# Roywangj/AdaptPoint

Measured on AMD Instinct MI355X. Metric: set-abstraction fwd+bwd point-clouds/sec (B=32,N=1024), higher is better.
Workload: dtype bf16

## Files before the change

adaptpoint_amd/_lib.py:

```python
import ctypes
import os

_HERE = os.path.dirname(os.path.abspath(__file__))
LIB_PATH = os.path.join(_HERE, "libadaptpoint_amd.so")
if os.environ.get("APN_LIB_PATH"):
    if os.environ.get("APN_ALLOW_UNSAFE_LIB") != "1":
        raise RuntimeError("APN_LIB_PATH is for diagnostic builds: set APN_ALLOW_UNSAFE_LIB=1 with it")
    LIB_PATH = os.path.abspath(os.environ["APN_LIB_PATH"])
REQUIRED_BUILD_FLAGS = ("-ffp-contract=off", "-fno-slp-vectorize")

_c_int, _c_float, _c_void_p = ctypes.c_int, ctypes.c_float, ctypes.c_void_p
_c_double = ctypes.c_double
_c_longlong = ctypes.c_longlong

SIGNATURES = {
    "apn_version": [],
    "apn_furthest_point_sampling": [_c_int] * 3 + [_c_void_p] * 4,
    "apn_ball_query": [_c_int] * 3 + [_c_float, _c_int] + [_c_void_p] * 4,
    "apn_group_points": [_c_int] * 5 + [_c_void_p] * 4,
    "apn_group_points_grad": [_c_int] * 5 + [_c_void_p] * 4,
    "apn_gather_points": [_c_int] * 4 + [_c_void_p] * 4,
    "apn_gather_points_grad": [_c_int] * 4 + [_c_void_p] * 4,
    "apn_resample_points": [_c_int] * 6 + [_c_void_p] * 6,
    "apn_three_nn": [_c_int] * 3 + [_c_void_p] * 5,
    "apn_three_interpolate": [_c_int] * 4 + [_c_void_p] * 5,
    "apn_three_interpolate_grad": [_c_int] * 4 + [_c_void_p] * 5,
    "apn_furthest_point_sampling_tuned": [_c_int] * 3 + [_c_void_p] * 3 + [_c_int] * 2 + [_c_void_p],
    "apn_fps_debug_stamps": [_c_int] * 3 + [_c_void_p] * 5,
    "apn_furthest_point_sampling_xyz": [_c_int] * 3 + [_c_void_p] * 5,
    "apn_ball_query_zero": [_c_int] * 3 + [_c_float, _c_int] + [_c_void_p] * 4,
    "apn_sa_grid_blocks": [_c_int] * 2,
    "apn_sa_grid_rows": [_c_int] * 3,
    "apn_sa_bwd_main_rows": [_c_int] * 2,
    "apn_sa_acc_words": [_c_int],
    "apn_sa_debug_stamps": [_c_void_p],
    "apn_zero_fill": [_c_void_p, _c_longlong, _c_void_p],
    "apn_debug_stamp": [_c_void_p, _c_int, _c_void_p],
    "apn_debug_vgpr_hold": [_c_int, _c_int, _c_void_p, _c_void_p],
    "apn_debug_vpk_probe": [_c_int, _c_int, _c_int, _c_void_p, _c_void_p],
    "apn_sa_geo_dd_doubles": [_c_int],
    "apn_sa_point_geo": [_c_int] * 4 + [_c_float] + [_c_void_p] * 6,
    "apn_sa_prep_rows": [_c_int] * 2,
    "apn_sa_prep_stats": [_c_int] * 2 + [_c_void_p] * 4 + [_c_int] * 2 + [_c_void_p] * 3 + [_c_longlong, _c_void_p],
    "apn_sa_reduce_rows": [_c_void_p, _c_int, _c_int, _c_double, _c_void_p, _c_void_p],
    "apn_sa_reduce_acc": [_c_void_p, _c_int, _c_double, _c_void_p, _c_void_p],
    "apn_sa_bn_fold": [_c_void_p, _c_int, _c_void_p, _c_int, _c_double, _c_void_p, _c_void_p,
                       _c_float, _c_float, _c_void_p, _c_void_p, _c_void_p, _c_int, _c_void_p,
                       _c_void_p, _c_int, _c_void_p, _c_void_p],
    "apn_sa_fwd_main": [_c_int] * 4 + [_c_float] + [_c_void_p] * 12 + [_c_float, _c_float, _c_int, _c_double,
                                                                        _c_void_p, _c_int] + [_c_void_p] * 7,
    "apn_sa_fwd_out": [_c_int] * 3 + [_c_void_p] * 8 + [_c_float, _c_float, _c_int, _c_double] + [_c_void_p] * 2
                      + [_c_int] + [_c_void_p] * 3 + [_c_int] + [_c_void_p] * 2 + [_c_longlong, _c_void_p],
    "apn_sa_bwd_prep_rows": [_c_int] * 2,
    "apn_sa_bwd_prep": [_c_int] * 3 + [_c_void_p] + [_c_longlong] * 3 + [_c_void_p] + [_c_int]
                       + [_c_void_p] * 3 + [_c_int] + [_c_void_p] * 8,
    "apn_sa_bwd_main": [_c_int] * 4 + [_c_float] + [_c_void_p] * 11 + [_c_double, _c_int] + [_c_void_p] * 9,
    "apn_sa_bwd_weight_rows": [_c_int] * 2,
    "apn_sa_bwd_point_grads": [_c_int] * 3 + [_c_void_p] * 7 + [_c_double, _c_int] + [_c_void_p] * 2 + [_c_int]
                              + [_c_void_p] * 4 + [_c_float] + [_c_void_p] * 5,
    "apn_sa_bwd_finalize": [_c_void_p, _c_int, _c_float, _c_void_p, _c_void_p, _c_int, _c_void_p, _c_void_p, _c_int]
                           + [_c_void_p] * 11,
    "apn_sa_forward_seq": ([_c_int] * 5 + [_c_float] + [_c_void_p] * 12
                           + [_c_void_p] * 5 + [_c_float, _c_float, _c_int]
                           + [_c_void_p] * 5 + [_c_float, _c_float, _c_int]
                           + [_c_double, _c_int] + [_c_void_p] * 11 + [_c_longlong, _c_void_p]),
    "apn_sa_backward_seq": ([_c_int] * 5 + [_c_float] + [_c_void_p] * 15 + [_c_int] * 3
                            + [_c_double] + [_c_void_p] + [_c_longlong] * 3 + [_c_void_p]
                            + [_c_longlong]
                            + [_c_void_p] * 26),
    "apn_attention_small_max": [],
    "apn_attention_small_fwd": [_c_int] * 3 + [_c_void_p] * 5,
    "apn_attention_small_bwd": [_c_int] * 3 + [_c_void_p] * 8,
    "apn_attention_prep": [_c_int] * 3 + [_c_void_p] * 4 + [_c_int, _c_void_p],
    "apn_attention_fwd": [_c_int] * 3 + [_c_void_p] * 4,
    "apn_attention_bwd": [_c_int] * 3 + [_c_void_p] * 9,
    "apn_token_attention_max_tokens": [],
    "apn_token_attention_fwd": [_c_int] * 3 + [_c_void_p] * 4,
    "apn_token_attention_bwd": [_c_int] * 3 + [_c_void_p] * 7,
    "apn_pointset_group_rows": [_c_int] * 3,
    "apn_pointset_group_max": [_c_int] * 5 + [_c_void_p] * 8,
    "apn_pointset_group_max_grad": [_c_int] * 5 + [_c_void_p] * 9,
    "apn_sa_wide_grid": [_c_int] * 2,
    "apn_sa_wide_colsum_chunks": [_c_int] * 2,
    "apn_sa_wide_colsum": [_c_void_p, _c_int, _c_int, _c_void_p, _c_void_p, _c_void_p],
    "apn_sa_wide_tilemap_ints": [_c_int] * 2,
    "apn_sa_wide_tilemap": [_c_int] * 3 + [_c_void_p] * 3,
    "apn_sa_wide_tilemap_many": [_c_int] * 4 + [_c_void_p] * 3,
    "apn_sa_rowmap_many": [_c_int] * 4 + [_c_void_p] * 6,
    "apn_sa_rowmap_ints": [_c_int] * 2,
    "apn_sa_rowmap_places": [_c_int] * 3,
    "apn_sa_wide_stats1": [_c_int] * 4 + [_c_void_p] * 6,
    "apn_sa_wide_fwd_main": [_c_int] * 5 + [_c_void_p] * 11,
    "apn_sa_wide_bwd_main": [_c_int] * 5 + [_c_void_p] * 15,
    "apn_sa_wide_wgrad_fused": [_c_int],
    "apn_sa_wide_image": [_c_void_p, _c_int, _c_int, _c_void_p, _c_int, _c_int, _c_int, _c_void_p, _c_void_p],
    "apn_sa_wide_bwd_prep_rows": [_c_int] * 2,
    "apn_sa_wide_bwd_prep": [_c_int] * 3 + [_c_void_p] + [_c_longlong] * 3 + [_c_void_p] * 7,
    "apn_sa_wide_consts2": [_c_void_p, _c_int, _c_void_p, _c_int, _c_void_p, _c_double, _c_int] + [_c_void_p] * 4,
    "apn_sa_wide_consts1": [_c_void_p, _c_int, _c_void_p, _c_int, _c_void_p, _c_double, _c_int] + [_c_void_p] * 4,
    "apn_sa_wide_point_terms": [_c_int] * 4 + [_c_void_p] * 5 + [_c_int, _c_float] + [_c_void_p] * 7,
    "apn_sa_wide_wgrad_splits": [_c_int] * 3,
    "apn_sa_wide_csr": [_c_int] * 3 + [_c_void_p] * 9,
    "apn_sa_wide_fwd_prep": [_c_int] * 6 + [_c_float] + [_c_void_p] * 13,
    "apn_sa_wide_fwd_prep_rows": [_c_int] * 3,
    "apn_sa_wide_out": [_c_int] * 3 + [_c_void_p] * 2 + [_c_int] + [_c_void_p] * 3 + [_c_int] + [_c_void_p] * 2,
    "apn_sa_wide_bwd_mid": [_c_void_p, _c_int, _c_void_p, _c_int, _c_int, _c_void_p, _c_double, _c_int] + [_c_void_p] * 7,
    "apn_sa_wide_bwd_fin": [_c_void_p, _c_int, _c_void_p, _c_int, _c_int, _c_void_p, _c_double, _c_int] + [_c_void_p] * 8,
    "apn_sa_wide_point_grads_rows": [_c_int] * 2,
    "apn_sa_wide_point_grads_cols": [_c_int] * 3,
    "apn_sa_wide_point_grads": [_c_int] * 5 + [_c_float] + [_c_void_p] * 13 + [_c_int] + [_c_void_p] * 9,
    "apn_sa_wide_colsum_f32": [_c_void_p, _c_int, _c_int, _c_void_p, _c_void_p],
    "apn_sa_wide_wgrad": [_c_int] * 5 + [_c_void_p] * 7 + [_c_int] + [_c_void_p] * 2,
    "apn_pw_conv_tiles": [_c_int] * 2,
    "apn_pw_conv_forward": [_c_int] * 5 + [_c_void_p] * 5,
    "apn_pw_bn_act": [_c_int] * 3 + [_c_void_p] * 2 + [_c_int] + [_c_void_p] * 2 + [_c_float] * 2 + [_c_int] * 2
                     + [_c_void_p] * 6,
    "apn_pw_bn_act_grad_splits": [_c_int] * 2,
    "apn_pw_bn_act_grad": [_c_int] * 3 + [_c_void_p] * 3 + [_c_int] * 2 + [_c_void_p] * 5,
    "apn_pw_conv_grad_input": [_c_int] * 5 + [_c_void_p] * 4,
    "apn_pw_conv_grad_weight_splits": [_c_int] * 4,
    "apn_pw_conv_grad_weight": [_c_int] * 5 + [_c_void_p] * 5,
    "apn_deform_forward": [_c_int] * 3 + [_c_void_p] * 6 + [_c_float] + [_c_void_p] * 4,
    "apn_deform_backward": [_c_int] * 3 + [_c_void_p] * 4 + [_c_float] + [_c_void_p] * 7,
    "apn_pw_contract_splits": [_c_int] * 4,
    "apn_pw_contract": [_c_int] * 4 + [_c_void_p, _c_longlong, _c_int, _c_int] * 2 + [_c_void_p, _c_longlong, _c_int, _c_int,
                                                                                         _c_void_p, _c_int, _c_void_p],
    "apn_pw_contract2_splits": [_c_int] * 9,
    "apn_pw_contract2": [_c_int] * 3 + [_c_void_p] * 16,
    "apn_fp_blend_stats": [_c_int] * 4 + [_c_void_p] * 6 + [_c_int] + [_c_void_p] * 4 + [_c_float, _c_int] + [_c_void_p] * 3,
    "apn_pw_transpose": [_c_int] * 3 + [_c_void_p] * 3,
    "apn_three_nn_weights": [_c_longlong] + [_c_void_p] * 3,
    "apn_anchor_transforms": [_c_int] + [_c_void_p] * 3 + [_c_float] * 3 + [_c_void_p] * 3,
    "apn_anchor_transforms_grad": [_c_int] + [_c_void_p] * 3 + [_c_float] * 3 + [_c_void_p] * 4,
    "apn_pw_conv_max_tiles": [_c_int],
    "apn_pw_conv_max_forward": [_c_int] * 5 + [_c_void_p] * 3 + [_c_int] + [_c_void_p] * 5,
    "apn_pw_conv_max_backward": [_c_int] * 4 + [_c_void_p] * 5 + [_c_int] + [_c_void_p] * 5,
    "apn_spectral_norm_blocks": [_c_int] * 2,
    "apn_spectral_norm": [_c_int] * 2 + [_c_void_p, _c_int, _c_float] + [_c_void_p] * 8,
    "apn_spectral_norm_grad": [_c_int] * 2 + [_c_void_p] * 8,
    "apn_spectral_norm_many": [_c_int] + [_c_void_p] * 3 + [_c_int, _c_float] + [_c_void_p] * 8,
    "apn_spectral_norm_grad_many": [_c_int] + [_c_void_p] * 10,
    "apn_sa_sample_overlap": [_c_int] * 3 + [_c_float, _c_int] + [_c_void_p] * 7,
    "apn_sa_sample_seq": [_c_int] * 3 + [_c_float, _c_int] + [_c_void_p] * 8,
    "apn_furthest_point_sampling_nested": [_c_int] * 3 + [_c_void_p] * 6,
    "apn_sa_sample_seq_nested": [_c_int] * 3 + [_c_float, _c_int] + [_c_void_p] * 9,
    "apn_pointwolf_params": [_c_int] * 2 + [_c_void_p, _c_int] + [_c_float] * 3 + [_c_void_p] * 4,
    "apn_rsmix_select": [_c_int] * 3 + [_c_void_p] * 2 + [_c_double, _c_int, _c_int] + [_c_void_p] * 3,
    "apn_rsmix_mix": [_c_int] * 4 + [_c_void_p] * 8,
    "apn_cloud_transform": [_c_int] * 4 + [_c_void_p] * 2 + [_c_int] * 2 + [_c_void_p] * 8,
    "apn_cls_confusion": [_c_int] * 2 + [_c_void_p, _c_int] + [_c_void_p] * 5,
    "apn_la_pool_rows": [_c_int] * 2,
    "apn_la_pool_fwd": [_c_int] * 4 + [_c_float] + [_c_void_p] * 3 + [_c_int] + [_c_void_p] * 7,
    "apn_la_stats_fold": [_c_void_p, _c_int, _c_int, _c_double, _c_void_p, _c_void_p],
    "apn_la_pool_bwd": [_c_int] * 4 + [_c_float] + [_c_void_p] * 11 + [_c_int] + [_c_void_p] * 4,
    "apn_knn_query": [_c_int] * 5 + [_c_void_p] * 5,
    "apn_knn_dilated": [_c_int] * 7 + [_c_void_p] * 6,
    "apn_ec_pool_rows": [_c_int] * 2,
    "apn_ec_pool_fwd": [_c_int] * 4 + [_c_void_p, _c_int] + [_c_void_p] * 7,
    "apn_ec_out": [_c_int] * 3 + [_c_void_p] * 2 + [_c_float] + [_c_void_p] * 2,
    "apn_ec_bwd_prep_rows": [_c_int] * 2,
    "apn_ec_bwd_prep": [_c_int] * 3 + [_c_void_p] + [_c_longlong] * 3 + [_c_void_p] * 2 + [_c_float] + [_c_void_p] * 3,
    "apn_ec_out_res": [_c_int] * 3 + [_c_void_p] * 2 + [_c_float, _c_void_p] + [_c_longlong] * 3 + [_c_void_p] * 2,
    "apn_ec_bwd_prep_act": [_c_int] * 3 + [_c_void_p] + [_c_longlong] * 3 + [_c_void_p] * 2 + [_c_float] + [_c_void_p] * 3,
    "apn_ec_csr": [_c_int] * 3 + [_c_void_p] * 5,
    "apn_ec_pool_bwd": [_c_int] * 4 + [_c_void_p] * 5 + [_c_int] + [_c_void_p] * 4,
    "apn_chamfer_max_points": [],
    "apn_chamfer_forward": [_c_int] * 3 + [_c_void_p] * 7,
    "apn_chamfer_backward": [_c_int] * 3 + [_c_void_p] * 9,
    "apn_emd_max_points": [],
    "apn_emd_one_launch_max": [],
    "apn_emd_cost_parts": [_c_int],
    "apn_emd_ratios": [_c_int] * 3 + [_c_void_p] * 6,
    "apn_emd_match": [_c_int] * 3 + [_c_void_p] * 6,
    "apn_emd_cost": [_c_int] * 3 + [_c_void_p] * 8,
    "apn_emd_cost_grad": [_c_int] * 3 + [_c_void_p] * 9,
    "apn_po_knn_query": [_c_int] * 4 + [_c_void_p] * 7,
    "apn_po_ball_query": [_c_int] * 3 + [_c_float, _c_int] + [_c_void_p] * 6,
    "apn_po_furthest_sampling": [_c_int] * 2 + [_c_void_p] * 6,
    "apn_po_csr": [_c_int] * 3 + [_c_void_p] * 5,
    "apn_po_grouping_fwd": [_c_int] * 4 + [_c_void_p] * 4,
    "apn_po_grouping_bwd": [_c_int] * 4 + [_c_void_p] * 5,
    "apn_po_interpolation_fwd": [_c_int] * 4 + [_c_void_p] * 5,
    "apn_po_interpolation_bwd": [_c_int] * 4 + [_c_void_p] * 6,
    "apn_po_subtraction_fwd": [_c_int] * 4 + [_c_void_p] * 5,
    "apn_po_subtraction_bwd": [_c_int] * 4 + [_c_void_p] * 6,
    "apn_po_aggregation_fwd": [_c_int] * 5 + [_c_void_p] * 6,
    "apn_po_aggregation_bwd": [_c_int] * 5 + [_c_void_p] * 11,
    "apn_pt_rows": [_c_int] * 3,
    "apn_pt_mid_rows": [_c_int] * 3,
    "apn_pt_rel_stats": [_c_int] * 3 + [_c_void_p, _c_int] + [_c_void_p] * 5,
    "apn_pt_fold": [_c_void_p, _c_int, _c_int, _c_void_p, _c_void_p],
    "apn_pt_colsum_rows": [_c_int],
    "apn_pt_colsum": [_c_int, _c_int, _c_void_p, _c_int, _c_void_p, _c_void_p],
    "apn_pt_mid": [_c_int] * 3 + [_c_void_p, _c_int] + [_c_void_p] * 7,
    "apn_pt_attend": [_c_int] * 3 + [_c_void_p, _c_int] + [_c_void_p] * 8,
    "apn_pt_attend_bwd": [_c_int] * 3 + [_c_void_p, _c_int] + [_c_void_p] * 10,
    "apn_pt_mid_bwd": [_c_int] * 3 + [_c_void_p, _c_int] + [_c_void_p] * 9,
    "apn_pt_rel_bwd": [_c_int] * 3 + [_c_void_p, _c_int] + [_c_void_p] * 12 + [_c_int, _c_void_p, _c_void_p],
    "apn_pt_scatter_bwd": [_c_int] * 3 + [_c_void_p] * 6 + [_c_int, _c_void_p],
    "apn_vg_scratch_ints": [_c_int],
    "apn_vg_voxelize": [_c_int] * 3 + [_c_void_p] + [_c_double] * 3 + [_c_void_p] * 9,
    "apn_vg_mean_fwd": [_c_int] * 3 + [_c_void_p] * 6,
    "apn_vg_mean_bwd": [_c_int] * 3 + [_c_void_p] * 5,
    "apn_rl_moment_rows": [_c_int] * 3,
    "apn_rl_bwd_rows": [_c_int] * 4,
    "apn_rl_moments": [_c_int] * 3 + [_c_void_p] * 3 + [_c_int] + [_c_void_p] * 3,
    "apn_rl_fold": [_c_int, _c_void_p, _c_double] + [_c_void_p] * 4 + [_c_float, _c_float, _c_int] + [_c_void_p] * 6,
    "apn_rl_forward": [_c_int] * 4 + [_c_void_p] * 3 + [_c_int] + [_c_void_p] * 4,
    "apn_rl_backward": [_c_int] * 4 + [_c_void_p] * 3 + [_c_int] + [_c_void_p] * 6,
    "apn_rl_finalize": [_c_int, _c_int, _c_void_p, _c_void_p, _c_double] + [_c_void_p] * 4 + [_c_int] + [_c_void_p] * 3,
    "apn_ag_moment_rows": [_c_int],
    "apn_ag_point_rows": [_c_int],
    "apn_ag_moments": [_c_int] * 5 + [_c_void_p] * 5,
    "apn_ag_fold": [_c_int] * 2 + [_c_void_p] * 3,
    "apn_ag_combine_fwd": [_c_int] * 5 + [_c_void_p] * 7 + [_c_int] + [_c_void_p] * 4 + [_c_float, _c_int] + [_c_void_p] * 3,
    "apn_ag_combine_bwd": [_c_int] * 5 + [_c_void_p] * 11,
    "apn_ag_sigma_bwd": [_c_int] * 5 + [_c_void_p] * 11,
    "apn_ag_res_relu_max": [_c_int] * 4 + [_c_void_p] * 5,
    "apn_ag_res_relu_max_grad": [_c_int] * 4 + [_c_void_p] * 6,
}

_lib = None


class ExtensionMissing(RuntimeError):
    pass


def load():
    global _lib
    if _lib is not None:
        return _lib
    if not os.path.exists(LIB_PATH):
        raise ExtensionMissing(
            f"{LIB_PATH} not found: build it with `python -m adaptpoint_amd.build` "
            "(hipcc --offload-arch=gfx950). There is no fallback path.")
    lib = ctypes.CDLL(LIB_PATH)
    for name, argtypes in SIGNATURES.items():
        fn = getattr(lib, name)
        fn.argtypes = argtypes
        fn.restype = _c_int
    lib.apn_error_string.argtypes = [_c_int]
    lib.apn_error_string.restype = ctypes.c_char_p
    lib.apn_build_flags.argtypes = []
    lib.apn_build_flags.restype = ctypes.c_char_p
    flags = lib.apn_build_flags().decode("utf-8", "replace").split()
    missing = [f for f in REQUIRED_BUILD_FLAGS if f not in flags]
    if missing and os.environ.get("APN_ALLOW_UNSAFE_LIB") != "1":
        raise ExtensionMissing(f"{LIB_PATH} was built without {missing} (its flags: {' '.join(flags)}): rebuild with "
                               "`python -m adaptpoint_amd.build --force`")
    _lib = lib
    return lib


def check(code, what):
    if code != 0:
        msg = load().apn_error_string(code).decode("utf-8", "replace")
        raise RuntimeError(f"{what} failed: {msg} (code {code})")
```

adaptpoint_amd/csrc/sa_fused.hip:

```cpp
#include "apn_common.h"
#include "apn_mfma.h"
#include <type_traits>
#include "sa_chain.h"

namespace apn {

constexpr int SA_C = 32;
constexpr int SA_C1 = 32;
constexpr int SA_C2 = 64;
constexpr int SA_K = 32;
constexpr int SA_WAVES = 4;

template <int NS>
__device__ __forceinline__ void put_frag(uint4 *base, int f, int lane, const Frag<NS> &v) {
#pragma unroll
    for (int p = 0; p < NS; ++p) base[(f * NS + p) * 64 + lane] = __builtin_bit_cast(uint4, v.p[p]);
}

template <int NS>
__device__ __forceinline__ Frag<NS> get_frag(const uint4 *base, int f, int lane) {
    Frag<NS> v;
#pragma unroll
    for (int p = 0; p < NS; ++p) v.p[p] = __builtin_bit_cast(bf16x8, base[(f * NS + p) * 64 + lane]);
    return v;
}

template <int NS>
__device__ __forceinline__ float eff(float v) {
    const __bf16 hi = (__bf16)v;
    float r = (float)hi;
    if (NS == 2) r += (float)(__bf16)(v - r);
    return r;
}

struct SaArgs {
    int b, n, m;
    const float *xyz;
    const float *new_xyz;
    const __bf16 *ft;
    const __bf16 *ft_lo;
    const int *idx;
    const float *w1;
    float radius;
    const int *tmap;
    unsigned long long *stamps;
};

__device__ __forceinline__ void stamp(const SaArgs &a, int wave, int k) {
    if (a.stamps && (threadIdx.x & 63) == 0)
        a.stamps[((size_t)blockIdx.x * SA_WAVES + wave) * 16 + k] = wall_clock64();
}

__device__ __forceinline__ int tm_tiles(const SaArgs &a) { return a.tmap[0]; }
__device__ __forceinline__ const int *tm_tq0(const SaArgs &a) { return a.tmap + 4; }
__device__ __forceinline__ const unsigned *tm_rows(const SaArgs &a) {
    return reinterpret_cast<const unsigned *>(a.tmap + 4 + ((a.b * a.m + 3) & ~3));
}
__device__ __forceinline__ const int *tm_nn(const SaArgs &a) {
    return a.tmap + 4 + ((a.b * a.m + 3) & ~3) + (size_t)32 * a.b * a.m;
}
__device__ __forceinline__ unsigned ri_q(unsigned info) { return info & 0xffu; }
__device__ __forceinline__ unsigned ri_slot(unsigned info) { return (info >> 8) & 0xffu; }
__device__ __forceinline__ unsigned ri_mult(unsigned info) { return (info >> 16) & 0xffu; }
__device__ __forceinline__ void row_meta(unsigned info, int h, unsigned (&meta)[16]) {
#pragma unroll
    for (int i = 0; i < 16; ++i) meta[i] = (unsigned)__builtin_amdgcn_ds_bpermute(acc_row(i, h) << 2, (int)info);
}

template <int NS>
__device__ __forceinline__ void load_w1_frags(const float *__restrict__ w1, int r, int h,
                                              Frag<NS> (&wf)[3]) {
#pragma unroll
    for (int s = 0; s < 3; ++s) {
        float t[8];
#pragma unroll
        for (int j = 0; j < 8; ++j)
            t[j] = s < 2 ? w1[r * 35 + 3 + 16 * s + 8 * h + j]
                         : ((h == 0 && j < 3) ? w1[r * 35 + j] : 0.0f);
        wf[s] = make_frag<NS>(t);
    }
}

constexpr int PS_PTS = 512, PS_MAX_ROWS = 64, PS_NT = 2 * PS_PTS;
constexpr double GEO_INV_UNIT = 1.0 / 68719476736.0;

#ifdef APN_WG_STAMPS
__device__ unsigned long long *d_wg_stamps_f = nullptr;
__device__ __forceinline__ void wg_stamp(int k) {
    unsigned long long *st = d_wg_stamps_f;
    if (st && threadIdx.x == 0) st[(size_t)blockIdx.x * 16 + k] = wall_clock64();
}
#else
__device__ __forceinline__ void wg_stamp(int) {}
#endif

template <int NS>
__global__ __launch_bounds__(PS_NT) void sa_prep_stats_kernel(
    int n, int tiles_per_cloud, int total_tiles, const float *__restrict__ f, const long long *__restrict__ geo,
    const double *__restrict__ dd, int dd_rows, const float *__restrict__ w1, int stats, __bf16 *__restrict__ ft,
    __bf16 *__restrict__ ft_lo, float *__restrict__ part, unsigned long long *__restrict__ zero, long long zero_words) {
    extern __shared__ float sf_raw[];
    float (*sf)[PS_PTS + 1] = reinterpret_cast<float (*)[PS_PTS + 1]>(sf_raw);
    __shared__ float4 sgeo[PS_PTS];
    __shared__ float red[PS_NT / 64][64];
    __shared__ double sdd[6];
    const int tid = threadIdx.x, lane = tid & 63, r = lane & 31, h = lane >> 5;
    const int wave = __builtin_amdgcn_readfirstlane(tid >> 6);
    critical_stream_priority();
    wg_stamp(0);
    for (long long e = (long long)blockIdx.x * PS_NT + tid; e < zero_words; e += (long long)gridDim.x * PS_NT) zero[e] = 0ull;
    Frag<NS> wf[3];
    load_w1_frags<NS>(w1, r, h, wf);
    const float wp0 = eff<NS>(w1[r * 35]), wp1 = eff<NS>(w1[r * 35 + 1]), wp2 = eff<NS>(w1[r * 35 + 2]);
    float s1 = 0.0f, s2 = 0.0f;
    for (int tile = blockIdx.x; tile < total_tiles; tile += gridDim.x) {
        const int cloud = tile / tiles_per_cloud, n0 = (tile % tiles_per_cloud) * PS_PTS;
        {
            const int pt = tid & (PS_PTS - 1), cg = tid / PS_PTS;
            const bool in = n0 + pt < n;
            float v[16];
#pragma unroll
            for (int k = 0; k < 16; ++k) v[k] = in ? f[((size_t)cloud * SA_C + cg + 2 * k) * n + n0 + pt] : 0.0f;
            float4 gv = make_float4(0.f, 0.f, 0.f, 0.f);
            if (stats && in && cg == 0) {
                const longlong2 *gp = reinterpret_cast<const longlong2 *>(geo + ((size_t)cloud * n + n0 + pt) * 4);
                const longlong2 g0 = gp[0], g1 = gp[1];
                gv = make_float4((float)g0.x, (float)((double)g0.y * GEO_INV_UNIT), (float)((double)g1.x * GEO_INV_UNIT),
                                 (float)((double)g1.y * GEO_INV_UNIT));
            }
            wg_stamp(1);
            __syncthreads();
#pragma unroll
            for (int k = 0; k < 16; ++k) sf[cg + 2 * k][pt] = v[k];
            if (cg == 0) sgeo[pt] = gv;
            wg_stamp(2);
        }
        __syncthreads();
        wg_stamp(3);
        const int pt = 32 * wave + r;
        float x0[8], x1[8];
#pragma unroll
        for (int j = 0; j < 8; ++j) { x0[j] = sf[8 * h + j][pt]; x1[j] = sf[16 + 8 * h + j][pt]; }
        const Frag<NS> a0 = make_frag<NS>(x0), a1 = make_frag<NS>(x1);
        if (n0 + pt < n) {
            uint4 *row = reinterpret_cast<uint4 *>(ft + ((size_t)cloud * n + n0 + pt) * SA_C);
            row[h] = __builtin_bit_cast(uint4, a0.p[0]);
            row[2 + h] = __builtin_bit_cast(uint4, a1.p[0]);
            if (NS == 2) {
                uint4 *rl = reinterpret_cast<uint4 *>(ft_lo + ((size_t)cloud * n + n0 + pt) * SA_C);
                rl[h] = __builtin_bit_cast(uint4, a0.p[NS - 1]);
                rl[2 + h] = __builtin_bit_cast(uint4, a1.p[NS - 1]);
            }
        }
        wg_stamp(4);
        if (stats) {
            f32x16 y = {0};
            y = mfma<NS>(a0, wf[0], y);
            y = mfma<NS>(a1, wf[1], y);
#pragma unroll
            for (int i = 0; i < 16; ++i) {
                const float4 g = sgeo[32 * wave + acc_row(i, h)];
                const float PD = __builtin_fmaf(wp2, g.w, __builtin_fmaf(wp1, g.z, wp0 * g.y));
                const float oF = g.x * y[i];
                s1 += oF + PD;
                s2 += __builtin_fmaf(oF, y[i], 2.0f * y[i] * PD);
            }
        }
    }
    wg_stamp(5);
    if (!stats) return;
    s1 += __shfl_xor(s1, 32);
    s2 += __shfl_xor(s2, 32);
    if (lane < 32) { red[wave][r] = s1; red[wave][32 + r] = s2; }
    if (blockIdx.x == 0 && wave >= 1 && wave < 7) {
        double s = 0.0;
        for (int e = lane; e < dd_rows; e += 64) s += dd[(size_t)e * 6 + (wave - 1)];
#pragma unroll
        for (int o = 32; o > 0; o >>= 1) s += __shfl_xor(s, o);
        if (lane == 0) sdd[wave - 1] = s;
    }
    __syncthreads();
    if (tid < 64) {
        float val = 0.0f;
#pragma unroll
        for (int w = 0; w < PS_NT / 64; ++w) val += red[w][tid];
        if (tid >= 32 && blockIdx.x == 0) {
            const double wx = wp0, wy = wp1, wz = wp2;
            const double t = wx * wx * sdd[0] + 2.0 * wx * wy * sdd[1] + 2.0 * wx * wz * sdd[2] + wy * wy * sdd[3] +
                             2.0 * wy * wz * sdd[4] + wz * wz * sdd[5];
            val += (float)t;
        }
        part[(size_t)blockIdx.x * 64 + tid] = val;
    }
    wg_stamp(6);
}

template <int NS>
struct TileRaw {
    uint4 f[2], fl[NS];
    float px, py, pz;
    float qx, qy, qz;
    int nb;
    unsigned info;
    int q0;
};

struct TileHead {
    int nb, q0;
    unsigned info;
    int tile;
};
template <bool CP>
__device__ __forceinline__ TileHead load_head(const SaArgs &a, int tile, int r) {
    TileHead t;
    t.tile = tile;
    if (CP) {
        t.nb = tm_nn(a)[(size_t)tile * SA_K + r];
        t.info = tm_rows(a)[(size_t)tile * SA_K + r];
        t.q0 = tm_tq0(a)[tile];
    } else {
        t.nb = a.idx[(size_t)tile * SA_K + r];
        t.info = 0x10000u | ((unsigned)r << 8);
        t.q0 = tile;
    }
    return t;
}

template <typename T>
__device__ __forceinline__ T ld_off(const void *base, unsigned byte_off) {
    return *reinterpret_cast<const T *>(reinterpret_cast<const char *>(base) + byte_off);
}

template <int NS>
__device__ __forceinline__ void fetch_tile(const SaArgs &a, const TileHead &hd, int h, TileRaw<NS> &t) {
    const int nb = hd.nb;
    const unsigned cloud = (unsigned)(hd.q0 / a.m);
    const unsigned pt = cloud * (unsigned)a.n + (unsigned)nb;
    const unsigned rowoff = pt * (unsigned)(SA_C * 2) + 16u * (unsigned)h;
    t.f[0] = ld_off<uint4>(a.ft, rowoff);
    t.f[1] = ld_off<uint4>(a.ft, rowoff + 32u);
    if (NS == 2) {
        t.fl[0] = ld_off<uint4>(a.ft_lo, rowoff);
        t.fl[NS - 1] = ld_off<uint4>(a.ft_lo, rowoff + 32u);
    }
    struct xyz3 { float x, y, z; };
    const xyz3 pp = ld_off<xyz3>(a.xyz, pt * 12u);
    t.px = pp.x; t.py = pp.y; t.pz = pp.z;
    const unsigned q = (unsigned)hd.q0 + (ri_mult(hd.info) ? ri_q(hd.info) : 0u);
    const xyz3 qq = ld_off<xyz3>(a.new_xyz, q * 12u);
    t.qx = qq.x; t.qy = qq.y; t.qz = qq.z;
    t.nb = nb;
    t.info = hd.info;
    t.q0 = hd.q0;
}

template <int NS>
__device__ __forceinline__ void build_frags(const SaArgs &a, const TileRaw<NS> &t, int h,
                                            Frag<NS> (&x)[3], float *deff = nullptr) {
    x[0].p[0] = __builtin_bit_cast(bf16x8, t.f[0]);
    x[1].p[0] = __builtin_bit_cast(bf16x8, t.f[1]);
    if (NS == 2) {
        x[0].p[NS - 1] = __builtin_bit_cast(bf16x8, t.fl[0]);
        x[1].p[NS - 1] = __builtin_bit_cast(bf16x8, t.fl[NS - 1]);
    }
    float d[8] = {0.f, 0.f, 0.f, 0.f, 0.f, 0.f, 0.f, 0.f};
    if (h == 0 || deff) {
        d[0] = (t.px - t.qx) / a.radius;
        d[1] = (t.py - t.qy) / a.radius;
        d[2] = (t.pz - t.qz) / a.radius;
    }
    if (deff) {
#pragma unroll
        for (int j = 0; j < 3; ++j) {
            const __bf16 hi = (__bf16)d[j];
            deff[j] = (float)hi;
            if (NS == 2) deff[j] += (float)(__bf16)(d[j] - (float)hi);
        }
        if (h != 0) d[0] = d[1] = d[2] = 0.0f;
    }
    x[2] = make_frag<NS>(d);
}

__device__ __forceinline__ void touch(const TileHead &hd) {
    asm volatile("" ::"v"(hd.nb), "v"(hd.info), "v"(hd.q0));
}

struct NoAhead {
    __device__ __forceinline__ void operator()(const TileHead &) const {}
};
template <int NS, bool CP, bool LATE = false, typename Pro, typename Pre, typename Body, typename Ahead = NoAhead>
__device__ __forceinline__ void for_each_tile(const SaArgs &a, int wave, int r, int h, Pro prologue, Pre pre, Body body,
                                              Ahead ahead = Ahead()) {
    const int cap = a.b * a.m, stride = gridDim.x * SA_WAVES;
    const int tiles = CP ? tm_tiles(a) : cap;
    const bool xcd = (gridDim.x & 7) == 0;
    const int per_x = (tiles + 7) >> 3;
    auto remap = [&](int t) {
        if (!xcd) return t;
        const int wg = t / SA_WAVES, wv = t - wg * SA_WAVES;
        const int x = wg & 7, u = (wg >> 3) * SA_WAVES + wv;
        return u < per_x ? x * per_x + u : tiles;
    };
    int slot = blockIdx.x * SA_WAVES + wave;
    int tile = remap(slot);
    const TileHead hd0 = load_head<CP>(a, tile < tiles ? tile : 0, r);
    TileHead hd_nxt = load_head<CP>(a, remap(slot + stride) < tiles ? remap(slot + stride) : 0, r);
    TileRaw<NS> cur, nxt;
    const bool any = tile < tiles;
    stamp(a, wave, 1);
    if (any) {
        ahead(hd0);
        fetch_tile<NS>(a, hd0, h, cur);
    }
    prologue();
    stamp(a, wave, 2);
    if (!any) return;
    int nst = 3;
    for (; tile < tiles; slot += stride, tile = remap(slot)) {
        const bool more = remap(slot + stride) < tiles;
        const int tile2 = remap(slot + 2 * stride);
        if (LATE) {
            const TileHead hd_nxt2 = load_head<CP>(a, tile2 < tiles ? tile2 : tile, r);
            body(tile, cur, nst == 4, [&] {
                asm volatile("" ::: "memory");
                touch(hd_nxt);
                if (more) {
                    ahead(hd_nxt);
                    fetch_tile<NS>(a, hd_nxt, h, cur);
                }
            });
            stamp(a, wave, nst < 5 ? nst : 5);
            ++nst;
            hd_nxt = hd_nxt2;
            continue;
        }
        touch(hd_nxt);
        pre();
        if (more) fetch_tile<NS>(a, hd_nxt, h, nxt);
        const TileHead hd_nxt2 = load_head<CP>(a, tile2 < tiles ? tile2 : tile, r);
        body(tile, cur, nst == 4, [&] { touch(hd_nxt2); });
        stamp(a, wave, nst < 5 ? nst : 5);
        ++nst;
        if (more) cur = nxt;
        hd_nxt = hd_nxt2;
    }
    pre();
    stamp(a, wave, 6);
}

template <int NV>
__device__ __forceinline__ float fold_partials(float (&vals)[NV], int lane, int wave) {
    __shared__ float red[SA_WAVES][NV][32];
#pragma unroll
    for (int i = 0; i < NV; ++i) {
        const float other = __shfl_xor(vals[i], 32);
        if (lane < 32) red[wave][i][lane] = vals[i] + other;
    }
    __syncthreads();
    float s = 0.0f;
    const int e = threadIdx.x;
    if (e < NV * 32) {
#pragma unroll
        for (int w = 0; w < SA_WAVES; ++w) s += red[w][e >> 5][e & 31];
    }
    return s;
}

__device__ __forceinline__ void fold_rows32(const float *__restrict__ part, int rows, const double *__restrict__ sums,
                                            const BnArgs &bn, float *__restrict__ pack, float &scale, float &shift,
                                            double *scratch ) {
    double (*fred)[64] = reinterpret_cast<double (*)[64]>(scratch);
    double *ftot = scratch + 16 * 64;
    const int tid = threadIdx.x;
    double count = bn.count;
    double gpre = 1.0, bpre = 0.0;
    if (tid < 32) {
        if (bn.gamma) gpre = (double)bn.gamma[tid];
        if (bn.beta) bpre = (double)bn.beta[tid];
    }
    if (bn.training) {
        if (part) {
            const int quad = tid & 15, rg = tid >> 4;
            const float4 *__restrict__ p4 = reinterpret_cast<const float4 *>(part) + quad;
            double s0 = 0.0, s1 = 0.0, s2 = 0.0, s3 = 0.0;
            int rr = rg;
            for (; rr + 7 * 16 < rows; rr += 8 * 16) {
                float4 v[8];
#pragma unroll
                for (int u = 0; u < 8; ++u) v[u] = p4[(size_t)(rr + 16 * u) * 16];
#pragma unroll
                for (int u = 0; u < 8; ++u) {
                    s0 += (double)v[u].x; s1 += (double)v[u].y; s2 += (double)v[u].z; s3 += (double)v[u].w;
                }
            }
            for (; rr + 3 * 16 < rows; rr += 4 * 16) {
                float4 v[4];
#pragma unroll
                for (int u = 0; u < 4; ++u) v[u] = p4[(size_t)(rr + 16 * u) * 16];
#pragma unroll
                for (int u = 0; u < 4; ++u) {
                    s0 += (double)v[u].x; s1 += (double)v[u].y; s2 += (double)v[u].z; s3 += (double)v[u].w;
                }
            }
            for (; rr < rows; rr += 16) {
                const float4 v = p4[(size_t)rr * 16];
                s0 += (double)v.x; s1 += (double)v.y; s2 += (double)v.z; s3 += (double)v.w;
            }
            fred[rg][4 * quad] = s0; fred[rg][4 * quad + 1] = s1; fred[rg][4 * quad + 2] = s2; fred[rg][4 * quad + 3] = s3;
            __syncthreads();
            if (tid < 64) {
                double s = 0.0;
#pragma unroll
                for (int k = 0; k < 16; ++k) s += fred[k][tid];
                ftot[tid] = s;
            }
        } else if (tid < 64) {
            ftot[tid] = sums[tid];
        }
// ... 385 lines not shown
        {
            const float4 *scv = reinterpret_cast<const float4 *>(bn1v[0][lane_o >> 5]);
            const float4 *shv = reinterpret_cast<const float4 *>(bn1v[1][lane_o >> 5]);
#pragma unroll
            for (int i4 = 0; i4 < 4; ++i4) {
                const float4 sc = scv[i4], sh = shv[i4];
                yT[4 * i4] = __builtin_fmaxf(__builtin_fmaf(yT[4 * i4], sc.x, sh.x), 0.0f);
                yT[4 * i4 + 1] = __builtin_fmaxf(__builtin_fmaf(yT[4 * i4 + 1], sc.y, sh.y), 0.0f);
                yT[4 * i4 + 2] = __builtin_fmaxf(__builtin_fmaf(yT[4 * i4 + 2], sc.z, sh.z), 0.0f);
                yT[4 * i4 + 3] = __builtin_fmaxf(__builtin_fmaf(yT[4 * i4 + 3], sc.w, sh.w), 0.0f);
            }
        }
        st2(1);
        Frag<NS> a0, a1;
        if (CP) {
            f32x16 yw;
#pragma unroll
            for (int i = 0; i < 16; ++i) yw[i] = yT[i] * mrow;
            a0 = pack8<NS>(yw, 0);
            a1 = pack8<NS>(yw, 8);
        } else {
            a0 = pack8<NS>(yT, 0);
            a1 = pack8<NS>(yT, 8);
        }

        Frag<NS> sp[4];
        {
            unsigned todo = starts;
            if (CP) {
                asm volatile("s_waitcnt vmcnt(0)" ::: "memory");
                const int dq = q0 - qb;
#pragma unroll
                for (int u = 0; u < 4; ++u) {
                    const int e = (u + dq < 4 ? u + dq : 3) * SA_C2 + lane_o;
                    gv4[u] = qgoa[wave][e];
                    kc4[u] = qksel[wave][e];
                }
            }
#pragma unroll 1
            for (int jb = 0; jb < nq; jb += 4) {
                if (jb) {
#pragma unroll
                    for (int u = 0; u < 4; ++u)
                        if (jb + u < nq) {
                            gv4[u] = g.goa[(size_t)(q0 + jb + u) * SA_C2 + lane];
                            kc4[u] = g.ksel[(size_t)(q0 + jb + u) * SA_C2 + lane];
                        }
                }
#pragma unroll
                for (int u = 0; u < 4; ++u) {
                    if (jb + u < nq) {
                        const float gv = gv4[u];
                        int kc = kc4[u];
                        if (CP) {
                            kc += __builtin_ctz(todo);
                            todo &= todo - 1u;
                        }
                        const __bf16 ghi = (__bf16)gv;
                        const __bf16 glo = (__bf16)(gv - (float)ghi);
                        __bf16 *cell = sp_img + kc * SP_ROW + lane;
                        cell[0] = ghi;
                        if (NS == 2) cell[SP_TILE] = glo;
                        if (!CP) kc4[u] = kc;
                    }
                }
            }
        }
        asm volatile("" ::: "memory");
        {
            f32x16 an;
            const float sc1 = chan[0][lane_o & 31], sh1 = chan[1][lane_o & 31];
#pragma unroll
            for (int i = 0; i < 16; ++i) {
                an[i] = __builtin_fmaxf(__builtin_fmaf(y1[i], sc1, sh1), 0.0f);
                if (CP) suma = __builtin_fmaf(multf(i), an[i], suma);
                else suma += an[i];
            }
            const Frag<NS> b0 = pack8<NS>(an, 0), b1 = pack8<NS>(an, 8);
            if (CP) {
                f32x16 aw;
#pragma unroll
                for (int i = 0; i < 16; ++i) aw[i] = an[i] * multf(i);
                gram = mfma<NS>(pack8<NS>(aw, 0), b0, gram);
                gram = mfma<NS>(pack8<NS>(aw, 8), b1, gram);
            } else {
                gram = mfma<NS>(b0, b0, gram);
                gram = mfma<NS>(b1, b1, gram);
            }
            typedef short tr_s4 __attribute__((ext_vector_type(4)));
            typedef short tr_s8 __attribute__((ext_vector_type(8)));
            typedef __attribute__((address_space(3))) tr_s4 tr_lds;
            const int li = lane_o & 15, gq = li >> 2, gp = li & 3, grh = (lane_o >> 4) & 1;
            const __bf16 *tb = sp_img + (4 * (lane_o >> 5) + gq) * SP_ROW + 16 * grh + 4 * gp;
#pragma unroll
            for (int t = 0; t < 2; ++t) {
#pragma unroll
                for (int sk = 0; sk < 2; ++sk) {
                    Frag<NS> at;
#pragma unroll
                    for (int pp = 0; pp < NS; ++pp) {
                        const __bf16 *src = tb + pp * SP_TILE + (16 * sk) * SP_ROW + 32 * t;
                        const tr_s4 lo4 = __builtin_amdgcn_ds_read_tr16_b64_v4i16((tr_lds *)(src));
                        const tr_s4 hi4 = __builtin_amdgcn_ds_read_tr16_b64_v4i16((tr_lds *)(src + 8 * SP_ROW));
                        const tr_s8 v8 = {lo4.x, lo4.y, lo4.z, lo4.w, hi4.x, hi4.y, hi4.z, hi4.w};
                        at.p[pp] = __builtin_bit_cast(bf16x8, v8);
                    }
                    dsp[t] = mfma<NS>(at, sk ? b1 : b0, dsp[t]);
                }
            }
        }
        st2(2);
#pragma unroll
        for (int s = 0; s < 4; ++s) {
            const __bf16 *src = sp_img + r * SP_ROW + 16 * s + 8 * h;
            sp[s].p[0] = *reinterpret_cast<const bf16x8 *>(src);
            if (NS == 2) sp[s].p[NS - 1] = *reinterpret_cast<const bf16x8 *>(src + SP_TILE);
        }
        asm volatile("" ::: "memory");
        if (!CP) {
            __bf16 *cell = sp_img + kc4[0] * SP_ROW + lane;
            cell[0] = (__bf16)0.0f;
            if (NS == 2) cell[SP_TILE] = (__bf16)0.0f;
        }
        f32x16 ga;
        const float ev = chan[4][lane_o & 31];
#pragma unroll
        for (int i = 0; i < 16; ++i) ga[i] = CP ? ev * multf(i) : ev;
        ga = mfma<NS>(a0, get_frag<NS>(cfrag, F_QM, lane_o), ga);
        ga = mfma<NS>(a1, get_frag<NS>(cfrag, F_QM + 1, lane_o), ga);
#pragma unroll
        for (int s = 0; s < 4; ++s) ga = mfma<NS>(sp[s], get_frag<NS>(cfrag, F_W2T + s, lane_o), ga);

        st2(3);
        float *gt = reinterpret_cast<float *>(sp_img);
        asm volatile("" ::: "memory");
        float s1 = 0.0f, s2 = 0.0f, hb = 0.0f;
        const float sc1l = chan[0][lane_o & 31], sh1l = chan[1][lane_o & 31], iv1 = chan[3][lane_o & 31];
        const float nmi = -chan[2][lane_o & 31] * iv1;
#pragma unroll
        for (int i = 0; i < 16; ++i) {
            const float u = __builtin_fmaf(y1[i], sc1l, sh1l);
            const float yhat = __builtin_fmaf(y1[i], iv1, nmi);
            ga[i] = u > 0.0f ? ga[i] : 0.0f;
            s1 += ga[i];
            s2 += ga[i] * yhat;
            if (CP) {
                gt[acc_row(i, h) * 33 + r] = ga[i];
                gt[32 * 33 + acc_row(i, h) * 33 + r] = multf(i) * yhat;
            } else {
                hb += yhat;
            }
        }
        st[0] += s1;
        st[1] += s2;

        st2(4);
        before_stores();
        {
            int live;
            if (CP) {
                asm volatile("" ::: "memory");
                const float *mine = gt + h * (32 * 33) + r;
                float *dst = (h ? HB : HA) + (size_t)q0 * SA_C1 + r;
                int seg = -1;
                float sum = 0.0f;
#pragma unroll
                for (int half16 = 0; half16 < 2; ++half16) {
                    float v[16];
#pragma unroll
                    for (int i = 0; i < 16; ++i) v[i] = mine[(16 * half16 + i) * 33];
#pragma unroll
                    for (int i = 0; i < 16; ++i) {
                        if ((starts >> (16 * half16 + i)) & 1u) {
                            if (seg >= 0 && seg < nq) dst[(size_t)seg * SA_C1] = sum;
                            ++seg;
                            sum = 0.0f;
                        }
                        sum += v[i];
                    }
                }
                if (seg >= 0 && seg < nq) dst[(size_t)seg * SA_C1] = sum;
                asm volatile("" ::: "memory");
                {
                    uint4 *z = reinterpret_cast<uint4 *>(sp_img);
#pragma unroll
                    for (int e = 0; e < (NS * SP_TILE * 2 / 16 + 63) / 64; ++e)
                        if (e * 64 + lane < NS * SP_TILE * 2 / 16) z[e * 64 + lane] = make_uint4(0u, 0u, 0u, 0u);
                }
                asm volatile("" ::: "memory");
                live = __popcll(__ballot(lane < 32 && live_row));
            } else {
                const float ha = s1 + __shfl_xor(s1, 32);
                hb += __shfl_xor(hb, 32);
                if (h == 0) {
                    HA[(size_t)tile * SA_C1 + r] = ha;
                    HB[(size_t)tile * SA_C1 + r] = hb;
                }
                live = 0;
            }

            st2(5);
            st2(6);
            if (CP) {
                const int *dl = &sdst[wave][body_n & 1][0];
#pragma unroll
                for (int gq = 0; gq < 4; ++gq) {
                    if (8 * gq < live) {
                        const int4 dd = *reinterpret_cast<const int4 *>(&dl[8 * gq + 4 * (lane_o >> 5)]);
                        const int base = 8 * gq + 4 * h;
                        if (base + 0 < live) gu_store(dd.x, ga[4 * gq + 0]);
                        if (base + 1 < live) gu_store(dd.y, ga[4 * gq + 1]);
                        if (base + 2 < live) gu_store(dd.z, ga[4 * gq + 2]);
                        if (base + 3 < live) gu_store(dd.w, ga[4 * gq + 3]);
                    }
                }
            }
            ++body_n;
        }
    }, ahead);
    {
        const float tot = fold_partials<2>(st, lane, wave);
        if (threadIdx.x < 64) acc_add(accT, 64, blockIdx.x % ACC_COPIES, threadIdx.x, tot);
    }
    float (*wred)[SA_C2 * SA_C1] = reinterpret_cast<float (*)[SA_C2 * SA_C1]>(sp_raw);
    __syncthreads();
#pragma unroll
    for (int i = 0; i < 16; ++i) {
        wred[wave][acc_row(i, h) * SA_C1 + r] = dsp[0][i];
        wred[wave][(32 + acc_row(i, h)) * SA_C1 + r] = dsp[1][i];
    }
    __syncthreads();
    const int ec = threadIdx.x >> 2, emid = (threadIdx.x & 3) * 8;
    float sp8[8];
    {
        float4 lo4 = make_float4(0.f, 0.f, 0.f, 0.f), hi4 = lo4;
#pragma unroll
        for (int w = 0; w < SA_WAVES; ++w) {
            const float4 a4 = *reinterpret_cast<const float4 *>(&wred[w][ec * SA_C1 + emid]);
            const float4 b4 = *reinterpret_cast<const float4 *>(&wred[w][ec * SA_C1 + emid + 4]);
            lo4.x += a4.x; lo4.y += a4.y; lo4.z += a4.z; lo4.w += a4.w;
            hi4.x += b4.x; hi4.y += b4.y; hi4.z += b4.z; hi4.w += b4.w;
        }
        sp8[0] = lo4.x; sp8[1] = lo4.y; sp8[2] = lo4.z; sp8[3] = lo4.w;
        sp8[4] = hi4.x; sp8[5] = hi4.y; sp8[6] = hi4.z; sp8[7] = hi4.w;
    }
    __syncthreads();
    suma += __shfl_xor(suma, 32);
#pragma unroll
    for (int i = 0; i < 16; ++i) wred[wave][acc_row(i, h) * SA_C1 + r] = gram[i];
    if (h == 0) wred[wave][SA_C1 * SA_C1 + r] = suma;
    __syncthreads();
    for (int e = threadIdx.x; e < SA_C1 * SA_C1 + SA_C1; e += SA_WAVES * 64)
        sqm[e >> 5][e & 31] = (wred[0][e] + wred[1][e]) + (wred[2][e] + wred[3][e]);
    __syncthreads();
    {
        float acc[8];
#pragma unroll
        for (int j = 0; j < 8; ++j) acc[j] = 0.0f;
#pragma unroll 8
        for (int k = 0; k < SA_C1; ++k) {
            const float w = sw2[ec][k];
            const float4 g0 = *reinterpret_cast<const float4 *>(&sqm[k][emid]);
            const float4 g1 = *reinterpret_cast<const float4 *>(&sqm[k][emid + 4]);
            acc[0] = __builtin_fmaf(w, g0.x, acc[0]); acc[1] = __builtin_fmaf(w, g0.y, acc[1]);
            acc[2] = __builtin_fmaf(w, g0.z, acc[2]); acc[3] = __builtin_fmaf(w, g0.w, acc[3]);
            acc[4] = __builtin_fmaf(w, g1.x, acc[4]); acc[5] = __builtin_fmaf(w, g1.y, acc[5]);
            acc[6] = __builtin_fmaf(w, g1.z, acc[6]); acc[7] = __builtin_fmaf(w, g1.w, acc[7]);
        }
        const float d = sD[ec], e = sE[ec];
        const float4 s0 = *reinterpret_cast<const float4 *>(&sqm[32][emid]);
        const float4 s1 = *reinterpret_cast<const float4 *>(&sqm[32][emid + 4]);
        float4 *row = reinterpret_cast<float4 *>(partW2 + (size_t)blockIdx.x * (SA_C2 * SA_C1) + ec * SA_C1 + emid);
        row[0] = make_float4(sp8[0] + d * acc[0] + e * s0.x, sp8[1] + d * acc[1] + e * s0.y,
                             sp8[2] + d * acc[2] + e * s0.z, sp8[3] + d * acc[3] + e * s0.w);
        row[1] = make_float4(sp8[4] + d * acc[4] + e * s1.x, sp8[5] + d * acc[5] + e * s1.y,
                             sp8[6] + d * acc[6] + e * s1.z, sp8[7] + d * acc[7] + e * s1.w);
    }
    stamp(a, wave, 7);
}

static int sa_grid(int tiles, bool compact = false) {
    const int cap = compact ? 768 : 512;
    int g = (tiles + SA_WAVES - 1) / SA_WAVES;
    return g < cap ? (g < 1 ? 1 : g) : cap;
}

static int sa_grid_bwd(int tiles) {
    int g = sa_grid(tiles);
    return g < 448 ? g : 448;
}

}

extern "C" int apn_sa_grid_blocks(int b, int m) { return apn::sa_grid(b * m); }
extern "C" int apn_sa_grid_rows(int b, int m, int with_tile_map) { return apn::sa_grid(b * m, with_tile_map != 0); }
extern "C" int apn_sa_bwd_main_rows(int b, int m) { return apn::sa_grid_bwd(b * m); }
extern "C" int apn_sa_acc_words(int ncol) { return ncol > 0 ? apn::acc_words(ncol) : 0; }

extern "C" int apn_sa_prep_rows(int b, int n) {
    const long long tiles = (long long)b * ((n + apn::PS_PTS - 1) / apn::PS_PTS);
    return (int)(tiles < apn::PS_MAX_ROWS ? (tiles < 1 ? 1 : tiles) : apn::PS_MAX_ROWS);
}

extern "C" int apn_sa_prep_stats(int b, int n, const float *f, const void *geo, const void *dd, const float *w1,
                                 int precision, int stats, void *ft, float *part1, void *zero, long long zero_words,
                                 void *stream) {
    using namespace apn;
    if (b <= 0 || n <= 0 || b > 65535 || (precision != 1 && precision != 2) || !f || !ft || !w1) return APN_EINVAL;
    if (stats && (!geo || !dd || !part1 || ((uintptr_t)geo & 15) || ((uintptr_t)part1 & 15))) return APN_EINVAL;
    if (zero_words < 0 || (zero_words && !zero)) return APN_EINVAL;
    __bf16 *hi = (__bf16 *)ft;
    __bf16 *lo = precision == 2 ? hi + (size_t)b * n * SA_C : nullptr;
    const int tpc = (n + PS_PTS - 1) / PS_PTS;
    auto kern = precision == 2 ? sa_prep_stats_kernel<2> : sa_prep_stats_kernel<1>;
    const int lds = SA_C * (PS_PTS + 1) * (int)sizeof(float);
    static DynLdsOnce lds_set[2];
    if (hipError_t e = set_dyn_lds(lds_set[precision - 1], (const void *)kern, lds)) return (int)e;
    hipLaunchKernelGGL(kern, dim3(apn_sa_prep_rows(b, n)), dim3(PS_NT), lds, (hipStream_t)stream, n, tpc, b * tpc, f,
                       (const long long *)geo, (const double *)dd, b * (apn_sa_geo_dd_doubles(n) / 6), w1, stats, hi, lo, part1,
                       (unsigned long long *)zero, zero_words);
    APN_LAUNCH_CHECK();
    return APN_OK;
}

#ifdef APN_WG_STAMPS
extern "C" __attribute__((visibility("default"))) int apn_sa_debug_wg_stamps_fused(void *buf) {
    return (int)hipMemcpyToSymbol(HIP_SYMBOL(apn::d_wg_stamps_f), &buf, sizeof(buf));
}
#endif

static unsigned long long *g_stamps = nullptr;
extern "C" int apn_sa_debug_stamps(void *buf) { g_stamps = (unsigned long long *)buf; return APN_OK; }

static apn::SaArgs sa_args(int b, int n, int m, const float *xyz, const float *new_xyz, const void *ft,
                           int precision, const int *idx, const float *w1, float radius, const int *tmap) {
    const __bf16 *hi = (const __bf16 *)ft;
    return apn::SaArgs{b, n, m, xyz, new_xyz, hi,
                       precision == 2 ? hi + (size_t)b * n * apn::SA_C : nullptr, idx, w1, radius, tmap, g_stamps};
}

static int sa_check(int b, int n, int m, int precision) {
    if (precision != 1 && precision != 2) return APN_EINVAL;
    if (b <= 0 || n <= 0 || m <= 0) return APN_EINVAL;
    if ((long long)b * m > 0x7fffffffLL / 64) return APN_EINVAL;
    if ((long long)b * n > 0xffffffffLL / 256) return APN_EINVAL;
    if ((long long)b * m > 0xffffffffLL / (32 * 128)) return APN_EINVAL;
    return APN_OK;
}

extern "C" int apn_sa_fwd_main(int b, int n, int m, int precision, float radius, const float *xyz,
                               const float *new_xyz, const void *ft, const int *idx, const int *tmap, const float *w1,
                               const float *w2, const float *g1, const float *b1, float *rm1, float *rv1, void *nbt1,
                               float eps1, float mom1, int train1, double count, const float *part1, int rows1,
                               const double *sums1, float *pack1, const float *gamma2, float *ysel, void *ksel,
                               void *acc2, void *stream) {
    using namespace apn;
    if (int e = sa_check(b, n, m, precision)) return e;
    if (!xyz || !new_xyz || !ft || !idx || !w1 || !w2 || !pack1 || !ysel || !ksel || !acc2) return APN_EINVAL;
    if (train1 && !part1 && !sums1) return APN_EINVAL;
    if (!train1 && (!rm1 || !rv1)) return APN_EINVAL;
    if (part1 && (((uintptr_t)part1 & 15) || rows1 <= 0)) return APN_EINVAL;
    SaArgs a = sa_args(b, n, m, xyz, new_xyz, ft, precision, idx, w1, radius, tmap);
    BnArgs bn{g1, b1, rm1, rv1, (long long *)nbt1, eps1, mom1, train1, count};
    auto kern = precision == 2 ? (tmap ? sa_fwd_main_kernel<2, true> : sa_fwd_main_kernel<2, false>)
                               : (tmap ? sa_fwd_main_kernel<1, true> : sa_fwd_main_kernel<1, false>);
    hipLaunchKernelGGL(kern, dim3(sa_grid(b * m, tmap != nullptr)), dim3(SA_WAVES * 64), 0, (hipStream_t)stream, a, w2, bn,
                       sums1 ? nullptr : part1, rows1, sums1, pack1, gamma2, ysel, (unsigned char *)ksel,
                       (unsigned long long *)acc2);
    APN_LAUNCH_CHECK();
    return APN_OK;
}

extern "C" int apn_sa_bwd_main(int b, int n, int m, int precision, float radius, const float *xyz,
                               const float *new_xyz, const void *ft, const int *idx, const int *tmap, const float *w1,
                               const float *w2, const float *pack1, const float *pack2, const void *accS,
                               const double *sumsS, double count, int train2, const float *goa, const void *ksel,
                               void *accT, float *partW2, const int *rowdst, float *GU, float *HA, float *HB, void *stream) {
    using namespace apn;
    if (int e = sa_check(b, n, m, precision)) return e;
    if (!w2 || !pack1 || !pack2 || (!accS && !sumsS) || !goa || !ksel || !accT || !partW2 || !GU || !HA || !HB)
        return APN_EINVAL;
    if (!tmap || !rowdst) return APN_EINVAL;
    SaArgs a = sa_args(b, n, m, xyz, new_xyz, ft, precision, idx, w1, radius, tmap);
    SaBwdArgs g;
    g.w2 = w2;
    g.scale1 = pack1; g.shift1 = pack1 + 32; g.mean1 = pack1 + 64; g.inv1 = pack1 + 96;
    g.pack2 = pack2;
    g.accS = (const unsigned long long *)accS; g.sumsS = sumsS;
    g.count = count; g.train2 = train2;
    g.goa = goa; g.ksel = (const unsigned char *)ksel;
    g.rowdst = rowdst;
    auto kern = precision == 2 ? sa_bwd_kernel<2, true> : sa_bwd_kernel<1, true>;
    hipLaunchKernelGGL(kern, dim3(sa_grid_bwd(b * m)), dim3(SA_WAVES * 64), 0, (hipStream_t)stream, a, g,
                       (unsigned long long *)accT, partW2, GU, HA, HB);
    APN_LAUNCH_CHECK();
    return APN_OK;
}
```

adaptpoint_amd/csrc/sa_glue.hip:

```cpp
#include "apn_common.h"
#include "sa_chain.h"
#include "apn_mfma.h"

namespace apn {

#ifdef APN_WG_STAMPS
__device__ unsigned long long *d_wg_stamps = nullptr;
__device__ __forceinline__ void wg_stamp(int k) {
    unsigned long long *st = d_wg_stamps;
    if (st && threadIdx.x == 0)
        st[((size_t)blockIdx.y * gridDim.x + blockIdx.x) * 16 + k] = wall_clock64();
}
#else
__device__ __forceinline__ void wg_stamp(int) {}
#endif


typedef __attribute__((ext_vector_type(8))) __bf16 bf16x8;

__device__ __forceinline__ void block_sum_rows(const float *__restrict__ part, int rows, int ncol,
                                               const double *__restrict__ sums, double *out) {
    __shared__ double red[1024 * 4];
    const int t = threadIdx.x;
    if (!part) {
        if (t < ncol) out[t] = sums[t];
        __syncthreads();
        return;
    }
    const int quads = ncol >> 2, q = t % quads, g = t / quads, groups = 1024 / quads;
    const float4 *__restrict__ p4 = (const float4 *)part;
    double s0 = 0.0, s1 = 0.0, s2 = 0.0, s3 = 0.0;
    int r = g;
    for (; r + 7 * groups < rows; r += 8 * groups) {
        float4 v[8];
#pragma unroll
        for (int u = 0; u < 8; ++u) v[u] = p4[(size_t)(r + u * groups) * quads + q];
#pragma unroll
        for (int u = 0; u < 8; ++u) {
            s0 += (double)v[u].x; s1 += (double)v[u].y; s2 += (double)v[u].z; s3 += (double)v[u].w;
        }
    }
    for (; r < rows; r += groups) {
        const float4 v = p4[(size_t)r * quads + q];
        s0 += (double)v.x; s1 += (double)v.y; s2 += (double)v.z; s3 += (double)v.w;
    }
    double *mine = red + (size_t)g * ncol + 4 * q;
    mine[0] = s0; mine[1] = s1; mine[2] = s2; mine[3] = s3;
    __syncthreads();
    for (int st = groups >> 1; st > 0; st >>= 1) {
        if (g < st) {
            const double *other = mine + (size_t)st * ncol;
#pragma unroll
            for (int j = 0; j < 4; ++j) mine[j] += other[j];
        }
        __syncthreads();
    }
    if (t < ncol) out[t] = red[t];
    __syncthreads();
}

__global__ __launch_bounds__(1024) void reduce_rows_kernel(const float *__restrict__ part, int rows,
                                                           int ncol, double count,
                                                           double *__restrict__ out) {
    __shared__ double s[128];
    block_sum_rows(part, rows, ncol, nullptr, s);
    if (threadIdx.x < ncol) out[threadIdx.x] = s[threadIdx.x];
    if (threadIdx.x == 0) { out[ncol] = count; out[ncol + 1] = 1.0; }
}

__device__ __forceinline__ void slice_sum_rows(const float *__restrict__ part, int rows, int quads,
                                               int qa, int qb, double (*red)[4]) {
    const int t = threadIdx.x, grp = t >> 1;
    const float4 *__restrict__ p4 = reinterpret_cast<const float4 *>(part) + ((t & 1) ? qb : qa);
    double s0 = 0.0, s1 = 0.0, s2 = 0.0, s3 = 0.0;
    int r = grp;
    for (; r + 3 * 128 < rows; r += 4 * 128) {
        float4 v[4];
#pragma unroll
        for (int u = 0; u < 4; ++u) v[u] = p4[(size_t)(r + 128 * u) * quads];
#pragma unroll
        for (int u = 0; u < 4; ++u) {
            s0 += (double)v[u].x; s1 += (double)v[u].y; s2 += (double)v[u].z; s3 += (double)v[u].w;
        }
    }
    for (; r < rows; r += 128) {
        const float4 v = p4[(size_t)r * quads];
        s0 += (double)v.x; s1 += (double)v.y; s2 += (double)v.z; s3 += (double)v.w;
    }
    red[t][0] = s0; red[t][1] = s1; red[t][2] = s2; red[t][3] = s3;
    __syncthreads();
    for (int st = 64; st > 0; st >>= 1) {
        if (grp < st) {
#pragma unroll
            for (int j = 0; j < 4; ++j) red[t][j] += red[t + 2 * st][j];
        }
        __syncthreads();
    }
}

__global__ __launch_bounds__(256) void bn_fold_kernel(
    const float *__restrict__ part, int rows, const double *__restrict__ sums_in, int c, double count,
    const float *__restrict__ gamma, const float *__restrict__ beta, float eps, float momentum,
    float *__restrict__ running_mean, float *__restrict__ running_var, long long *__restrict__ nbt,
    int training, float *__restrict__ pack, const float *__restrict__ sgn_gamma, int sgn_c,
    float *__restrict__ sgn_out) {
    __shared__ double red[256][4];
    const int t = threadIdx.x, i = blockIdx.x * 4 + t;
    float g32 = 1.0f, b32 = 0.0f, rm = 0.0f, rv = 1.0f;
    if (t < 4) {
        if (gamma) g32 = gamma[i];
        if (beta) b32 = beta[i];
        if (running_mean) { rm = running_mean[i]; rv = running_var[i]; }
    }
    if (blockIdx.x == 0) {
        if (t == 0 && training && nbt) *nbt += 1;
        if (sgn_out)
            for (int k = t; k < sgn_c; k += 256) sgn_out[k] = (!sgn_gamma || sgn_gamma[k] >= 0.0f) ? 1.0f : -1.0f;
    }
    double sum = 0.0, sumsq = 0.0;
    if (training) {
        if (part) {
            slice_sum_rows(part, rows, c / 2, blockIdx.x, c / 4 + blockIdx.x, red);
            if (t < 4) { sum = red[0][t]; sumsq = red[1][t]; }
        } else if (t < 4) {
            sum = sums_in[i];
            sumsq = sums_in[c + i];
            count = sums_in[2 * c];
        }
    }
    if (t >= 4) return;
    double mean, var;
    if (training) {
        mean = sum / count;
        var = sumsq / count - mean * mean;
        if (var < 0.0) var = 0.0;
        if (running_mean) {
            const double unbiased = var * (count / (count > 1.0 ? count - 1.0 : 1.0));
            running_mean[i] = (float)((1.0 - momentum) * rm + momentum * mean);
            running_var[i] = (float)((1.0 - momentum) * rv + momentum * unbiased);
        }
    } else {
        mean = rm;
        var = rv;
    }
    const double inv = 1.0 / sqrt(var + (double)eps);
    const double g = g32, b = b32;
    pack[i] = (float)(g * inv);
    pack[c + i] = (float)(b - mean * g * inv);
    pack[2 * c + i] = (float)mean;
    pack[3 * c + i] = (float)inv;
}

template <int NT, int QT, int WST, int FST>
__device__ __forceinline__ void stage_skip_operands(int cloud, int n, int m, int m0,
                                                    const __bf16 *__restrict__ ft,
                                                    const __bf16 *__restrict__ ft_lo,
                                                    const int *__restrict__ fidx,
                                                    const float *__restrict__ ws,
                                                    float (*sws)[WST], float (*sfi)[FST], int *ssrc) {
    constexpr int G = NT / 32, QPT = QT / G, WPT = 64 / G;
    const int tid = threadIdx.x, i = tid & 31, q0 = tid >> 5;
    int src[QPT];
#pragma unroll
    for (int t = 0; t < QPT; ++t) {
        const int q = m0 + q0 + G * t;
        const int got = fidx[(size_t)cloud * m + (q < m ? q : m - 1)];
        src[t] = q < m ? got : -1;
    }
    float wv[WPT];
#pragma unroll
    for (int t = 0; t < WPT; ++t) wv[t] = ws[(q0 + G * t) * 32 + i];
    const __bf16 *lo_tab = ft_lo ? ft_lo : ft;
    __bf16 hv[QPT], lv[QPT];
#pragma unroll
    for (int t = 0; t < QPT; ++t) {
        const size_t o = ((size_t)cloud * n + (src[t] < 0 ? 0 : src[t])) * 32 + i;
        hv[t] = ft[o];
        lv[t] = lo_tab[o];
    }
    float v[QPT];
#pragma unroll
    for (int t = 0; t < QPT; ++t) {
        const float f = (float)hv[t] + (ft_lo ? (float)lv[t] : 0.0f);
        v[t] = src[t] >= 0 ? f : 0.0f;
    }
#pragma unroll
    for (int t = 0; t < QPT; ++t) {
        sfi[q0 + G * t][i] = v[t];
        if (ssrc && i == 0) ssrc[q0 + G * t] = src[t] < 0 ? 0 : src[t];
    }
#pragma unroll
    for (int t = 0; t < WPT; ++t) sws[q0 + G * t][i] = wv[t];
}

template <int QT>
__global__ __launch_bounds__(QT * 16) void fwd_out_kernel(int n, int m, const float *__restrict__ ysel,
                                                          const unsigned long long *__restrict__ acc2,
                                                          const double *__restrict__ sums2, BnArgs bn2,
                                                          float *__restrict__ pack2,
                                                          const __bf16 *__restrict__ ft,
                                                          const __bf16 *__restrict__ ft_lo,
                                                          const int *__restrict__ fidx,
                                                          const float *__restrict__ ws,
                                                          const float *__restrict__ bs, int relu,
                                                          float *__restrict__ out, float4 *__restrict__ zero,
                                                          long long zero_n4) {
    constexpr int NT = QT * 16, NW = NT / 64, HALVES = 64 / QT;
    __shared__ float tile[QT][65];
    __shared__ __attribute__((aligned(16))) float sfi[QT][36];
    __shared__ double ftot[128];
    __shared__ float s_sc[64], s_sh[64];
    const bool first = blockIdx.x == 0 && blockIdx.y == 0;
    critical_stream_priority();
    wg_stamp(0);
    double count2 = bn2.count;
    double g2pre = 1.0, b2pre = 0.0;
    if (threadIdx.x < 64) {
        if (bn2.gamma) g2pre = (double)bn2.gamma[threadIdx.x];
        if (bn2.beta) b2pre = (double)bn2.beta[threadIdx.x];
    }
    if (bn2.training) {
        if (threadIdx.x < 128) ftot[threadIdx.x] = sums2 ? sums2[threadIdx.x] : acc_read(acc2, 128, threadIdx.x);
        if (sums2) count2 = sums2[128];
    }
    __shared__ __attribute__((aligned(16))) float sws[64][36];
    __shared__ float s_bs[64];
    const int cloud = blockIdx.y, m0 = blockIdx.x * QT;
    const int tx = threadIdx.x & 63, ty = threadIdx.x >> 6;
    if (threadIdx.x >= 128 && threadIdx.x < 192) s_bs[tx] = (ws && bs) ? bs[tx] : 0.0f;
    float ys4[4];
#pragma unroll
    for (int k = 0; k < 4; ++k) {
        const int q = m0 + ty + NW * k;
        ys4[k] = ysel[((size_t)cloud * m + (q < m ? q : m - 1)) * 64 + tx];
    }
    if (ws) stage_skip_operands<NT, QT, 36, 36>(cloud, n, m, m0, ft, ft_lo, fidx, ws, sws, sfi, nullptr);
    wg_stamp(1);
    __syncthreads();
    wg_stamp(2);
    if (threadIdx.x < 64) {
        if (first && threadIdx.x == 0 && bn2.training && bn2.nbt) *bn2.nbt += 1;
        float sc, sh;
        bn_channel(bn2, 64, threadIdx.x, bn2.training ? ftot[threadIdx.x] : 0.0, bn2.training ? ftot[64 + threadIdx.x] : 0.0,
                   count2, first, pack2, sc, sh, g2pre, b2pre);
        s_sc[threadIdx.x] = sc;
        s_sh[threadIdx.x] = sh;
    }
    __syncthreads();
    {
        const float sc = s_sc[tx], sh = s_sh[tx];
#pragma unroll
        for (int k = 0; k < 4; ++k) {
            const int j = ty + NW * k;
            tile[j][tx] = m0 + j < m ? ys4[k] * sc + sh : 0.f;
        }
    }
    wg_stamp(3);
    __syncthreads();
    wg_stamp(4);
    if (ws) {
        constexpr int QB = QT / 32;
        if (ty < 2 * QB) {
            const int cb = ty & 1, qb = ty >> 1, r = tx & 31, h = tx >> 5;
            f32x16 acc = {0};
#pragma unroll
            for (int st = 0; st < 2; ++st) {
                float av[8], bv[8];
                const float4 a0 = *reinterpret_cast<const float4 *>(&sws[32 * cb + r][16 * st + 8 * h]);
                const float4 a1 = *reinterpret_cast<const float4 *>(&sws[32 * cb + r][16 * st + 8 * h + 4]);
                const float4 b0 = *reinterpret_cast<const float4 *>(&sfi[32 * qb + r][16 * st + 8 * h]);
                const float4 b1 = *reinterpret_cast<const float4 *>(&sfi[32 * qb + r][16 * st + 8 * h + 4]);
                av[0] = a0.x; av[1] = a0.y; av[2] = a0.z; av[3] = a0.w; av[4] = a1.x; av[5] = a1.y; av[6] = a1.z; av[7] = a1.w;
                bv[0] = b0.x; bv[1] = b0.y; bv[2] = b0.z; bv[3] = b0.w; bv[4] = b1.x; bv[5] = b1.y; bv[6] = b1.z; bv[7] = b1.w;
                acc = mfma<2>(make_frag<2>(av), make_frag<2>(bv), acc);
            }
            const int ql = 32 * qb + r;
#pragma unroll
            for (int e = 0; e < 16; ++e) {
                const int c = 32 * cb + acc_row(e, h);
                float v = tile[ql][c] + (acc[e] + s_bs[c]);
                if (relu) v = fmaxf(v, 0.0f);
                if (m0 + ql < m) out[((size_t)cloud * 64 + c) * m + m0 + ql] = v;
            }
        }
    } else {
        const int ql = tx % QT, hh = tx / QT;
#pragma unroll
        for (int k = 0; k < 4; ++k) {
            const int c = 4 * (ty * HALVES + hh) + k;
            float v = tile[ql][c];
            if (relu) v = fmaxf(v, 0.0f);
            if (m0 + ql < m) out[((size_t)cloud * 64 + c) * m + m0 + ql] = v;
        }
    }
    wg_stamp(5);
    if (zero) {
        const long long nb = (long long)gridDim.x * gridDim.y, bid = (long long)blockIdx.y * gridDim.x + blockIdx.x;
        for (long long i = bid * NT + threadIdx.x; i < zero_n4; i += nb * NT) zero[i] = make_float4(0.f, 0.f, 0.f, 0.f);
    }
    wg_stamp(6);
}

template <int QT>
__global__ __launch_bounds__(QT * 16) void bwd_prep_kernel(int n, int m, const float *__restrict__ g_out,
                                                           long long gs_b, long long gs_c, long long gs_m,
                                                           const float *__restrict__ out, int relu,
                                                           const float *__restrict__ ysel,
                                                           const float *__restrict__ pack2,
                                                           const __bf16 *__restrict__ ft,
                                                           const __bf16 *__restrict__ ft_lo,
                                                           const int *__restrict__ fidx,
                                                           const float *__restrict__ ws,
                                                           float *__restrict__ goa,
                                                           unsigned long long *__restrict__ accS,
                                                           float *__restrict__ partWs,
                                                           float *__restrict__ gip,
                                                           const int *__restrict__ dup) {
    constexpr int NT = QT * 16, NW = NT / 64, HALVES = 64 / QT;
    __shared__ float tile[QT][65];
    __shared__ float red[NW][2][64];
    __shared__ __attribute__((aligned(16))) float sfi[QT][36];
    __shared__ float sws[64][33];
    __shared__ int ssrc[QT];
    constexpr int DW = QT == 32 ? 4 : 2;
    __shared__ float sdfi[DW][QT][33];
    const int cloud = blockIdx.y, m0 = blockIdx.x * QT;
    const int tx = threadIdx.x & 63, ty = threadIdx.x >> 6;
    const int ql = tx % QT, hh = tx / QT;
    critical_stream_priority();
    wg_stamp(0);
    const bool distinct = dup && dup[cloud] == 0;
    const int qc = m0 + ql < m ? m0 + ql : m - 1;
    const float *outp = relu ? out : g_out;
    float gv[4], ov[4];
#pragma unroll
    for (int k = 0; k < 4; ++k) {
        const int c = (ty + NW * k) * HALVES + hh;
        gv[k] = g_out[cloud * gs_b + c * gs_c + qc * gs_m];
        ov[k] = relu ? outp[((size_t)cloud * 64 + c) * m + qc] : 1.0f;
    }
    float ys[4];
#pragma unroll
    for (int k = 0; k < 4; ++k) {
        const int q = m0 + ty + NW * k;
        ys[k] = ysel[((size_t)cloud * m + (q < m ? q : m - 1)) * 64 + tx];
    }
    if (ws) stage_skip_operands<NT, QT, 33, 36>(cloud, n, m, m0, ft, ft_lo, fidx, ws, sws, sfi, ssrc);
#pragma unroll
    for (int k = 0; k < 4; ++k) {
        const int c = (ty + NW * k) * HALVES + hh;
        tile[ql][c] = (m0 + ql < m && ov[k] > 0.0f) ? gv[k] : 0.0f;
    }
    const float sc = pack2[tx], mu = pack2[128 + tx], iv = pack2[192 + tx];
    wg_stamp(1);
    __syncthreads();
    wg_stamp(2);
    float s1 = 0.0f, s2 = 0.0f;
#pragma unroll
    for (int k = 0; k < 4; ++k) {
        const int j = ty + NW * k, q = m0 + j;
        if (q < m) {
            const float g = tile[j][tx];
            const float gs = g * sc;
            goa[((size_t)cloud * m + q) * 64 + tx] = gs;
            s1 += g;
            s2 += g * ((ys[k] - mu) * iv);
        }
    }
    red[ty][0][tx] = s1;
    red[ty][1][tx] = s2;
    wg_stamp(3);
    __syncthreads();
    wg_stamp(4);
    const size_t blk = (size_t)blockIdx.y * gridDim.x + blockIdx.x;
    float sacc = 0.0f;
    if (ty < 2) {
#pragma unroll
        for (int k = 0; k < NW; ++k) sacc += red[k][ty][tx];
    }
    wg_stamp(5);
    if (ws) {
        constexpr int QB = QT / 32;
        const int r = tx & 31, h = tx >> 5;
        if (ty < DW * QB) {
            const int qb = ty / DW, part = ty % DW;
            f32x16 acc = {0};
#pragma unroll
            for (int s4 = 0; s4 < 4 / DW; ++s4) {
                const int st = (4 / DW) * part + s4;
                float av[8], bv[8];
#pragma unroll
                for (int j = 0; j < 8; ++j) {
                    av[j] = tile[32 * qb + r][16 * st + 8 * h + j];
                    bv[j] = sws[16 * st + 8 * h + j][r];
                }
                acc = mfma<2>(make_frag<2>(av), make_frag<2>(bv), acc);
            }
#pragma unroll
            for (int e = 0; e < 16; ++e)
                sdfi[part][32 * qb + acc_row(e, h)][r] = acc[e];
        } else if (ty < DW * QB + 2) {
            const int cb = ty - DW * QB;
            f32x16 acc = {0};
#pragma unroll
            for (int st = 0; st < QT / 16; ++st) {
                float av[8], bv[8];
#pragma unroll
                for (int j = 0; j < 8; ++j) {
                    av[j] = tile[16 * st + 8 * h + j][32 * cb + r];
                    bv[j] = sfi[16 * st + 8 * h + j][r];
                }
                acc = mfma<2>(make_frag<2>(av), make_frag<2>(bv), acc);
            }
#pragma unroll
            for (int e = 0; e < 16; ++e)
                partWs[blk * 2048 + (32 * cb + acc_row(e, h)) * 32 + r] = acc[e];
        }
        __syncthreads();
#pragma unroll
        for (int k = 0; k < QT * 32 / NT; ++k) {
            const int o = threadIdx.x + NT * k, q = o >> 5, i = o & 31;
            float v = sdfi[0][q][i] + sdfi[1][q][i];
            if (DW == 4) v += sdfi[DW - 2][q][i] + sdfi[DW - 1][q][i];
            float *dst = gip + ((size_t)cloud * n + ssrc[q]) * 32 + i;
            if (m0 + q < m) {
                if (distinct) *dst = v;
                else atomicAdd(dst, v);
            }
        }
        wg_stamp(6);
    }
    if (ty < 2) acc_add(accS, 128, (int)(blk % ACC_COPIES), ty * 64 + tx, sacc);
    wg_stamp(7);
}

constexpr int WG_PTS = 64;
constexpr int PG_NT = 512, PG_K = WG_PTS * 32 / PG_NT, PG_M = 32 * 64 / PG_NT;
constexpr int PG_RB = 8;

__global__ __launch_bounds__(PG_NT) void bwd_point_grads_kernel(
    int n, int total_q, int split, const float *__restrict__ GU, const int *__restrict__ pcnt,
    const int *__restrict__ poff, const long long *__restrict__ geo,
    const float *__restrict__ HA, const float *__restrict__ HB, const unsigned long long *__restrict__ accT,
    const double *__restrict__ sumsT, double count, int train1,
    const float *__restrict__ pack1, const __bf16 *__restrict__ ft,
    const __bf16 *__restrict__ ft_lo, const float *__restrict__ xyz,
    const float *__restrict__ new_xyz, const float *__restrict__ w1, const float *__restrict__ gip,
    float inv_r, float *__restrict__ partW, float *__restrict__ g_f, float *__restrict__ g_p,
    float *__restrict__ g_q) {
    __shared__ __attribute__((aligned(16))) float swt[35][36];
    __shared__ __attribute__((aligned(16))) float swr[32][36];
    __shared__ float sG[WG_PTS][33];
    __shared__ float sH[WG_PTS][33];
    __shared__ float sI[WG_PTS][33];
    __shared__ float sB[WG_PTS][41];
    __shared__ float sGeo[WG_PTS][4];
    __shared__ float sc[5][32];
    const int tid = threadIdx.x;
    critical_stream_priority();
    wg_stamp(0);
    const int cloud = blockIdx.y, n0 = blockIdx.x * WG_PTS;
    const int block = cloud * gridDim.x + blockIdx.x;
    const size_t p0 = (size_t)cloud * n + n0;
    const int q0 = block * WG_PTS;
    const int n_here = n - n0 < WG_PTS ? n - n0 : WG_PTS;
    const int c_ld = tid & 31;
    float f_hi[PG_K], f_lo[PG_K], g_i[PG_K], h_a[PG_K], h_b[PG_K];
    const int g_pt = tid >> 3, g_c4 = (tid & 7) * 4;
    int r_cnt, r_off;
    {
        const size_t gp = p0 + (g_pt < n_here ? g_pt : 0);
        r_cnt = g_pt < n_here ? pcnt[gp] : 0;
        r_off = poff[gp];
    }
    float4 a_g = make_float4(0.f, 0.f, 0.f, 0.f);
    {
        const __bf16 *lo_tab = ft_lo ? ft_lo : ft;
        const float *gip_tab = gip ? gip : HA;
#pragma unroll
        for (int k = 0; k < PG_K; ++k) {
            const int pt = (tid >> 5) + (PG_NT / 32) * k;
            const size_t pr = (p0 + (pt < n_here ? pt : 0)) * 32 + c_ld;
            const size_t qr = (size_t)(q0 + pt < total_q ? q0 + pt : 0) * 32 + c_ld;
            f_hi[k] = (float)ft[pr];
            f_lo[k] = (float)lo_tab[pr];
            g_i[k] = gip_tab[gip ? pr : qr];
            h_a[k] = HA[qr];
            h_b[k] = HB[qr];
        }
    }
    float xq_v[2] = {0.0f, 0.0f};
    long long geo_v = 0ll;
    if (tid < WG_PTS * 3) {
        const int pt = tid / 3, d = tid % 3;
        xq_v[0] = xyz[(p0 + (pt < n_here ? pt : 0)) * 3 + d];
        xq_v[1] = new_xyz[(size_t)(q0 + pt < total_q ? q0 + pt : 0) * 3 + d];
    } else if (tid >= PG_NT - WG_PTS * 4) {
        const int e = tid - (PG_NT - WG_PTS * 4), pt = e >> 2, j = e & 3;
        geo_v = geo[(p0 + (pt < n_here ? pt : 0)) * 4 + j];
    }
    for (int e = tid; e < 32 * 35; e += PG_NT) {
        const int mid = e / 35, col = e % 35;
        const float w = w1[e];
        const __bf16 hi = (__bf16)w;
        float wr = (float)hi;
        if (split) wr += (float)(__bf16)(w - wr);
        swt[col][mid] = w;
        swr[mid][col < 3 ? 32 + col : col - 3] = wr;
    }
    if (tid < 64) {
        const int c = tid & 31;
        const float sca = pack1[c];
        float val = 0.0f;
        if (train1) {
            const double t = sumsT ? sumsT[tid] : acc_read(accT, 64, tid);
            const double cnt = sumsT ? sumsT[64] : count;
            val = (float)(-(double)sca * t / cnt);
        }
        sc[tid < 32 ? 2 : 1][c] = val;
        if (tid < 32) sc[0][c] = sca;
    } else if (tid >= 96 && tid < 160) sc[3 + ((tid - 96) >> 5)][tid & 31] = pack1[64 + tid - 96];
    {
        const float *rows = GU + (size_t)(r_cnt > 0 ? r_off : 0) * 32 + g_c4;
        for (int j0 = 0; j0 < r_cnt; j0 += PG_RB) {
            float4 v[PG_RB];
#pragma unroll
            for (int u = 0; u < PG_RB; ++u) {
                const int j = j0 + u < r_cnt ? j0 + u : r_cnt - 1;
                v[u] = *reinterpret_cast<const float4 *>(rows + (size_t)j * 32);
            }
#pragma unroll
            for (int u = 0; u < PG_RB; ++u)
                if (j0 + u < r_cnt) { a_g.x += v[u].x; a_g.y += v[u].y; a_g.z += v[u].z; a_g.w += v[u].w; }
        }
    }
    wg_stamp(1);
    __syncthreads();
    wg_stamp(2);
    {
        const int c = tid & 31;
        const float ca = sc[0][c], cb = sc[1][c], cc = sc[2][c];
#pragma unroll
        for (int k = 0; k < PG_K; ++k) {
            const int pt = (tid >> 5) + (PG_NT / 32) * k;
            const bool ok = pt < n_here;
            sB[pt][6 + c] = ok ? f_hi[k] + (ft_lo ? f_lo[k] : 0.0f) : 0.0f;
            sI[pt][c] = (gip && ok) ? g_i[k] : 0.0f;
            sH[pt][c] = q0 + pt < total_q ? __builtin_fmaf(ca, h_a[k], __builtin_fmaf(cb, h_b[k], cc * 32.0f)) : 0.0f;
        }
    }
    sG[g_pt][g_c4] = a_g.x; sG[g_pt][g_c4 + 1] = a_g.y;
    sG[g_pt][g_c4 + 2] = a_g.z; sG[g_pt][g_c4 + 3] = a_g.w;
    if (tid < WG_PTS * 3) {
        const int pt = tid / 3, d = tid % 3;
        const float xv = xq_v[0], qv = xq_v[1];
        sB[pt][d] = pt < n_here ? xv : 0.0f;
        sB[pt][3 + d] = q0 + pt < total_q ? qv : 0.0f;
        sB[pt][38 + d] = 0.0f;
    } else if (tid >= PG_NT - WG_PTS * 4) {
        const int e = tid - (PG_NT - WG_PTS * 4), pt = e >> 2, j = e & 3;
        const long long gv = pt < n_here ? geo_v : 0ll;
        sGeo[pt][j] = j == 0 ? (float)gv : (float)((double)gv * (1.0 / 68719476736.0));
    }
    wg_stamp(3);
    __syncthreads();
    wg_stamp(4);

    const int tx = tid & 63, ty = tid >> 6;
    {
        const float cnt = sGeo[tx][0], gx = sGeo[tx][1], gy = sGeo[tx][2], gz = sGeo[tx][3];
        float fx[32];
#pragma unroll
        for (int i = 0; i < 32; ++i) fx[i] = sB[tx][6 + i];
#pragma unroll
        for (int mm = 0; mm < PG_M; ++mm) {
            const int mid = PG_M * ty + mm;
            const float4 *wrow = reinterpret_cast<const float4 *>(swr[mid]);
            float accf = 0.0f;
#pragma unroll
            for (int i4 = 0; i4 < 8; ++i4) {
                const float4 w = wrow[i4];
                accf = __builtin_fmaf(w.x, fx[4 * i4], accf);
                accf = __builtin_fmaf(w.y, fx[4 * i4 + 1], accf);
                accf = __builtin_fmaf(w.z, fx[4 * i4 + 2], accf);
                accf = __builtin_fmaf(w.w, fx[4 * i4 + 3], accf);
            }
            const float4 wx = wrow[8];
            const float ys = wx.x * gx + wx.y * gy + wx.z * gz + cnt * accf;
            const float yhs = sc[4][mid] * (ys - cnt * sc[3][mid]);
            sG[tx][mid] = sc[0][mid] * sG[tx][mid] + sc[1][mid] * yhs + sc[2][mid] * cnt;
        }
    }
    wg_stamp(5);
    __syncthreads();
    wg_stamp(6);

    {
        const int r = tx & 31, h = tx >> 5;
        if (ty < 3) {
            const float (*X)[33] = ty == 2 ? sH : sG;
            const int col = ty == 1 ? 32 + r : r;
            const bool mine = ty == 0 ? !(r >= 3 && r <= 5) : (ty == 1 ? r < 6 : (r >= 3 && r <= 5));
            f32x16 acc = {0};
#pragma unroll
            for (int st = 0; st < WG_PTS / 16; ++st) {
                float av[8], bv[8];
#pragma unroll
                for (int j = 0; j < 8; ++j) {
                    av[j] = X[16 * st + 8 * h + j][r];
                    bv[j] = mine ? sB[16 * st + 8 * h + j][col] : 0.0f;
                }
                acc = mfma<2>(make_frag<2>(av), make_frag<2>(bv), acc);
            }
            float *row = partW + (size_t)block * 32 * 38;
            if (mine) {
#pragma unroll
                for (int e = 0; e < 16; ++e) row[acc_row(e, h) * 38 + col] = acc[e];
            }
        } else if (ty < 5) {
            const int pb = ty - 3;
            f32x16 acc = {0};
#pragma unroll
            for (int st = 0; st < 2; ++st) {
                float av[8], bv[8];
                const float4 a0 = *reinterpret_cast<const float4 *>(&swt[3 + r][16 * st + 8 * h]);
                const float4 a1 = *reinterpret_cast<const float4 *>(&swt[3 + r][16 * st + 8 * h + 4]);
                av[0] = a0.x; av[1] = a0.y; av[2] = a0.z; av[3] = a0.w; av[4] = a1.x; av[5] = a1.y; av[6] = a1.z; av[7] = a1.w;
#pragma unroll
                for (int j = 0; j < 8; ++j) bv[j] = sG[32 * pb + r][16 * st + 8 * h + j];
                acc = mfma<2>(make_frag<2>(av), make_frag<2>(bv), acc);
            }
            const int pt = 32 * pb + r;
#pragma unroll
            for (int e = 0; e < 16; ++e) {
                const int i = acc_row(e, h);
                if (pt < n_here) g_f[((size_t)cloud * 32 + i) * n + n0 + pt] = acc[e] + sI[pt][i];
            }
        }
    }
    if (!g_p && !g_q) {
        wg_stamp(7);
        return;
    }

    float gr[32];
#pragma unroll
    for (int mid = 0; mid < 32; ++mid) gr[mid] = sG[tx][mid];
    auto dot_col = [&](const float (&v)[32], int col) {
        const float4 *wcol = reinterpret_cast<const float4 *>(swt[col]);
        float s = 0.0f;
#pragma unroll
        for (int i4 = 0; i4 < 8; ++i4) {
            const float4 w = wcol[i4];
            s = __builtin_fmaf(v[4 * i4], w.x, s);
            s = __builtin_fmaf(v[4 * i4 + 1], w.y, s);
            s = __builtin_fmaf(v[4 * i4 + 2], w.z, s);
            s = __builtin_fmaf(v[4 * i4 + 3], w.w, s);
        }
        return s;
    };
    if (ty < 3 && g_p && tx < n_here) g_p[(p0 + tx) * 3 + ty] += dot_col(gr, ty) * inv_r;
    if (ty >= 4 && ty < 7 && g_q && q0 + tx < total_q) {
        float hr[32];
#pragma unroll
        for (int mid = 0; mid < 32; ++mid) hr[mid] = sH[tx][mid];
        g_q[(size_t)(q0 + tx) * 3 + ty - 4] = -dot_col(hr, ty - 4) * inv_r;
    }
    wg_stamp(7);
}

constexpr int FIN_COLS = 32, FIN_GROUPS = 16;
__device__ __forceinline__ double col_sum(const float *__restrict__ base, int rows, int stride,
                                          int col, int g) {
    double s = 0.0;
    int r = g;
    for (; r + 15 * FIN_GROUPS < rows; r += 16 * FIN_GROUPS) {
        float v[16];
#pragma unroll
        for (int u = 0; u < 16; ++u) v[u] = base[(size_t)(r + FIN_GROUPS * u) * stride + col];
#pragma unroll
        for (int u = 0; u < 16; ++u) s += (double)v[u];
    }
    for (; r + 3 * FIN_GROUPS < rows; r += 4 * FIN_GROUPS) {
        float v[4];
#pragma unroll
        for (int u = 0; u < 4; ++u) v[u] = base[(size_t)(r + FIN_GROUPS * u) * stride + col];
#pragma unroll
        for (int u = 0; u < 4; ++u) s += (double)v[u];
    }
    for (; r < rows; r += FIN_GROUPS) s += (double)base[(size_t)r * stride + col];
    return s;
}

constexpr int FIN_W1 = 32 * 35, FIN_WS = 2048, FIN_W2 = 2048, FIN_SMALL = 64 * 3 + 32 * 2;
constexpr int FIN_TOTAL = FIN_W1 + FIN_WS + FIN_W2 + FIN_SMALL;

__global__ __launch_bounds__(FIN_COLS * FIN_GROUPS) void bwd_finalize_kernel(
    const float *__restrict__ partW, int rowsW, double inv_r, float *__restrict__ g_w1,
    const float *__restrict__ partWs, int rowsS, float *__restrict__ g_ws,
    const float *__restrict__ partW2, int rows2, float *__restrict__ g_w2,
    const unsigned long long *__restrict__ accS, const double *__restrict__ sumsS,
    const unsigned long long *__restrict__ accT, const double *__restrict__ sumsT,
    float *__restrict__ g_bs, float *__restrict__ g_g2, float *__restrict__ g_b2, float *__restrict__ g_g1,
    float *__restrict__ g_b1) {
    __shared__ double red[FIN_GROUPS][FIN_COLS];
    critical_stream_priority();
    const int o = threadIdx.x % FIN_COLS, g = threadIdx.x / FIN_COLS;
    const int e = blockIdx.x * FIN_COLS + o;
    double v = 0.0;
    float *dst = nullptr;
    if (e < FIN_W1) {
        const int mid = e / 35, col = e % 35;
        dst = g_w1 + e;
        if (col < 3)
            v = (col_sum(partW, rowsW, 1216, mid * 38 + col, g) -
                 col_sum(partW, rowsW, 1216, mid * 38 + 3 + col, g)) * inv_r;
        else
            v = col_sum(partW, rowsW, 1216, mid * 38 + 3 + col, g);
    } else if (e < FIN_W1 + FIN_WS) {
        if (g_ws) { dst = g_ws + (e - FIN_W1); v = col_sum(partWs, rowsS, 2048, e - FIN_W1, g); }
    } else if (e < FIN_W1 + FIN_WS + FIN_W2) {
        if (g_w2) { dst = g_w2 + (e - FIN_W1 - FIN_WS); v = col_sum(partW2, rows2, 2048, e - FIN_W1 - FIN_WS, g); }
    } else if (e < FIN_TOTAL) {
        if (g == 0) {
            const int k = e - FIN_W1 - FIN_WS - FIN_W2;
            if (k < 192) {
                const int c = k & 63, which = k >> 6;
                const double scale = (sumsS && which) ? 1.0 / sumsS[129] : 1.0;
                if (which == 0) {
                    if (g_bs) { dst = g_bs + c; v = acc_read(accS, 128, c); }
                } else {
                    const int col = which == 1 ? c : 64 + c;
                    dst = which == 1 ? (g_b2 ? g_b2 + c : nullptr) : (g_g2 ? g_g2 + c : nullptr);
                    if (dst) v = (sumsS ? sumsS[col] : acc_read(accS, 128, col)) * scale;
                }
            } else {
                const int c = (k - 192) & 31, which = (k - 192) >> 5;
                const double scale = sumsT ? 1.0 / sumsT[65] : 1.0;
                dst = which == 0 ? (g_b1 ? g_b1 + c : nullptr) : (g_g1 ? g_g1 + c : nullptr);
                if (dst) v = (sumsT ? sumsT[32 * which + c] : acc_read(accT, 64, 32 * which + c)) * scale;
            }
        }
    }
    red[g][o] = v;
    __syncthreads();
    if (g == 0 && dst) {
        double acc = 0.0;
#pragma unroll
        for (int k = 0; k < FIN_GROUPS; ++k) acc += red[k][o];
        *dst = (float)acc;
    }
}

__global__ __launch_bounds__(128) void reduce_acc_kernel(const unsigned long long *__restrict__ acc, int ncol,
                                                         double count, double *__restrict__ out) {
    const int t = threadIdx.x;
    if (t < ncol) out[t] = acc_read(acc, ncol, t);
    if (t == 0) { out[ncol] = count; out[ncol + 1] = 1.0; }
}

}

#define APN_ST ((hipStream_t)stream)

extern "C" int apn_sa_reduce_rows(const float *part, int rows, int ncol, double count, double *out,
                                  void *stream) {
    if (rows < 0 || ncol < 4 || ncol > 128 || (1024 % ncol) || !part || !out) return APN_EINVAL;
    if ((uintptr_t)part & 15) return APN_EINVAL;
    hipLaunchKernelGGL(apn::reduce_rows_kernel, dim3(1), dim3(1024), 0, APN_ST, part, rows, ncol, count,
                       out);
    APN_LAUNCH_CHECK();
    return APN_OK;
}

extern "C" int apn_sa_reduce_acc(const void *acc, int ncol, double count, double *out, void *stream) {
    if (ncol < 1 || ncol > 128 || !acc || !out) return APN_EINVAL;
    hipLaunchKernelGGL(apn::reduce_acc_kernel, dim3(1), dim3(128), 0, APN_ST, (const unsigned long long *)acc, ncol,
                       count, out);
    APN_LAUNCH_CHECK();
    return APN_OK;
}

extern "C" int apn_sa_bn_fold(const float *part, int rows, const double *sums, int c, double count,
                              const float *gamma, const float *beta, float eps, float momentum,
                              float *running_mean, float *running_var, void *num_batches_tracked,
                              int training, float *pack, const float *sgn_gamma, int sgn_c,
                              float *sgn_out, void *stream) {
    if (c < 4 || c > 1024 || (c & 3) || !pack || sgn_c > 1024) return APN_EINVAL;
    if (training && !part && !sums) return APN_EINVAL;
    if (!training && (!running_mean || !running_var)) return APN_EINVAL;
    if (part && ((uintptr_t)part & 15)) return APN_EINVAL;
    hipLaunchKernelGGL(apn::bn_fold_kernel, dim3(c / 4), dim3(256), 0, APN_ST, part, rows, sums, c, count,
                       gamma, beta, eps, momentum, running_mean, running_var,
                       (long long *)num_batches_tracked, training, pack, sgn_gamma, sgn_c, sgn_out);
    APN_LAUNCH_CHECK();
    return APN_OK;
}

static int apn_sa_glue_tile(int b, int m) { return (long long)b * ((m + 63) / 64) <= 512 ? 32 : 64; }

extern "C" int apn_sa_fwd_out(int b, int n, int m, const float *ysel, const void *acc2, const double *sums2,
                              const float *g2, const float *b2, float *rm2, float *rv2, void *nbt2, float eps2,
                              float mom2, int train2, double count, float *pack2, const void *ft, int precision,
                              const int *fidx, const float *ws, const float *bs, int relu, float *out,
                              float *zero_base, long long zero_floats, void *stream) {
    if (b <= 0 || m <= 0 || b > 65535 || !ysel || !pack2 || !out) return APN_EINVAL;
    if (train2 && !acc2 && !sums2) return APN_EINVAL;
    if (!train2 && (!rm2 || !rv2)) return APN_EINVAL;
    if (ws && (!ft || !fidx || n <= 0 || (precision != 1 && precision != 2))) return APN_EINVAL;
    const __bf16 *hi = (const __bf16 *)ft;
    const __bf16 *lo = (ws && precision == 2) ? hi + (size_t)b * n * 32 : nullptr;
    if (zero_base && (zero_floats < 0 || (zero_floats & 3) || ((uintptr_t)zero_base & 15))) return APN_EINVAL;
    apn::BnArgs bn{g2, b2, rm2, rv2, (long long *)nbt2, eps2, mom2, train2, count};
    if (apn_sa_glue_tile(b, m) == 32)
        hipLaunchKernelGGL(apn::fwd_out_kernel<32>, dim3((m + 31) / 32, b), dim3(512), 0, APN_ST, n, m, ysel,
                           (const unsigned long long *)(sums2 ? nullptr : acc2), sums2, bn, pack2, hi, lo, fidx, ws, bs,
                           relu, out, (float4 *)zero_base, zero_base ? zero_floats / 4 : 0);
    else
        hipLaunchKernelGGL(apn::fwd_out_kernel<64>, dim3((m + 63) / 64, b), dim3(1024), 0, APN_ST, n, m, ysel,
                           (const unsigned long long *)(sums2 ? nullptr : acc2), sums2, bn, pack2, hi, lo, fidx, ws, bs,
                           relu, out, (float4 *)zero_base, zero_base ? zero_floats / 4 : 0);
    APN_LAUNCH_CHECK();
    return APN_OK;
}

extern "C" int apn_sa_bwd_prep_rows(int b, int m) {
    const int qt = apn_sa_glue_tile(b, m);
    return b * ((m + qt - 1) / qt);
}

extern "C" int apn_sa_bwd_prep(int b, int n, int m, const float *g_out, long long gs_b,
                               long long gs_c, long long gs_m, const float *out, int relu,
                               const float *ysel, const float *pack2, const void *ft, int precision,
                               const int *fidx, const float *ws, float *goa, void *accS,
                               float *partWs, float *gip, const int *dup, void *stream) {
    if (b <= 0 || m <= 0 || b > 65535 || !g_out || !ysel || !pack2 || !goa || !accS) return APN_EINVAL;
    if (relu && !out) return APN_EINVAL;
    if (ws && (!ft || !fidx || !partWs || !gip || n <= 0 || (precision != 1 && precision != 2)))
        return APN_EINVAL;
    const __bf16 *hi = (const __bf16 *)ft;
    const __bf16 *lo = (ws && precision == 2) ? hi + (size_t)b * n * 32 : nullptr;
    if (apn_sa_glue_tile(b, m) == 32)
        hipLaunchKernelGGL(apn::bwd_prep_kernel<32>, dim3((m + 31) / 32, b), dim3(512), 0, APN_ST, n, m, g_out,
                           gs_b, gs_c, gs_m, out, relu, ysel, pack2, hi, lo, fidx, ws, goa, (unsigned long long *)accS,
                           partWs, gip, dup);
    else
        hipLaunchKernelGGL(apn::bwd_prep_kernel<64>, dim3((m + 63) / 64, b), dim3(1024), 0, APN_ST, n, m, g_out,
                           gs_b, gs_c, gs_m, out, relu, ysel, pack2, hi, lo, fidx, ws, goa, (unsigned long long *)accS,
                           partWs, gip, dup);
    APN_LAUNCH_CHECK();
    return APN_OK;
}

#ifdef APN_WG_STAMPS
extern "C" __attribute__((visibility("default"))) int apn_sa_debug_wg_stamps(void *buf) {
    return (int)hipMemcpyToSymbol(HIP_SYMBOL(apn::d_wg_stamps), &buf, sizeof(buf));
}
#endif

extern "C" int apn_sa_bwd_weight_rows(int b, int n) { return b * ((n + apn::WG_PTS - 1) / apn::WG_PTS); }

extern "C" int apn_sa_bwd_point_grads(int b, int n, int m, const float *GU, const int *pcnt_poff, const void *geo,
                                      const float *HA, const float *HB, const void *accT, const double *sumsT,
                                      double count, int train1, const float *pack1, const void *ft, int precision,
                                      const float *xyz, const float *new_xyz, const float *w1,
                                      const float *gip, float radius, float *partW, float *g_f,
                                      float *g_p, float *g_newp, void *stream) {
    if (b <= 0 || n <= 0 || m <= 0 || b > 65535) return APN_EINVAL;
    if (!GU || !pcnt_poff || !geo || !HA || !HB || (!accT && !sumsT) || !pack1 || !ft || !xyz || !new_xyz || !w1 || !partW ||
        !g_f)
        return APN_EINVAL;
    if (precision != 1 && precision != 2) return APN_EINVAL;
    if (m > n) return APN_EINVAL;
    const __bf16 *hi = (const __bf16 *)ft;
    const __bf16 *lo = precision == 2 ? hi + (size_t)b * n * 32 : nullptr;
    hipLaunchKernelGGL(apn::bwd_point_grads_kernel, dim3((n + apn::WG_PTS - 1) / apn::WG_PTS, b),
                       dim3(apn::PG_NT), 0, APN_ST, n, b * m, precision == 2 ? 1 : 0, GU, pcnt_poff,
                       pcnt_poff + (size_t)b * n, (const long long *)geo, HA, HB,
                       (const unsigned long long *)accT, sumsT, count, train1,
                       pack1, hi, lo, xyz, new_xyz, w1, gip, 1.0f / radius, partW, g_f, g_p, g_newp);
    APN_LAUNCH_CHECK();
    return APN_OK;
}

extern "C" int apn_sa_bwd_finalize(const float *partW, int rows_w, float radius, float *g_w1,
                                   const float *partWs, int rows_s, float *g_ws, const float *partW2, int rows_2,
                                   float *g_w2, const void *accS, const double *sumsS,
                                   const void *accT, const double *sumsT, float *g_bs, float *g_g2, float *g_b2,
                                   float *g_g1, float *g_b1, void *stream) {
    if (!partW || !g_w1 || (g_ws && !partWs) || (g_w2 && !partW2) || !accS || (!accT && !sumsT))
        return APN_EINVAL;
    hipLaunchKernelGGL(apn::bwd_finalize_kernel, dim3((apn::FIN_TOTAL + apn::FIN_COLS - 1) / apn::FIN_COLS),
                       dim3(apn::FIN_COLS * apn::FIN_GROUPS), 0, APN_ST, partW,
                       rows_w, 1.0 / (double)radius, g_w1, partWs, rows_s, g_ws, partW2, rows_2, g_w2,
                       (const unsigned long long *)accS, sumsS, (const unsigned long long *)accT, sumsT, g_bs,
                       g_g2, g_b2, g_g1, g_b1);
    APN_LAUNCH_CHECK();
    return APN_OK;
}
```

adaptpoint_amd/csrc/sa_seq.hip:

```cpp
#include "apn_common.h"

#define APN_TRY(expr)            \
    do {                         \
        int rc__ = (expr);       \
        if (rc__) return rc__;   \
    } while (0)

namespace apn {
__global__ __launch_bounds__(256) void zero16_kernel(uint4 *__restrict__ p, long long n16) {
    const long long stride = (long long)gridDim.x * 256;
    for (long long e = (long long)blockIdx.x * 256 + threadIdx.x; e < n16; e += stride) p[e] = make_uint4(0, 0, 0, 0);
}
__global__ __launch_bounds__(256) void fill32_kernel(unsigned *__restrict__ p, unsigned word, long long n) {
    const long long stride = (long long)gridDim.x * 256;
    for (long long e = (long long)blockIdx.x * 256 + threadIdx.x; e < n; e += stride) p[e] = word;
}
}

extern "C" int apn_zero_fill(void *base, long long bytes, void *stream) {
    if (bytes < 0 || (bytes & 15) || (bytes && (!base || ((uintptr_t)base & 15)))) return APN_EINVAL;
    if (!bytes) return APN_OK;
    long long blocks = (bytes / 16 + 255) / 256;
    if (blocks > 1024) blocks = 1024;
    hipLaunchKernelGGL(apn::zero16_kernel, dim3((unsigned)blocks), dim3(256), 0, (hipStream_t)stream, (uint4 *)base,
                       bytes / 16);
    APN_LAUNCH_CHECK();
    return APN_OK;
}

extern "C" int apn_sa_forward_seq(
    int phases, int precision, int b, int n, int m, float radius, const float *xyz, const float *new_xyz,
    const float *f, const int *idx, const int *tmap, const int *fidx, const void *geo, const void *dd,
    const float *w1, const float *w2, const float *ws, const float *bs,
    const float *g1, const float *b1, float *rm1, float *rv1, void *nbt1, float eps1, float mom1,
    int train1,
    const float *g2, const float *b2, float *rm2, float *rv2, void *nbt2, float eps2, float mom2,
    int train2,
    double count, int relu, void *ft, float *part1, const double *sums1, const double *sums2,
    float *pack1, float *pack2, void *acc2, float *ysel, void *ksel,
    float *out, float *zero_base, long long zero_floats, void *stream) {
    if (phases & 1)
        APN_TRY(apn_sa_prep_stats(b, n, f, geo, dd, w1, precision, train1, ft, part1, acc2, apn_sa_acc_words(128),
                                  stream));
    if (phases & 2)
        APN_TRY(apn_sa_fwd_main(b, n, m, precision, radius, xyz, new_xyz, ft, idx, tmap, w1, w2, g1, b1, rm1, rv1,
                                nbt1, eps1, mom1, train1, count, part1, apn_sa_prep_rows(b, n), sums1, pack1, g2,
                                ysel, ksel, acc2, stream));
    if (phases & 4)
        APN_TRY(apn_sa_fwd_out(b, n, m, ysel, acc2, sums2, g2, b2, rm2, rv2, nbt2, eps2, mom2, train2, count, pack2,
                               ws ? ft : nullptr, precision, ws ? fidx : nullptr, ws, bs, relu, out, zero_base,
                               zero_floats, stream));
    return APN_OK;
}

extern "C" int apn_sa_backward_seq(
    int phases, int precision, int b, int n, int m, float radius, const float *xyz, const float *new_xyz,
    const int *idx, const int *tmap, const int *fidx, const void *geo, const float *w1, const float *w2,
    const float *ws, const void *ft, const float *pack1, const float *pack2, const float *ysel,
    const void *ksel, const float *out, int relu, int train1, int train2, double count,
    const float *g_out, long long gs_b, long long gs_c, long long gs_m,
    void *zero_base, long long zero_bytes, float *gip, void *accS, void *accT,
    const int *pcnt_poff, const int *rowdst, float *GU,
    float *goa, float *partWs, float *partW2, float *partW, const double *sumsS, const double *sumsT,
    float *HA, float *HB,
    float *g_f, float *g_p, float *g_newp, float *g_w1, float *g_w2, float *g_g1, float *g_b1, float *g_g2,
    float *g_b2, float *g_ws, float *g_bs, void *stream) {
    if (phases & 1) {
        if (zero_bytes) APN_TRY(apn_zero_fill(zero_base, zero_bytes, stream));
        APN_TRY(apn_sa_bwd_prep(b, n, m, g_out, gs_b, gs_c, gs_m, out, relu, ysel, pack2, ws ? ft : nullptr, precision,
                                ws ? fidx : nullptr, ws, goa, accS, partWs, gip,
                                pcnt_poff ? pcnt_poff + 2ll * b * n : nullptr, stream));
    }
    if (phases & 2)
        APN_TRY(apn_sa_bwd_main(b, n, m, precision, radius, xyz, new_xyz, ft, idx, tmap, w1, w2, pack1, pack2, accS,
                                sumsS, count, train2, goa, ksel, accT, partW2, rowdst, GU, HA, HB, stream));
    if (phases & 4) {
        APN_TRY(apn_sa_bwd_point_grads(b, n, m, GU, pcnt_poff, geo, HA, HB, accT, sumsT, count, train1, pack1, ft, precision, xyz,
                                       new_xyz, w1, gip, radius, partW, g_f, g_p, g_newp, stream));
        APN_TRY(apn_sa_bwd_finalize(partW, apn_sa_bwd_weight_rows(b, n), radius, g_w1, partWs,
                                    apn_sa_bwd_prep_rows(b, m), g_ws, partW2, apn_sa_bwd_main_rows(b, m), g_w2, accS,
                                    sumsS, accT, sumsT, g_bs, g_g2, g_b2, g_g1, g_b1, stream));
    }
    return APN_OK;
}

extern "C" int apn_sa_sample_seq_nested(int b, int n, int m, float radius, int nsample, const float *xyz,
                                        const int *tie_prev, int *tie_out, int *fidx, float *new_xyz, int *idx, void *geo,
                                        void *dd, void *stream) {
    if (b <= 0 || n <= 0 || m <= 0 || !tie_out) return APN_EINVAL;
    APN_TRY(apn_furthest_point_sampling_nested(b, n, m, xyz, tie_prev, fidx, new_xyz, tie_out, stream));
    APN_TRY(apn_ball_query_zero(b, n, m, radius, nsample, new_xyz, xyz, idx, stream));
    if (geo) APN_TRY(apn_sa_point_geo(b, n, m, nsample, radius, xyz, new_xyz, idx, geo, dd, stream));
    return APN_OK;
}

extern "C" int apn_sa_sample_seq(int b, int n, int m, float radius, int nsample, const float *xyz,
                                 float *temp, int *fidx, float *new_xyz, int *idx, void *geo, void *dd,
                                 void *stream) {
    if (b <= 0 || n <= 0 || m <= 0) return APN_EINVAL;
    if (temp) {
        long long blocks = ((long long)b * n + 255) / 256;
        if (blocks > 2048) blocks = 2048;
        hipLaunchKernelGGL(apn::fill32_kernel, dim3((unsigned)blocks), dim3(256), 0, (hipStream_t)stream, (unsigned *)temp,
                           0x501502F9u, (long long)b * n);
        APN_LAUNCH_CHECK();
    }
    APN_TRY(apn_furthest_point_sampling_xyz(b, n, m, xyz, temp, fidx, new_xyz, stream));
    APN_TRY(apn_ball_query_zero(b, n, m, radius, nsample, new_xyz, xyz, idx, stream));
    if (geo) APN_TRY(apn_sa_point_geo(b, n, m, nsample, radius, xyz, new_xyz, idx, geo, dd, stream));
    return APN_OK;
}
```

adaptpoint_amd/fused.py:

```python
import torch
import torch.distributed as dist
import torch.nn as nn

from . import _lib
from . import ops as _ops

C_IN, C_MID, C_OUT, K_NS = 32, 32, 64, 32
DETERMINISTIC = True

PRECISION = "bf16x3"
_PREC = {"bf16": 1, "bf16x3": 2}

PER_KERNEL_LAUNCH = False


def covers(B, N, M, K, C, w1, w2, biased=False, momenta=()):
    return (C == C_IN and K == K_NS and tuple(w1) == (C_MID, C_IN + 3) and tuple(w2) == (C_OUT, C_MID) and not biased
            and (M is None or M <= N) and B <= 65535 and all(m is not None for m in momenta))


def supported(p, f, idx_or_k, conv1, conv2, bns=(), npoint=None):
    k = idx_or_k.shape[2] if torch.is_tensor(idx_or_k) else int(idx_or_k)
    m = idx_or_k.shape[1] if torch.is_tensor(idx_or_k) else npoint
    return (f.is_cuda and f.dtype == torch.float32 and p.dtype == torch.float32
            and covers(p.shape[0], p.shape[1], m, k, f.shape[1], conv1.weight.shape[:2], conv2.weight.shape[:2],
                       conv1.bias is not None or conv2.bias is not None, [bn.momentum for bn in bns]))


_FN = {}


def _call(name, dev, *args, stream=None):
    fn = _FN.get(name)
    if fn is None:
        fn = _FN[name] = getattr(_lib.load(), name)
    if stream is None:
        if dev.index is not None and dev.index != torch.cuda.current_device():
            with torch.cuda.device(dev):
                code = fn(*args, torch.cuda.current_stream(dev).cuda_stream)
            if code:
                _lib.check(code, name)
            return
        stream = torch.cuda.current_stream(dev).cuda_stream
    code = fn(*args, stream)
    if code:
        _lib.check(code, name)


class _Launcher:

    def __init__(self, dev):
        self.dev = dev
        if dev.index is not None and dev.index != torch.cuda.current_device():
            self.stream = None
        else:
            self.stream = torch.cuda.current_stream(dev).cuda_stream

    def __call__(self, name, *args):
        _call(name, self.dev, *args, stream=self.stream)


def _ptr(t):
    return None if t is None else t.data_ptr()


FORCE_PHASED = False


def _world(sync):
    if sync and dist.is_available() and dist.is_initialized():
        return dist.get_world_size()
    return 1


def _allreduce_sum_(t):
    if dist.is_available() and dist.is_initialized() and (dist.get_world_size() > 1 or FORCE_PHASED):
        from . import dp
        dp.all_reduce_sum_(t)


def _phased(sync):
    return _world(sync) > 1 or (FORCE_PHASED and sync)


def _carve(dev, sizes, zero=False):
    offs, total = [], 0
    for _, nfl in sizes:
        offs.append(total)
        total += (int(nfl) + 63) // 64 * 64
    buf = (torch.zeros if zero else torch.empty)(max(total, 64), dtype=torch.float32, device=dev)
    return {name: buf[o:o + int(nfl)] for (name, nfl), o in zip(sizes, offs)}, buf


def _all_reduce_rows(call, part, rows, ncol, count, dev):
    sums = torch.empty(ncol + 2, dtype=torch.float64, device=dev)
    call("apn_sa_reduce_rows", part.data_ptr(), rows, ncol, float(count), sums.data_ptr())
    _allreduce_sum_(sums)
    return sums


def _all_reduce_acc(call, acc, ncol, count, dev):
    sums = torch.empty(ncol + 2, dtype=torch.float64, device=dev)
    call("apn_sa_reduce_acc", acc.data_ptr(), ncol, float(count), sums.data_ptr())
    _allreduce_sum_(sums)
    return sums


def _bn_args(bn):
    training = bn.training or not bn.track_running_stats
    track = bn.track_running_stats
    if bn.momentum is None:
        raise RuntimeError("fused set abstraction: BatchNorm(momentum=None) is not covered "
                           "(fused.supported() routes it to the unfused path)")
    mom = bn.momentum
    return (_ptr(bn.weight), _ptr(bn.bias), _ptr(bn.running_mean) if track else None,
            _ptr(bn.running_var) if track else None,
            _ptr(bn.num_batches_tracked) if (track and bn.training) else None,
            float(bn.eps), float(mom), 1 if training else 0)


def _mat(w, rows, cols):
    w = w.detach().reshape(rows, cols)
    return w if w.is_contiguous() else w.contiguous()


def _acc_floats(ncol):
    return 2 * _lib.load().apn_sa_acc_words(ncol)


class _Forward:

    def __init__(self, p, f, new_p, idx, fidx, radius, conv1, bn1, conv2, bn2, skip_conv, relu,
                 sync_bn, tmap=None, geo=None, dd=None, want_backward=False, rowmap=None):
        dev = f.device
        call = _Launcher(dev)
        lib = _lib.load()
        B, C, N = f.shape
        M = new_p.shape[1]
        self.dims = (B, N, M)
        self.radius = float(radius)
        self.sync = sync_bn
        self.relu = 1 if relu else 0
        self.prec = prec = _PREC[PRECISION]
        w1 = _mat(conv1.weight, C_MID, C_IN + 3)
        w2 = _mat(conv2.weight, C_OUT, C_MID)
        ws = bs = None
        if skip_conv is not None:
            ws = _mat(skip_conv.weight, C_OUT, C_IN)
            bs = skip_conv.bias.detach() if skip_conv.bias is not None else None
        count = float(B * M * K_NS)
        if geo is None:
            geo, dd = point_geo(p, new_p, idx, radius)
        if want_backward:
            from . import fused_wide
            if tmap is None:
                tmap = fused_wide.tile_map(idx)
                rowmap = None
            if rowmap is None:
                rowmap = fused_wide.row_map(tmap, B, N, M, fidx=fidx)
        rows1 = lib.apn_sa_prep_rows(B, N)
        v, _buf = _carve(dev, [("ft", prec * B * N * C // 2), ("pack1", 4 * C_MID), ("pack2", 4 * C_OUT),
                               ("ysel", B * M * C_OUT), ("ksel", B * M * C_OUT // 4),
                               ("part1", rows1 * 64), ("acc2", _acc_floats(128))])
        out = torch.empty(B, C_OUT, M, dtype=torch.float32, device=dev)
        self.zsizes = (([("gip", B * N * C_MID)] if ws is not None else [])
                       + [("accS", _acc_floats(128)), ("accT", _acc_floats(64))])
        self.zviews = self.zbuf = None
        if want_backward:
            self.zviews, self.zbuf = _carve(dev, self.zsizes)
        zptr, zfl = _ptr(self.zbuf), (self.zbuf.numel() if self.zbuf is not None else 0)
        bn1a, bn2a = _bn_args(bn1), _bn_args(bn2)
        self.train1, self.train2 = bool(bn1a[7]), bool(bn2a[7])

        def run(phases, sums1=None, sums2=None):
            if PER_KERNEL_LAUNCH:
                return _forward_per_kernel(call, phases, prec, B, N, M, self.radius, p, new_p, f, idx, fidx, geo, dd,
                                           w1, w2, ws, bs, bn1a, bn2a, count, self.relu, v, sums1,
                                           sums2, out, rows1, tmap, zptr, zfl)
            call("apn_sa_forward_seq", phases, prec, B, N, M, self.radius, p.data_ptr(), new_p.data_ptr(),
                 f.data_ptr(), idx.data_ptr(), _ptr(tmap), _ptr(fidx), geo.data_ptr(), dd.data_ptr(),
                 w1.data_ptr(), w2.data_ptr(), _ptr(ws), _ptr(bs), *bn1a, *bn2a, count, self.relu,
                 v["ft"].data_ptr(), v["part1"].data_ptr(), _ptr(sums1), _ptr(sums2),
                 v["pack1"].data_ptr(), v["pack2"].data_ptr(), v["acc2"].data_ptr(),
                 v["ysel"].data_ptr(), v["ksel"].data_ptr(), out.data_ptr(), zptr, zfl)

        if not _phased(sync_bn):
            run(7)
        else:
            run(1)
            s1 = _all_reduce_rows(call, v["part1"], rows1, 64, count, dev) if self.train1 else None
            run(2, sums1=s1)
            s2 = _all_reduce_acc(call, v["acc2"], 128, count, dev) if self.train2 else None
            run(4, sums2=s2)
        self.out = out
        self.saved = dict(p=p, f=f, new_p=new_p, idx=idx, tmap=tmap, rowmap=rowmap, fidx=fidx,
                          geo=geo, ft=v["ft"], w1=w1, w2=w2, ws=ws,
                          has_bs=bs is not None, pack1=v["pack1"], pack2=v["pack2"], ysel=v["ysel"],
                          ksel=v["ksel"], count=count)


def _backward(fw, g_out, need_p, need_newp):
    if fw is None:
        raise RuntimeError("fused set abstraction: backward called a second time (its saved state is "
                           "released after the first backward; retain_graph is not supported)")
    sv = fw.saved
    B, N, M = fw.dims
    dev = fw.out.device
    P, sync = sv["count"], fw.sync
    f32 = dict(dtype=torch.float32, device=dev)
    if g_out is None:
        g_out = torch.zeros_like(fw.out)
    if g_out.dtype != torch.float32:
        g_out = g_out.float()
    gs = g_out.stride()
    w1, w2, ws = sv["w1"], sv["w2"], sv["ws"]
    has_skip = ws is not None
    lib = _lib.load()
    call = _Launcher(dev)
    rows = lib.apn_sa_bwd_main_rows(B, M)
    prow = lib.apn_sa_bwd_prep_rows(B, M)
    wrows = lib.apn_sa_bwd_weight_rows(B, N)

    prezeroed = fw.zbuf is not None
    zsizes = [] if prezeroed else fw.zsizes
    if sv["rowmap"] is None:
        raise RuntimeError("fused set abstraction: backward without a row map (the forward was run with want_backward=False)")
    pcnt_poff, rowdst = sv["rowmap"]
    sizes = zsizes + [("goa", B * M * C_OUT), ("partWs", prow * C_OUT * C_IN if has_skip else 0),
                      ("partW2", rows * C_OUT * C_MID), ("partW", wrows * 32 * 38),
                      ("HA", B * M * C_MID), ("HB", B * M * C_MID), ("GU", lib.apn_sa_rowmap_places(B, N, M) * C_MID)]
    v, buf = _carve(dev, sizes)
    zero_floats = sum((nfl + 63) // 64 * 64 for _, nfl in zsizes)
    if prezeroed:
        v.update(fw.zviews)
        fw.zbuf = fw.zviews = None
    gsz = [("w2", C_OUT * C_MID), ("w1", C_MID * (C_IN + 3)), ("g1", C_MID), ("b1", C_MID),
           ("g2", C_OUT), ("b2", C_OUT), ("ws", C_OUT * C_IN if has_skip else 0),
           ("bs", C_OUT if (has_skip and sv["has_bs"]) else 0)]
    g, _gbuf = _carve(dev, gsz)
    g_f = torch.empty(B, C_IN, N, **f32)
    g_p = _ops.zeros(B, N, 3, **f32) if need_p else None
    g_newp = torch.empty(B, M, 3, **f32) if need_newp else None
    gws = g["ws"].data_ptr() if has_skip else None
    gbs = g["bs"].data_ptr() if (has_skip and sv["has_bs"]) else None

    def run(phases, sumsS=None, sumsT=None):
        if PER_KERNEL_LAUNCH:
            return _backward_per_kernel(call, phases, fw, sv, g_out, buf, zero_floats, v, g, sumsS,
                                        sumsT, g_f, g_p, g_newp, rows, prow, wrows, has_skip, pcnt_poff, rowdst)
        call("apn_sa_backward_seq", phases, fw.prec, B, N, M, fw.radius, sv["p"].data_ptr(),
             sv["new_p"].data_ptr(), sv["idx"].data_ptr(), _ptr(sv["tmap"]), _ptr(sv["fidx"]), sv["geo"].data_ptr(),
             w1.data_ptr(), w2.data_ptr(), _ptr(ws), sv["ft"].data_ptr(), sv["pack1"].data_ptr(),
             sv["pack2"].data_ptr(), sv["ysel"].data_ptr(), sv["ksel"].data_ptr(),
             fw.out.data_ptr(), fw.relu, 1 if fw.train1 else 0, 1 if fw.train2 else 0, float(P),
             g_out.data_ptr(), gs[0], gs[1], gs[2], buf.data_ptr(), zero_floats * 4,
             v["gip"].data_ptr() if has_skip else None, v["accS"].data_ptr(),
             v["accT"].data_ptr(), pcnt_poff.data_ptr(), rowdst.data_ptr(), v["GU"].data_ptr(), v["goa"].data_ptr(),
             v["partWs"].data_ptr() if has_skip else None, v["partW2"].data_ptr(), v["partW"].data_ptr(),
             _ptr(sumsS), _ptr(sumsT), v["HA"].data_ptr(), v["HB"].data_ptr(),
             g_f.data_ptr(), _ptr(g_p), _ptr(g_newp), g["w1"].data_ptr(), g["w2"].data_ptr(),
             g["g1"].data_ptr(), g["b1"].data_ptr(), g["g2"].data_ptr(), g["b2"].data_ptr(), gws, gbs)

    if not _phased(sync):
        run(7)
    else:
        run(1)
        sS = _all_reduce_acc(call, v["accS"], 128, P, dev)
        run(2, sumsS=sS)
        sT = _all_reduce_acc(call, v["accT"], 64, P, dev)
        run(4, sumsS=sS, sumsT=sT)
    return dict(f=g_f, p=g_p, new_p=g_newp, w1=g["w1"].view(C_MID, C_IN + 3, 1, 1),
                w2=g["w2"].view(C_OUT, C_MID, 1, 1), g1=g["g1"], b1=g["b1"], g2=g["g2"], b2=g["b2"],
                ws=g["ws"].view(C_OUT, C_IN, 1) if has_skip else None,
                bs=g["bs"] if (has_skip and sv["has_bs"]) else None)


def _forward_per_kernel(call, phases, prec, B, N, M, radius, p, new_p, f, idx, fidx, geo, dd, w1, w2, ws, bs,
                        bn1a, bn2a, count, relu, v, sums1, sums2, out, rows1, tmap=None, zptr=None, zfl=0):
    lib = _lib.load()
    if phases & 1:
        call("apn_sa_prep_stats", B, N, f.data_ptr(), geo.data_ptr(), dd.data_ptr(), w1.data_ptr(), prec,
             bn1a[7], v["ft"].data_ptr(), v["part1"].data_ptr(), v["acc2"].data_ptr(), lib.apn_sa_acc_words(128))
    if phases & 2:
        call("apn_sa_fwd_main", B, N, M, prec, radius, p.data_ptr(), new_p.data_ptr(), v["ft"].data_ptr(),
             idx.data_ptr(), _ptr(tmap), w1.data_ptr(), w2.data_ptr(), *bn1a, count, v["part1"].data_ptr(), rows1,
             _ptr(sums1), v["pack1"].data_ptr(), bn2a[0], v["ysel"].data_ptr(), v["ksel"].data_ptr(),
             v["acc2"].data_ptr())
    if phases & 4:
        call("apn_sa_fwd_out", B, N, M, v["ysel"].data_ptr(), v["acc2"].data_ptr(), _ptr(sums2), *bn2a, count,
             v["pack2"].data_ptr(), v["ft"].data_ptr() if ws is not None else None, prec,
             _ptr(fidx) if ws is not None else None, _ptr(ws), _ptr(bs), relu, out.data_ptr(), zptr, zfl)


def _backward_per_kernel(call, phases, fw, sv, g_out, buf, zero_floats, v, g, sumsS, sumsT, g_f, g_p,
                         g_newp, rows, prow, wrows, has_skip, pcnt_poff, rowdst):
    B, N, M = fw.dims
    w1, w2, ws, P = sv["w1"], sv["w2"], sv["ws"], float(sv["count"])
    gip = v["gip"].data_ptr() if has_skip else None
    if phases & 1:
        if zero_floats:
            call("apn_zero_fill", buf.data_ptr(), zero_floats * 4)
        call("apn_sa_bwd_prep", B, N, M, g_out.data_ptr(), *g_out.stride(), fw.out.data_ptr(), fw.relu,
             sv["ysel"].data_ptr(), sv["pack2"].data_ptr(), sv["ft"].data_ptr() if has_skip else None,
             fw.prec, _ptr(sv["fidx"]) if has_skip else None, _ptr(ws), v["goa"].data_ptr(),
             v["accS"].data_ptr(), v["partWs"].data_ptr() if has_skip else None, gip,
             pcnt_poff.data_ptr() + 8 * B * N)
    if phases & 2:
        call("apn_sa_bwd_main", B, N, M, fw.prec, fw.radius, sv["p"].data_ptr(), sv["new_p"].data_ptr(),
             sv["ft"].data_ptr(), sv["idx"].data_ptr(), _ptr(sv["tmap"]), w1.data_ptr(), w2.data_ptr(),
             sv["pack1"].data_ptr(), sv["pack2"].data_ptr(), v["accS"].data_ptr(), _ptr(sumsS), P,
             1 if fw.train2 else 0, v["goa"].data_ptr(), sv["ksel"].data_ptr(), v["accT"].data_ptr(),
             v["partW2"].data_ptr(), rowdst.data_ptr(), v["GU"].data_ptr(), v["HA"].data_ptr(), v["HB"].data_ptr())
    if phases & 4:
        call("apn_sa_bwd_point_grads", B, N, M, v["GU"].data_ptr(), pcnt_poff.data_ptr(), sv["geo"].data_ptr(),
             v["HA"].data_ptr(), v["HB"].data_ptr(), v["accT"].data_ptr(), _ptr(sumsT), P, 1 if fw.train1 else 0,
             sv["pack1"].data_ptr(), sv["ft"].data_ptr(), fw.prec, sv["p"].data_ptr(), sv["new_p"].data_ptr(),
             w1.data_ptr(), gip, fw.radius, v["partW"].data_ptr(), g_f.data_ptr(), _ptr(g_p), _ptr(g_newp))
        call("apn_sa_bwd_finalize", v["partW"].data_ptr(), wrows, fw.radius, g["w1"].data_ptr(),
             v["partWs"].data_ptr() if has_skip else None, prow, g["ws"].data_ptr() if has_skip else None,
             v["partW2"].data_ptr(), rows, g["w2"].data_ptr(), v["accS"].data_ptr(), _ptr(sumsS),
             v["accT"].data_ptr(), _ptr(sumsT), g["bs"].data_ptr() if (has_skip and sv["has_bs"]) else None,
             g["g2"].data_ptr(), g["b2"].data_ptr(), g["g1"].data_ptr(), g["b1"].data_ptr())


class _GroupedMlpMax(torch.autograd.Function):
    @staticmethod
    def forward(ctx, p, new_p, f, idx, w1, g1, b1, w2, g2, b2, mods):
        radius, conv1, bn1, conv2, bn2, sync_bn = mods
        fw = _Forward(p.contiguous(), f.contiguous(), new_p.contiguous(), idx.contiguous(), None,
                      radius, conv1, bn1, conv2, bn2, None, False, sync_bn, want_backward=any(ctx.needs_input_grad))
        ctx.fw = fw
        ctx.save_for_backward(p, new_p, f, idx)
        ctx.set_materialize_grads(False)
        ctx.flags = (p.requires_grad, new_p.requires_grad,
                     g1 is not None, b1 is not None, g2 is not None, b2 is not None)
        return fw.out

    @staticmethod
    def backward(ctx, g_out):
        need_p, need_q, a1, a2, a3, a4 = ctx.flags
        ctx.saved_tensors
        g = _backward(ctx.fw, g_out, need_p, need_q)
        ctx.fw = None
        return (g["p"], g["new_p"], g["f"], None, g["w1"], g["g1"] if a1 else None,
                g["b1"] if a2 else None, g["w2"], g["g2"] if a3 else None,
                g["b2"] if a4 else None, None)


def grouped_mlp_max(p, new_p, f, idx, radius, conv1, bn1, conv2, bn2, sync_bn=False):
    return _GroupedMlpMax.apply(p, new_p, f, idx, conv1.weight, bn1.weight, bn1.bias,
                                conv2.weight, bn2.weight, bn2.bias,
                                (radius, conv1, bn1, conv2, bn2, sync_bn))


class Sampling:

    def __init__(self, B, M, K, device):
        self.shape = (B, M, K)
        self.buf = torch.empty(B * M * (1 + 3 + K), dtype=torch.int32, device=device)
        o = 0
        self.fidx = self.buf[o:o + B * M].view(B, M)
        o += B * M
        self.new_p = self.buf[o:o + B * M * 3].view(torch.float32).view(B, M, 3)
        o += B * M * 3
        self.idx = self.buf[o:o + B * M * K].view(B, M, K)
        self.index = None
        self.tmap = None
        self.rowmap = None
        self.geo = None
        self.dd = None
        self.ready = None
        self.ties = None

    def alloc_geo(self, n_points):
        if self.geo is None or self.geo.shape[1] != n_points:
            B = self.shape[0]
            dev = self.buf.device
            self.geo = torch.empty(B, n_points, 4, dtype=torch.int64, device=dev)
            self.dd = torch.empty(B, _lib.load().apn_sa_geo_dd_doubles(n_points), dtype=torch.float64, device=dev)
        return self.geo, self.dd

    def clouds(self, lo, hi):
        v = object.__new__(Sampling)
        for name, t in vars(self).items():
            setattr(v, name, t[lo:hi] if name in _PER_CLOUD and t is not None else None)
        v.shape = (hi - lo,) + self.shape[1:]
        return v


_PER_CLOUD = ("fidx", "new_p", "idx", "geo", "dd", "ties")


@torch.no_grad()
def point_geo(p, new_p, idx, radius, out=None):
    B, N, _ = p.shape
    M, K = idx.shape[1], idx.shape[2]
    dev = p.device
    if out is None:
        geo = torch.empty(B, N, 4, dtype=torch.int64, device=dev)
        dd = torch.empty(B, _lib.load().apn_sa_geo_dd_doubles(N), dtype=torch.float64, device=dev)
    else:
        geo, dd = out
    _Launcher(dev)("apn_sa_point_geo", B, N, M, K, float(radius), p.contiguous().data_ptr(),
                   new_p.contiguous().data_ptr(), idx.contiguous().data_ptr(), geo.data_ptr(), dd.data_ptr())
    return geo, dd


@torch.no_grad()
def sample_and_query(p, npoint, radius, nsample=K_NS, out=None, geo=False, nested=False, ties=None):
    p = p.contiguous()
    dev = p.device
    B, N, _ = p.shape
    smp = out if out is not None else Sampling(B, npoint, nsample, dev)
    assert smp.shape == (B, npoint, nsample)
    gptr = dptr = None
    if geo and nsample == K_NS and smp.buf is not None:
        g_, d_ = smp.alloc_geo(N)
        gptr, dptr = g_.data_ptr(), d_.data_ptr()
    elif geo and nsample == K_NS and smp.geo is not None:
        gptr, dptr = smp.geo.data_ptr(), smp.dd.data_ptr()
    call = _Launcher(dev)
    if nested and N <= 4096:
        if smp.ties is None:
            smp.ties = torch.empty(B, dtype=torch.int32, device=dev)
        if PER_KERNEL_LAUNCH:
            call("apn_furthest_point_sampling_nested", B, N, npoint, p.data_ptr(), _ptr(ties), smp.fidx.data_ptr(),
                 smp.new_p.data_ptr(), smp.ties.data_ptr())
            call("apn_ball_query_zero", B, N, npoint, float(radius), nsample, smp.new_p.data_ptr(), p.data_ptr(),
                 smp.idx.data_ptr())
            if gptr is not None:
                call("apn_sa_point_geo", B, N, npoint, nsample, float(radius), p.data_ptr(), smp.new_p.data_ptr(),
                     smp.idx.data_ptr(), gptr, dptr)
            return smp
        call("apn_sa_sample_seq_nested", B, N, npoint, float(radius), nsample, p.data_ptr(), _ptr(ties), smp.ties.data_ptr(),
             smp.fidx.data_ptr(), smp.new_p.data_ptr(), smp.idx.data_ptr(), gptr, dptr)
        return smp
    if PER_KERNEL_LAUNCH:
        call("apn_furthest_point_sampling_xyz", B, N, npoint, p.data_ptr(), None,
             smp.fidx.data_ptr(), smp.new_p.data_ptr())
        call("apn_ball_query_zero", B, N, npoint, float(radius), nsample, smp.new_p.data_ptr(),
             p.data_ptr(), smp.idx.data_ptr())
        if gptr is not None:
            call("apn_sa_point_geo", B, N, npoint, nsample, float(radius), p.data_ptr(),
                 smp.new_p.data_ptr(), smp.idx.data_ptr(), gptr, dptr)
        return smp
    call("apn_sa_sample_seq", B, N, npoint, float(radius), nsample, p.data_ptr(), None,
         smp.fidx.data_ptr(), smp.new_p.data_ptr(), smp.idx.data_ptr(), gptr, dptr)
    return smp


@torch.no_grad()
def sample_and_query_many(ps, npoint, radius, nsample=K_NS, outs=None):
    ps = [p.contiguous() for p in ps]
    B, N, _ = ps[0].shape
    dev = ps[0].device
    if outs is None:
        outs = [Sampling(B, npoint, nsample, dev) for _ in ps]
    assert len(outs) == len(ps) and all(o.shape == (B, npoint, nsample) for o in outs)
    call = _Launcher(dev)
    for i in range(len(ps) + 1):
        a = i if i < len(ps) else None
        b = i - 1 if i >= 1 else None
        call("apn_sa_sample_overlap", B, N, npoint, float(radius), nsample,
             ps[a].data_ptr() if a is not None else None,
             outs[a].fidx.data_ptr() if a is not None else None,
             outs[a].new_p.data_ptr() if a is not None else None,
             ps[b].data_ptr() if b is not None else None,
             outs[b].new_p.data_ptr() if b is not None else None,
             outs[b].idx.data_ptr() if b is not None else None)
        if b is not None and outs[b].geo is not None:
            point_geo(ps[b], outs[b].new_p, outs[b].idx, radius, out=(outs[b].geo, outs[b].dd))
    return outs


class _SetAbstraction(torch.autograd.Function):
    @staticmethod
    def forward(ctx, p, f, w1, g1, b1, w2, g2, b2, ws, bs, mods):
        npoint, radius, conv1, bn1, conv2, bn2, skip_conv, relu, sync_bn, sampling = mods
        p = p.contiguous()
        f = f.contiguous()
        smp = sampling if sampling is not None else sample_and_query(p, npoint, radius, geo=True)
        fidx, new_p, idx = smp.fidx, smp.new_p, smp.idx
        if p.requires_grad:
            new_p = new_p.clone()
        fw = _Forward(p, f, new_p, idx, fidx, radius, conv1, bn1, conv2, bn2, skip_conv, relu,
                      sync_bn, tmap=smp.tmap, geo=smp.geo, dd=smp.dd, want_backward=any(ctx.needs_input_grad),
                      rowmap=smp.rowmap)
        ctx.fw = fw
        ctx.save_for_backward(p, f)
        ctx.set_materialize_grads(False)
        ctx.flags = (p.requires_grad, g1 is not None, b1 is not None, g2 is not None,
                     b2 is not None, ws is not None, bs is not None)
        ctx.mark_non_differentiable(new_p) if not p.requires_grad else None
        return new_p, fw.out

    @staticmethod
    def backward(ctx, g_newp_in, g_out):
        need_p, a1, a2, a3, a4, a5, a6 = ctx.flags
        fw = ctx.fw
        ctx.saved_tensors
        g = _backward(fw, g_out, need_p, need_p)
        g_p = g["p"]
        if need_p:
            gq = g["new_p"] if g_newp_in is None else g["new_p"] + g_newp_in
            g_p = g_p.scatter_add(1, fw.saved["fidx"].long().unsqueeze(-1).expand(-1, -1, 3), gq)
        ctx.fw = None
        return (g_p, g["f"], g["w1"], g["g1"] if a1 else None, g["b1"] if a2 else None, g["w2"],
                g["g2"] if a3 else None, g["b2"] if a4 else None, g["ws"] if a5 else None,
                g["bs"] if a6 else None, None)


def fused_set_abstraction(p, f, npoint, radius, conv1, bn1, conv2, bn2, skip_conv=None, relu=True,
                          sync_bn=False, sampling=None):
    assert skip_conv is None or isinstance(skip_conv, nn.Conv1d)
    ws = skip_conv.weight if skip_conv is not None else None
    bs = skip_conv.bias if skip_conv is not None else None
    return _SetAbstraction.apply(p, f, conv1.weight, bn1.weight, bn1.bias, conv2.weight, bn2.weight,
                                 bn2.bias, ws, bs,
                                 (npoint, radius, conv1, bn1, conv2, bn2, skip_conv, relu, sync_bn,
                                  sampling))
```

include/adaptpoint_amd.h:

```cpp
#ifndef ADAPTPOINT_AMD_H
#define ADAPTPOINT_AMD_H

#include <stddef.h>

#ifdef __cplusplus
extern "C" {
#endif

#define APN_OK 0
#define APN_EINVAL (-1)

#if defined(__GNUC__)
#define APN_API __attribute__((visibility("default")))
#else
#define APN_API
#endif

APN_API int apn_version(void);

APN_API const char *apn_error_string(int code);

APN_API const char *apn_build_flags(void);

APN_API int apn_furthest_point_sampling(int b, int n, int m, const float *xyz, float *temp,
                                int *idxs, void *stream);

APN_API int apn_ball_query(int b, int n, int m, float radius, int nsample, const float *new_xyz,
                   const float *xyz, int *idx, void *stream);

APN_API int apn_group_points(int b, int c, int n, int npoints, int nsample, const float *points,
                     const int *idx, float *out, void *stream);

APN_API int apn_group_points_grad(int b, int c, int n, int npoints, int nsample,
                          const float *grad_out, const int *idx, float *grad_points,
                          void *stream);

APN_API int apn_gather_points(int b, int c, int n, int npoints, const float *points,
                      const int *idx, float *out, void *stream);

APN_API int apn_gather_points_grad(int b, int c, int n, int npoints, const float *grad_out,
                           const int *idx, float *grad_points, void *stream);

APN_API int apn_resample_points(int b, int n, int c, int p_all, int s_cnt, int cx,
                                const float *points, const int *fidx, const int *choice,
                                float *pos, float *x, void *stream);

APN_API int apn_three_nn(int b, int n, int m, const float *unknown, const float *known,
                 float *dist2, int *idx, void *stream);

APN_API int apn_three_interpolate(int b, int c, int m, int n, const float *points, const int *idx,
                          const float *weight, float *out, void *stream);

APN_API int apn_three_interpolate_grad(int b, int c, int n, int m, const float *grad_out,
                               const int *idx, const float *weight, float *grad_points,
                               void *stream);


APN_API int apn_furthest_point_sampling_xyz(int b, int n, int m, const float *xyz, float *temp,
                                            int *idxs, float *new_xyz, void *stream);

APN_API int apn_ball_query_zero(int b, int n, int m, float radius, int nsample,
                                const float *new_xyz, const float *xyz, int *idx, void *stream);

APN_API int apn_sa_grid_blocks(int b, int m);
APN_API int apn_sa_grid_rows(int b, int m, int with_tile_map);
APN_API int apn_sa_bwd_main_rows(int b, int m);
APN_API int apn_sa_acc_words(int ncol);
APN_API int apn_zero_fill(void *base, long long bytes, void *stream);
APN_API int apn_debug_stamp(void *stamps, int slot, void *stream);
APN_API int apn_debug_vgpr_hold(int blocks, int turns, unsigned long long *bad, void *stream);
APN_API int apn_debug_vpk_probe(int blocks, int turns, int form, unsigned long long *bad, void *stream);


APN_API int apn_sa_geo_dd_doubles(int n);
APN_API int apn_sa_point_geo(int b, int n, int m, int nsample, float radius, const float *xyz,
                             const float *new_xyz, const int *idx, void *geo, void *dd, void *stream);

APN_API int apn_sa_prep_rows(int b, int n);
APN_API int apn_sa_prep_stats(int b, int n, const float *f, const void *geo, const void *dd, const float *w1,
                              int precision, int stats, void *ft, float *part1, void *zero, long long zero_words,
                              void *stream);

APN_API int apn_sa_reduce_rows(const float *part, int rows, int ncol, double count, double *out,
                               void *stream);
APN_API int apn_sa_reduce_acc(const void *acc, int ncol, double count, double *out, void *stream);

APN_API int apn_sa_bn_fold(const float *part, int rows, const double *sums, int c, double count,
                           const float *gamma, const float *beta, float eps, float momentum,
                           float *running_mean, float *running_var, void *num_batches_tracked,
                           int training, float *pack, const float *sgn_gamma, int sgn_c,
                           float *sgn_out, void *stream);

APN_API int apn_sa_fwd_main(int b, int n, int m, int precision, float radius, const float *xyz,
                            const float *new_xyz, const void *ft, const int *idx, const int *tmap, const float *w1,
                            const float *w2, const float *g1, const float *b1, float *rm1, float *rv1, void *nbt1,
                            float eps1, float mom1, int train1, double count, const float *part1, int rows1,
                            const double *sums1, float *pack1, const float *gamma2, float *ysel, void *ksel,
                            void *acc2, void *stream);

APN_API int apn_sa_fwd_out(int b, int n, int m, const float *ysel, const void *acc2, const double *sums2,
                           const float *g2, const float *b2, float *rm2, float *rv2, void *nbt2, float eps2,
                           float mom2, int train2, double count, float *pack2, const void *ft, int precision,
                           const int *fidx, const float *ws, const float *bs, int relu, float *out,
                           float *zero_base, long long zero_floats, void *stream);

APN_API int apn_sa_bwd_prep_rows(int b, int m);
APN_API int apn_sa_bwd_prep(int b, int n, int m, const float *g_out, long long gs_b,
                            long long gs_c, long long gs_m, const float *out, int relu,
                            const float *ysel, const float *pack2, const void *ft, int precision,
                            const int *fidx, const float *ws, float *goa, void *accS,
                            float *partWs, float *gip, const int *dup, void *stream);

APN_API int apn_sa_bwd_main(int b, int n, int m, int precision, float radius, const float *xyz,
                            const float *new_xyz, const void *ft, const int *idx, const int *tmap, const float *w1,
                            const float *w2, const float *pack1, const float *pack2, const void *accS,
                            const double *sumsS, double count, int train2, const float *goa, const void *ksel,
                            void *accT, float *partW2, const int *rowdst, float *GU, float *HA, float *HB,
                            void *stream);

APN_API int apn_sa_bwd_weight_rows(int b, int n);
APN_API int apn_sa_bwd_point_grads(int b, int n, int m, const float *GU, const int *pcnt_poff, const void *geo,
                                   const float *HA, const float *HB, const void *accT, const double *sumsT,
                                   double count, int train1, const float *pack1, const void *ft, int precision,
                                   const float *xyz, const float *new_xyz, const float *w1,
                                   const float *gip, float radius, float *partW, float *g_f,
                                   float *g_p, float *g_newp, void *stream);

APN_API int apn_sa_bwd_finalize(const float *partW, int rows_w, float radius, float *g_w1,
                                const float *partWs, int rows_s, float *g_ws, const float *partW2, int rows_2,
                                float *g_w2, const void *accS, const double *sumsS,
                                const void *accT, const double *sumsT, float *g_bs, float *g_g2, float *g_b2,
                                float *g_g1, float *g_b1, void *stream);

APN_API int apn_sa_debug_stamps(void *buf);

APN_API int apn_sa_forward_seq(
    int phases, int precision, int b, int n, int m, float radius, const float *xyz, const float *new_xyz,
    const float *f, const int *idx, const int *tmap, const int *fidx, const void *geo, const void *dd,
    const float *w1, const float *w2, const float *ws, const float *bs,
    const float *g1, const float *b1, float *rm1, float *rv1, void *nbt1, float eps1, float mom1,
    int train1,
    const float *g2, const float *b2, float *rm2, float *rv2, void *nbt2, float eps2, float mom2,
    int train2,
    double count, int relu, void *ft, float *part1, const double *sums1, const double *sums2,
    float *pack1, float *pack2, void *acc2, float *ysel, void *ksel,
    float *out, float *zero_base, long long zero_floats, void *stream);
APN_API int apn_sa_backward_seq(
    int phases, int precision, int b, int n, int m, float radius, const float *xyz, const float *new_xyz,
    const int *idx, const int *tmap, const int *fidx, const void *geo, const float *w1, const float *w2,
    const float *ws, const void *ft, const float *pack1, const float *pack2, const float *ysel,
    const void *ksel, const float *out, int relu, int train1, int train2, double count,
    const float *g_out, long long gs_b, long long gs_c, long long gs_m,
    void *zero_base, long long zero_bytes, float *gip, void *accS, void *accT,
    const int *pcnt_poff, const int *rowdst, float *GU,
    float *goa, float *partWs, float *partW2, float *partW, const double *sumsS, const double *sumsT,
    float *HA, float *HB,
    float *g_f, float *g_p, float *g_newp, float *g_w1, float *g_w2, float *g_g1, float *g_b1, float *g_g2,
    float *g_b2, float *g_ws, float *g_bs, void *stream);
APN_API int apn_sa_sample_overlap(int b, int n, int m, float radius, int nsample,
                                  const float *xyz_a, int *fidx_a, float *new_xyz_a,
                                  const float *xyz_b, const float *new_xyz_b, int *idx_b,
                                  void *stream);
APN_API int apn_furthest_point_sampling_nested(int b, int n, int m, const float *xyz, const int *tie_prev, int *idxs,
                                               float *new_xyz, int *tie_out, void *stream);
APN_API int apn_sa_sample_seq_nested(int b, int n, int m, float radius, int nsample, const float *xyz,
                                     const int *tie_prev, int *tie_out, int *fidx, float *new_xyz, int *idx, void *geo,
                                     void *dd, void *stream);
APN_API int apn_sa_sample_seq(int b, int n, int m, float radius, int nsample, const float *xyz,
                              float *temp, int *fidx, float *new_xyz, int *idx, void *geo, void *dd,
                              void *stream);

APN_API int apn_pointset_group_rows(int b, int m, int c);
APN_API int apn_pointset_group_max(int b, int n, int m, int c, int k, const float *points,
                                   const int *idx, const int *fidx, const float *alpha,
                                   const float *beta, float *out, void *ksel, void *stream);
APN_API int apn_pointset_group_max_grad(int b, int n, int m, int c, int k, const float *points,
                                        const int *idx, const int *fidx, const float *alpha,
                                        const void *ksel, const float *g_out, float *g_points,
                                        float *part, void *stream);

APN_API int apn_attention_small_max(void);
APN_API int apn_attention_small_fwd(int b, int m, int heads, const float *q, const float *k, const float *v,
                                    float *out, void *stream);
APN_API int apn_attention_small_bwd(int b, int m, int heads, const float *q, const float *k, const float *v,
                                    const float *g_out, float *dq, float *dk, float *dv, void *stream);
APN_API int apn_attention_prep(int b, int m, int heads, const float *q, const float *k,
                               const float *v, void *images, int for_backward, void *stream);
APN_API int apn_attention_fwd(int b, int m, int heads, const void *images, float *out, float *lse,
                              void *stream);
APN_API int apn_attention_bwd(int b, int m, int heads, const void *images, const float *out,
                              const float *lse, const float *g_out, void *scratch, float *dq,
                              float *dk, float *dv, void *stream);

APN_API int apn_token_attention_max_tokens(void);
APN_API int apn_token_attention_fwd(int b, int t, int heads, const float *qkv, float *out, float *lse, void *stream);
APN_API int apn_token_attention_bwd(int b, int t, int heads, const float *qkv, const float *out, const float *lse,
                                    const float *g_out, float *delta, float *dqkv, void *stream);

APN_API int apn_sa_wide_grid(int b, int m);
APN_API int apn_sa_wide_tilemap_ints(int b, int m);
APN_API int apn_sa_wide_tilemap(int b, int m, int mode, const int *idx, int *tmap, void *stream);
APN_API int apn_sa_wide_tilemap_many(int count, int b, int m, int mode, const int *idx, int *tmap, void *stream);
APN_API int apn_sa_rowmap_places(int b, int n, int m);
APN_API int apn_sa_rowmap_ints(int b, int n);
APN_API int apn_sa_rowmap_many(int count, int b, int n, int m, const int *tmap, const int *fidx, int *pcnt_poff, int *rowdst, int *scratch,
                               void *stream);
APN_API int apn_sa_wide_colsum_chunks(int rows, int ncol);
APN_API int apn_sa_wide_colsum(const float *part, int rows, int ncol, double *scratch, double *out,
                               void *stream);
APN_API int apn_sa_wide_stats1(int b, int n, int m, int c_mid, const float *U, const float *V,
                               const int *idx, const int *tmap, float *part, void *stream);
APN_API int apn_sa_wide_fwd_main(int b, int n, int m, int c_mid, int c_out, const float *U, const float *V,
                                 const int *idx, const int *tmap, const void *w2_image, const float *pack1,
                                 const float *sgn2, float *ysel, void *ksel, float *part, void *stream);
APN_API int apn_sa_wide_bwd_main(int b, int n, int m, int c_mid, int c_out, const float *U, const float *V,
                                 const int *idx, const int *tmap, const void *z_image, const float *pack1,
                                 const float *evec, const float *goa, const void *ksel, float *GU,
                                 float *HA, float *HB, float *part, float *r_part, void *stream);
APN_API int apn_sa_wide_wgrad_fused(int c_mid);
APN_API int apn_sa_wide_image(const float *src0, int k0, int trans0, const float *src1, int kd, int nc, int ct,
                              void *image, void *stream);
APN_API int apn_sa_wide_bwd_prep_rows(int b, int m);
APN_API int apn_sa_wide_bwd_prep(int b, int m, int c_out, const float *g, long long gs_b, long long gs_c,
                                 long long gs_m, const float *ysel, const float *pack2, const float *out_act,
                                 float *gpre, float *goa, float *part_s, void *stream);
APN_API int apn_sa_wide_consts2(const float *part_s, int rows, const double *sums, int c_out,
                                const float *pack2, double count, int training, float *d2e2,
                                float *g_gamma2, float *g_beta2, void *stream);
APN_API int apn_sa_wide_consts1(const float *part_t, int rows, const double *sums, int c_mid,
                                const float *pack1, double count, int training, float *cabc,
                                float *g_gamma1, float *g_beta1, void *stream);
APN_API int apn_sa_wide_point_terms(int b, int n, int m, int c_mid, const float *cabc, const float *pack1,
                                    const float *U, const float *geo, const float *w1, int ldw, float radius,
                                    const float *GU, const int *pcnt_poff, const int *plist, float *G, float *HA,
                                    const float *HB, void *stream);
APN_API int apn_sa_wide_wgrad_splits(int b, int m, int c_mid);
APN_API int apn_sa_wide_wgrad(int b, int n, int m, int c_mid, int c_out, const float *U, const float *V,
                              const int *idx, const int *tmap, const float *pack1, const float *goa,
                              const void *ksel, int splits, float *r_part, void *stream);

APN_API int apn_sa_wide_csr(int b, int n, int m, const int *idx, const float *new_xyz, const int *tmap,
                            int *pcnt_poff, int *plist, float *geo, const int *fidx, int *fq, void *stream);
APN_API int apn_sa_wide_fwd_prep(int b, int c_in, int n, int m, int c_mid, int c_out, float radius, const float *f,
                                 const float *p, const float *new_p, const float *w1, const float *w2, float *U,
                                 float *V, void *w2_image, const int *fq, float *fs, const float *geo, float *part1,
                                 void *stream);
APN_API int apn_sa_wide_fwd_prep_rows(int b, int n, int m);
APN_API int apn_sa_wide_out(int b, int m, int c_out, const float *ysel, const float *pack2, int c_in,
                            const float *fs, const float *ws, const float *bs, int relu, float *out, void *stream);
APN_API int apn_sa_wide_bwd_mid(const float *part_s, int rows, const double *sums, int c_mid, int c_out,
                                const float *pack2, double count, int training, const float *w2, float *d2e2,
                                float *g_gamma2, float *g_beta2, float *evec, void *z_image, void *stream);
APN_API int apn_sa_wide_bwd_fin(const float *part_t, int rows, const double *sums, int c_mid, int c_out,
                                const float *pack1, double count, int training, float *cabc, float *g_gamma1,
                                float *g_beta1, const double *R, const float *d2e2, const float *w2, float *g_w2,
                                void *stream);
APN_API int apn_sa_wide_point_grads_rows(int b, int n);
APN_API int apn_sa_wide_point_grads(int b, int c_in, int n, int m, int c_mid, float radius, const float *GU,
                                    const int *pcnt_poff, const int *plist, const float *geo, const float *U,
                                    const float *f, const float *p, const float *new_p, const float *HA,
                                    const float *HB, const float *cabc, const float *pack1, const float *w1,
                                    int c_skip, const float *gpre, const int *fq, const float *fs, const float *ws,
                                    float *g_f, float *g_p, float *g_q, float *w_part, void *stream);
APN_API int apn_sa_wide_point_grads_cols(int c_in, int c_mid, int c_skip);
APN_API int apn_sa_wide_colsum_f32(const float *part, int rows, int ncol, float *out, void *stream);

APN_API int apn_pw_conv_tiles(int b, int n);
APN_API int apn_pw_conv_forward(int b, int c_in, int c_out, int n, int precision, const float *x, const float *w,
                                float *y, float *part, void *stream);
APN_API int apn_pw_bn_act(int b, int c, int n, const float *y, const float *part, int tiles, const float *gamma,
                          const float *beta, float eps, float momentum, int training, int relu, float *run_mean,
                          float *run_var, long long *batches, float *stat, float *out, void *stream);
APN_API int apn_pw_bn_act_grad_splits(int b, int c);
APN_API int apn_pw_bn_act_grad(int b, int c, int n, const float *g, const float *y, const float *stat, int training,
                               int relu, float *part_b, float *gy, float *g_gamma, float *g_beta, void *stream);
APN_API int apn_pw_conv_grad_input(int b, int c_in, int c_out, int n, int precision, const float *gy, const float *w,
                                   float *gx, void *stream);
APN_API int apn_pw_conv_grad_weight_splits(int b, int c_in, int c_out, int n);
APN_API int apn_pw_conv_grad_weight(int b, int c_in, int c_out, int n, int precision, const float *gy, const float *x,
                                    float *scratch, float *gw, void *stream);

APN_API int apn_pw_contract_splits(int nbatch, int r, int q, int k);
APN_API int apn_pw_contract(int nbatch, int r, int q, int k, const float *a, long long a_batch, int lda, int a_kcont,
                            const float *b, long long b_batch, int ldb, int b_kcont, float *d, long long d_batch, int ldd,
                            int splits, float *scratch, int precision, void *stream);
APN_API int apn_pw_contract2_splits(int which, int nbatch0, int r0, int q0, int k0, int nbatch1, int r1, int q1, int k1);
APN_API int apn_pw_contract2(int a_kcont, int b_kcont, int precision, const int *nbatch, const int *r, const int *q,
                             const int *k, const float *const *a, const long long *a_batch, const int *lda,
                             const float *const *b, const long long *b_batch, const int *ldb, float *const *d,
                             const long long *d_batch, const int *ldd, const int *splits, float *const *scratch,
                             void *stream);

APN_API int apn_fp_blend_stats(int b, int o, int m, int n, const float *a, const float *u, const int *idx,
                               const float *weight, float *y, float *part, int training, const float *gamma,
                               const float *beta, const float *run_mean, const float *run_var, float eps, int relu,
                               float *stat, float *out, void *stream);

APN_API int apn_pw_transpose(int nbatch, int r, int c, const float *in, float *out, void *stream);
APN_API int apn_three_nn_weights(long long n, const float *dist2, float *weight, void *stream);

APN_API int apn_anchor_transforms(int n, const float *prob, const float *keep, const float *axes, float r_range,
                                  float s_range, float t_range, float *lin, float *off, void *stream);
APN_API int apn_anchor_transforms_grad(int n, const float *prob, const float *keep, const float *axes, float r_range,
                                       float s_range, float t_range, const float *g_lin, const float *g_off,
                                       float *g_prob, void *stream);

APN_API int apn_deform_forward(int b, int n, int m, const float *xyz, const float *anchors, const float *lin,
                               const float *off, const float *axes, const float *mask, float sigma, float *z, float *stat,
                               float *out, void *stream);
APN_API int apn_deform_backward(int b, int n, int m, const float *xyz, const float *anchors, const float *axes,
                                const float *mask, float sigma, const float *z, const float *stat, const float *g_out,
                                float *g_lin, float *g_off, float *g_mask, void *stream);

APN_API int apn_pointwolf_params(int b, int m, const float *draws, int uniform, float r_range, float s_range,
                                 float t_range, float *lin, float *off, float *kaxes, void *stream);

APN_API int apn_rsmix_select(int b, int n, int c, const float *points, const int *draws, double r2, int knn_k,
                             int nsample, int *members, int *counts, void *stream);
APN_API int apn_rsmix_mix(int b, int n, int c, int nsample, const float *points, const int *draws, const int *members,
                          const int *counts, const int *pick, float *out, float *lam, void *stream);

#define APN_CT_PERMUTE 1
#define APN_CT_SCALE 2
#define APN_CT_HEIGHTS_SCALED 4
#define APN_CT_CENTER 8
#define APN_CT_NORMALIZE 16
#define APN_CT_ROTATE 32
#define APN_CT_UNIFORM 64
#define APN_CT_ANISOTROPIC 128
#define APN_CT_MIRROR 256
APN_API int apn_cloud_transform(int b, int n, int n_raw, int s, const float *raw, const int *rows, int flags,
                                int gravity_dim, const double *cfg, const int *perm, const float *params,
                                const float *uniforms, int *perm_out, float *params_out, float *out, void *stream);

APN_API int apn_cls_confusion(int b, int k, const float *logits, int ld, const int *target, const int *valid,
                              unsigned long long *cm, int *pred, void *stream);

APN_API int apn_pw_conv_max_tiles(int n);
APN_API int apn_pw_conv_max_forward(int b, int c_in, int c_out, int n, int precision, const float *x, const float *w,
                                    const float *bias, int relu, float *tile_val, int *tile_idx, float *out, int *idx,
                                    void *stream);
APN_API int apn_pw_conv_max_backward(int b, int c_in, int c_out, int n, const float *g_out, const float *out,
                                     const int *idx, const float *x, const float *w, int relu, float *xsel, float *g_x,
                                     float *g_w, float *g_bias, void *stream);

APN_API int apn_spectral_norm_blocks(int rows, int cols);
APN_API int apn_spectral_norm(int rows, int cols, const float *w, int training, float eps, float *u, float *v,
                              float *scratch, float *u_used, float *v_used, float *sigma, float *w_normalized,
                              void *stream);
APN_API int apn_spectral_norm_grad(int rows, int cols, const float *g, const float *w_normalized, const float *sigma,
                                   const float *u_used, const float *v_used, double *part, float *g_w, void *stream);

APN_API int apn_spectral_norm_many(int n_layers, const int *rows, const int *cols, const float *const *w, int training,
                                   float eps, float *const *u, float *const *v, float *const *scratch,
                                   float *const *u_used, float *const *v_used, float *const *sigma,
                                   float *const *w_normalized, void *stream);
APN_API int apn_spectral_norm_grad_many(int n_layers, const int *rows, const int *cols, const float *const *g,
                                        const float *const *w_normalized, const float *const *sigma,
                                        const float *const *u_used, const float *const *v_used, double *const *part,
                                        float *const *g_w, void *stream);

APN_API int apn_la_pool_rows(int b, int n);
APN_API int apn_la_pool_fwd(int b, int n, int c, int nsample, float radius, const float *U, const float *xyz,
                            const float *wp, int ldw, const int *idx, const float *gamma, float *ext, void *sel,
                            float *ysum, double *part, void *stream);
APN_API int apn_la_stats_fold(const double *part, int rows, int c, double count, double *sums, void *stream);
APN_API int apn_la_pool_bwd(int b, int n, int c, int nsample, float radius, const float *gsel, const void *sel,
                            const int *tmap, const int *pcnt_poff, const int *plist, const float *geo, const float *U,
                            const float *xyz, const float *ysum, const float *de, const float *wp, int ldw, float *dU,
                            float *dT, float *dp, void *stream);

APN_API int apn_knn_query(int b, int n, int m, int c, int k, const float *support, const float *query, int *idx,
                          float *dist2, void *stream);

APN_API int apn_knn_dilated(int b, int n, int m, int c, int kd, int k, int dilation, const int *slots,
                            const float *support, const float *query, int *idx, float *dist2, void *stream);

APN_API int apn_ec_pool_rows(int b, int n);
APN_API int apn_ec_pool_fwd(int b, int n, int c, int k, const float *uv, int ld, const int *idx, const float *gamma,
                            float *ext, void *sel, float *ysum, double *part, void *stream);
APN_API int apn_ec_out(int b, int n, int c, const float *ext, const float *pack, float slope, float *out, void *stream);
APN_API int apn_ec_bwd_prep_rows(int b, int n);
APN_API int apn_ec_bwd_prep(int b, int n, int c, const float *g, long long gs_b, long long gs_c, long long gs_n,
                            const float *ext, const float *pack, float slope, float *gsel, float *part_s, void *stream);
APN_API int apn_ec_out_res(int b, int n, int c, const float *ext, const float *pack, float slope, const float *res,
                           long long rs_b, long long rs_c, long long rs_n, float *out, void *stream);
APN_API int apn_ec_bwd_prep_act(int b, int n, int c, const float *g, long long gs_b, long long gs_c, long long gs_n,
                                const float *ext, const float *pack, float slope, float *gsel, float *part_s,
                                void *stream);
APN_API int apn_ec_csr(int b, int n, int k, const int *idx, int *pcnt_poff, int *plist, int *scratch, void *stream);
APN_API int apn_ec_pool_bwd(int b, int n, int c, int k, const float *gsel, const void *sel, const int *pcnt_poff,
                            const int *plist, const float *uv, int ld, const float *ysum, const float *de, float *duv,
                            void *stream);

APN_API int apn_chamfer_max_points(void);
APN_API int apn_chamfer_forward(int b, int n, int m, const float *xyz1, const float *xyz2, float *dist1, float *dist2,
                                int *idx1, int *idx2, void *stream);
APN_API int apn_chamfer_backward(int b, int n, int m, const float *xyz1, const float *xyz2, const int *idx1,
                                 const int *idx2, const float *grad_dist1, const float *grad_dist2, float *grad_xyz1,
                                 float *grad_xyz2, void *stream);

APN_API int apn_emd_max_points(void);
APN_API int apn_emd_one_launch_max(void);
APN_API int apn_emd_cost_parts(int n);
APN_API int apn_emd_ratios(int b, int n, int m, const float *xyz1, const float *xyz2, float *ratio_l, float *ratio_r,
                           float *state, void *stream);
APN_API int apn_emd_match(int b, int n, int m, const float *xyz1, const float *xyz2, const float *ratio_l,
                          const float *ratio_r, float *match, void *stream);
APN_API int apn_emd_cost(int b, int n, int m, const float *xyz1, const float *xyz2, const float *match,
                         const float *ratio_l, const float *ratio_r, float *part, float *cost, void *stream);
APN_API int apn_emd_cost_grad(int b, int n, int m, const float *grad_cost, const float *xyz1, const float *xyz2,
                              const float *match, const float *ratio_l, const float *ratio_r, float *grad1, float *grad2,
                              void *stream);

APN_API int apn_po_knn_query(int b, int n, int m, int k, const float *xyz, const float *new_xyz, const int *offset,
                             const int *new_offset, int *idx, float *dist2, void *stream);
APN_API int apn_po_ball_query(int b, int n, int m, float radius, int nsample, const float *xyz, const float *new_xyz,
                              const int *offset, const int *new_offset, int *idx, void *stream);
APN_API int apn_po_furthest_sampling(int b, int n_max, const float *xyz, const int *offset, const int *new_offset,
                                     float *tmp, int *idx, void *stream);
APN_API int apn_po_csr(int n, int m, int k, const int *idx, int *pcnt_poff, int *plist, int *scratch, void *stream);
APN_API int apn_po_grouping_fwd(int n, int m, int k, int c, const float *input, const int *idx, float *out, void *stream);
APN_API int apn_po_grouping_bwd(int n, int m, int k, int c, const float *grad_out, const int *pcnt_poff, const int *plist,
                                float *grad_input, void *stream);
APN_API int apn_po_interpolation_fwd(int n, int m, int k, int c, const float *input, const int *idx, const float *weight,
                                     float *out, void *stream);
APN_API int apn_po_interpolation_bwd(int n, int m, int k, int c, const float *grad_out, const float *weight,
                                     const int *pcnt_poff, const int *plist, float *grad_input, void *stream);
APN_API int apn_po_subtraction_fwd(int n, int m, int k, int c, const float *input1, const float *input2, const int *idx,
                                   float *out, void *stream);
APN_API int apn_po_subtraction_bwd(int n, int m, int k, int c, const float *grad_out, const int *pcnt_poff,
                                   const int *plist, float *grad_input1, float *grad_input2, void *stream);
APN_API int apn_po_aggregation_fwd(int n, int m, int k, int c, int w_c, const float *input, const float *position,
                                   const float *weight, const int *idx, float *out, void *stream);
APN_API int apn_po_aggregation_bwd(int n, int m, int k, int c, int w_c, const float *input, const float *position,
                                   const float *weight, const int *idx, const float *grad_out, const int *pcnt_poff,
                                   const int *plist, float *grad_input, float *grad_position, float *grad_weight,
                                   void *stream);

APN_API int apn_pt_rows(int n, int k, int c);
APN_API int apn_pt_mid_rows(int n, int k, int c);
APN_API int apn_pt_rel_stats(int n, int k, int c, const float *qkv, int ld, const float *h, const int *idx,
                             const float *wts, double *part, void *stream);
APN_API int apn_pt_fold(const double *part, int rows, int width, double *sums, void *stream);
APN_API int apn_pt_colsum_rows(int n);
APN_API int apn_pt_colsum(int n, int width, const float *src, int ld, double *part, void *stream);
APN_API int apn_pt_mid(int n, int k, int c, const float *qkv, int ld, const float *h, const int *idx, const float *wts,
                       const float *bn, float *t, double *part, void *stream);
APN_API int apn_pt_attend(int n, int k, int c, const float *qkv, int ld, const float *h, const int *idx,
                          const float *wts, const float *bn, const float *t, float *a, float *out, void *stream);
APN_API int apn_pt_attend_bwd(int n, int k, int c, const float *qkv, int ld, const float *h, const int *idx,
                              const float *wts, const float *bn, const float *t, const float *a, const float *go,
                              float *g1, double *part, void *stream);
APN_API int apn_pt_mid_bwd(int n, int k, int c, const float *qkv, int ld, const float *h, const int *idx,
                           const float *wts, const float *bn, const float *de, const float *t, const float *g1,
                           double *part, void *stream);
APN_API int apn_pt_rel_bwd(int n, int k, int c, const float *qkv, int ld, const float *h, const int *idx,
                           const float *wts, const float *bn, const float *de, const float *t, const float *g1,
                           const float *a, const float *go, float *dr, float *dh, float *dqkv, int ldg, double *part,
                           void *stream);
APN_API int apn_pt_scatter_bwd(int n, int k, int c, const float *dr, const float *go, const float *a,
// ... 58 lines not shown
```

Measured before the change: 122,700.

## Hoist skip-connection rows and identity GEMM into extra prep-kernel workgroups

Adds extra workgroups to the prep-stats kernel that gather the sampled input rows into a compact row-major buffer (fq). When skip weights are present, they also precompute the skip linear projection (ident) with MFMA. The forward output kernel then adds the precomputed identity instead of staging operands and doing the skip GEMM. The backward prep kernel reads the compact rows instead of strided gathers from ft. This moves skip work off the critical tail and onto otherwise idle CUs, at the cost of extra global buffers and writes.

```diff
diff --git a/adaptpoint_amd/_lib.py b/adaptpoint_amd/_lib.py
--- a/adaptpoint_amd/_lib.py
+++ b/adaptpoint_amd/_lib.py
@@ -42,6 +42,8 @@
     "apn_sa_point_geo": [_c_int] * 4 + [_c_float] + [_c_void_p] * 6,
     "apn_sa_prep_rows": [_c_int] * 2,
     "apn_sa_prep_stats": [_c_int] * 2 + [_c_void_p] * 4 + [_c_int] * 2 + [_c_void_p] * 3 + [_c_longlong, _c_void_p],
+    "apn_sa_prep_stats_skip": [_c_int] * 3 + [_c_void_p] * 4 + [_c_int] * 2 + [_c_void_p] * 3 + [_c_longlong]
+                              + [_c_void_p] * 6,
     "apn_sa_reduce_rows": [_c_void_p, _c_int, _c_int, _c_double, _c_void_p, _c_void_p],
     "apn_sa_reduce_acc": [_c_void_p, _c_int, _c_double, _c_void_p, _c_void_p],
     "apn_sa_bn_fold": [_c_void_p, _c_int, _c_void_p, _c_int, _c_double, _c_void_p, _c_void_p,
@@ -50,10 +52,10 @@
     "apn_sa_fwd_main": [_c_int] * 4 + [_c_float] + [_c_void_p] * 12 + [_c_float, _c_float, _c_int, _c_double,
                                                                         _c_void_p, _c_int] + [_c_void_p] * 7,
     "apn_sa_fwd_out": [_c_int] * 3 + [_c_void_p] * 8 + [_c_float, _c_float, _c_int, _c_double] + [_c_void_p] * 2
-                      + [_c_int] + [_c_void_p] * 3 + [_c_int] + [_c_void_p] * 2 + [_c_longlong, _c_void_p],
+                      + [_c_int] + [_c_void_p] * 3 + [_c_int] + [_c_void_p] * 2 + [_c_longlong] + [_c_void_p] * 3,
     "apn_sa_bwd_prep_rows": [_c_int] * 2,
     "apn_sa_bwd_prep": [_c_int] * 3 + [_c_void_p] + [_c_longlong] * 3 + [_c_void_p] + [_c_int]
-                       + [_c_void_p] * 3 + [_c_int] + [_c_void_p] * 8,
+                       + [_c_void_p] * 3 + [_c_int] + [_c_void_p] * 9,
     "apn_sa_bwd_main": [_c_int] * 4 + [_c_float] + [_c_void_p] * 11 + [_c_double, _c_int] + [_c_void_p] * 9,
     "apn_sa_bwd_weight_rows": [_c_int] * 2,
     "apn_sa_bwd_point_grads": [_c_int] * 3 + [_c_void_p] * 7 + [_c_double, _c_int] + [_c_void_p] * 2 + [_c_int]
@@ -63,11 +65,11 @@
     "apn_sa_forward_seq": ([_c_int] * 5 + [_c_float] + [_c_void_p] * 12
                            + [_c_void_p] * 5 + [_c_float, _c_float, _c_int]
                            + [_c_void_p] * 5 + [_c_float, _c_float, _c_int]
-                           + [_c_double, _c_int] + [_c_void_p] * 11 + [_c_longlong, _c_void_p]),
+                           + [_c_double, _c_int] + [_c_void_p] * 11 + [_c_longlong] + [_c_void_p] * 3),
     "apn_sa_backward_seq": ([_c_int] * 5 + [_c_float] + [_c_void_p] * 15 + [_c_int] * 3
                             + [_c_double] + [_c_void_p] + [_c_longlong] * 3 + [_c_void_p]
                             + [_c_longlong]
-                            + [_c_void_p] * 26),
+                            + [_c_void_p] * 27),
     "apn_attention_small_max": [],
     "apn_attention_small_fwd": [_c_int] * 3 + [_c_void_p] * 5,
     "apn_attention_small_bwd": [_c_int] * 3 + [_c_void_p] * 8,
diff --git a/adaptpoint_amd/csrc/sa_fused.hip b/adaptpoint_amd/csrc/sa_fused.hip
--- a/adaptpoint_amd/csrc/sa_fused.hip
+++ b/adaptpoint_amd/csrc/sa_fused.hip
@@ -94,11 +94,91 @@
 __device__ __forceinline__ void wg_stamp(int) {}
 #endif
 
+constexpr int SR_MAX_ROWS = 192;
+
+template <int NS>
+__device__ __forceinline__ void skip_rows_role(int role, int roles, int by_xcd, int b, int n, int m, const float *__restrict__ f,
+                                               const int *__restrict__ fidx, const float *__restrict__ ws,
+                                               const float *__restrict__ bs, float *__restrict__ fq,
+                                               float *__restrict__ ident) {
+    const int tid = threadIdx.x, lane = tid & 63, r = lane & 31, h = lane >> 5;
+    const int wave = __builtin_amdgcn_readfirstlane(tid >> 6);
+    const int tpc = (m + 31) / 32;
+    int c0 = 0, cstep = 1, slot = role, slots = roles, total = b * tpc;
+    if (by_xcd) {
+        const int x = (int)blockIdx.x & 7;
+        c0 = x; cstep = 8; slot = role >> 3; slots = roles >> 3;
+        total = x < b ? ((b - x + 7) / 8) * tpc : 0;
+    }
+    if (slot + slots * wave >= total) return;
+    Frag<2> wa[2][2];
+    float bv[2][16];
+    if (ident) {
+#pragma unroll
+        for (int cb = 0; cb < 2; ++cb) {
+#pragma unroll
+            for (int st = 0; st < 2; ++st) {
+                float av[8];
+                const float4 a0 = *reinterpret_cast<const float4 *>(ws + (32 * cb + r) * 32 + 16 * st + 8 * h);
+                const float4 a1 = *reinterpret_cast<const float4 *>(ws + (32 * cb + r) * 32 + 16 * st + 8 * h + 4);
+                av[0] = a0.x; av[1] = a0.y; av[2] = a0.z; av[3] = a0.w; av[4] = a1.x; av[5] = a1.y; av[6] = a1.z; av[7] = a1.w;
+                wa[cb][st] = make_frag<2>(av);
+            }
+#pragma unroll
+            for (int e = 0; e < 16; ++e) bv[cb][e] = bs ? bs[32 * cb + acc_row(e, h)] : 0.0f;
+        }
+    }
+    for (int t = slot + slots * wave; t < total; t += slots * (PS_NT / 64)) {
+        const int cloud = c0 + cstep * (t / tpc), q = (t % tpc) * 32 + r;
+        const bool in = q < m;
+        const size_t row = (size_t)cloud * m + (in ? q : m - 1);
+        const int src = fidx[row];
+        wg_stamp(1);
+        float x[2][8];
+#pragma unroll
+        for (int st = 0; st < 2; ++st)
+#pragma unroll
+            for (int j = 0; j < 8; ++j) x[st][j] = f[((size_t)cloud * SA_C + 16 * st + 8 * h + j) * n + src];
+        wg_stamp(2);
+        float4 *frow = reinterpret_cast<float4 *>(fq + row * SA_C);
+#pragma unroll
+        for (int st = 0; st < 2; ++st) {
+            const Frag<NS> a = make_frag<NS>(x[st]);
+#pragma unroll
+            for (int j = 0; j < 8; ++j) x[st][j] = (float)a.p[0][j] + (NS == 2 ? (float)a.p[NS - 1][j] : 0.0f);
+            if (in) {
+                frow[4 * st + 2 * h] = make_float4(x[st][0], x[st][1], x[st][2], x[st][3]);
+                frow[4 * st + 2 * h + 1] = make_float4(x[st][4], x[st][5], x[st][6], x[st][7]);
+            }
+        }
+        wg_stamp(3);
+        if (ident) {
+            const Frag<2> b0 = make_frag<2>(x[0]), b1 = make_frag<2>(x[1]);
+            float4 *irow = reinterpret_cast<float4 *>(ident + row * SA_C2);
+#pragma unroll
+            for (int cb = 0; cb < 2; ++cb) {
+                f32x16 acc = {0};
+                acc = mfma<2>(wa[cb][0], b0, acc);
+                acc = mfma<2>(wa[cb][1], b1, acc);
+                if (in) {
+#pragma unroll
+                    for (int g = 0; g < 4; ++g)
+                        irow[8 * cb + 2 * g + h] = make_float4(acc[4 * g] + bv[cb][4 * g], acc[4 * g + 1] + bv[cb][4 * g + 1],
+                                                               acc[4 * g + 2] + bv[cb][4 * g + 2], acc[4 * g + 3] + bv[cb][4 * g + 3]);
+                }
+            }
+        }
+        wg_stamp(4);
+    }
+}
+
 template <int NS>
 __global__ __launch_bounds__(PS_NT) void sa_prep_stats_kernel(
     int n, int tiles_per_cloud, int total_tiles, const float *__restrict__ f, const long long *__restrict__ geo,
     const double *__restrict__ dd, int dd_rows, const float *__restrict__ w1, int stats, __bf16 *__restrict__ ft,
-    __bf16 *__restrict__ ft_lo, float *__restrict__ part, unsigned long long *__restrict__ zero, long long zero_words) {
+    __bf16 *__restrict__ ft_lo, float *__restrict__ part, unsigned long long *__restrict__ zero, long long zero_words,
+    int main_rows, int by_xcd, int b, int m, const int *__restrict__ fidx, const float *__restrict__ ws, const float *__restrict__ bs,
+    float *__restrict__ fq, float *__restrict__ ident) {
     extern __shared__ float sf_raw[];
     float (*sf)[PS_PTS + 1] = reinterpret_cast<float (*)[PS_PTS + 1]>(sf_raw);
     __shared__ float4 sgeo[PS_PTS];
@@ -108,12 +188,16 @@
     const int wave = __builtin_amdgcn_readfirstlane(tid >> 6);
     critical_stream_priority();
     wg_stamp(0);
-    for (long long e = (long long)blockIdx.x * PS_NT + tid; e < zero_words; e += (long long)gridDim.x * PS_NT) zero[e] = 0ull;
+    if ((int)blockIdx.x >= main_rows) {
+        skip_rows_role<NS>((int)blockIdx.x - main_rows, (int)gridDim.x - main_rows, by_xcd, b, n, m, f, fidx, ws, bs, fq, ident);
+        return;
+    }
+    for (long long e = (long long)blockIdx.x * PS_NT + tid; e < zero_words; e += (long long)main_rows * PS_NT) zero[e] = 0ull;
     Frag<NS> wf[3];
     load_w1_frags<NS>(w1, r, h, wf);
     const float wp0 = eff<NS>(w1[r * 35]), wp1 = eff<NS>(w1[r * 35 + 1]), wp2 = eff<NS>(w1[r * 35 + 2]);
     float s1 = 0.0f, s2 = 0.0f;
-    for (int tile = blockIdx.x; tile < total_tiles; tile += gridDim.x) {
+    for (int tile = blockIdx.x; tile < total_tiles; tile += main_rows) {
         const int cloud = tile / tiles_per_cloud, n0 = (tile % tiles_per_cloud) * PS_PTS;
         {
             const int pt = tid & (PS_PTS - 1), cg = tid / PS_PTS;
@@ -1105,13 +1189,17 @@
     return (int)(tiles < apn::PS_MAX_ROWS ? (tiles < 1 ? 1 : tiles) : apn::PS_MAX_ROWS);
 }
 
-extern "C" int apn_sa_prep_stats(int b, int n, const float *f, const void *geo, const void *dd, const float *w1,
-                                 int precision, int stats, void *ft, float *part1, void *zero, long long zero_words,
-                                 void *stream) {
+extern "C" int apn_sa_prep_stats_skip(int b, int n, int m, const float *f, const void *geo, const void *dd,
+                                      const float *w1, int precision, int stats, void *ft, float *part1, void *zero,
+                                      long long zero_words, const int *fidx, const float *ws, const float *bs, float *fq,
+                                      float *ident, void *stream) {
     using namespace apn;
     if (b <= 0 || n <= 0 || b > 65535 || (precision != 1 && precision != 2) || !f || !ft || !w1) return APN_EINVAL;
     if (stats && (!geo || !dd || !part1 || ((uintptr_t)geo & 15) || ((uintptr_t)part1 & 15))) return APN_EINVAL;
     if (zero_words < 0 || (zero_words && !zero)) return APN_EINVAL;
+    if (ident && !fq) return APN_EINVAL;
+    if (fq && (m <= 0 || !fidx || ((uintptr_t)fq & 15))) return APN_EINVAL;
+    if (ident && (!ws || ((uintptr_t)ws & 15) || ((uintptr_t)ident & 15))) return APN_EINVAL;
     __bf16 *hi = (__bf16 *)ft;
     __bf16 *lo = precision == 2 ? hi + (size_t)b * n * SA_C : nullptr;
     const int tpc = (n + PS_PTS - 1) / PS_PTS;
@@ -1119,11 +1207,28 @@
     const int lds = SA_C * (PS_PTS + 1) * (int)sizeof(float);
     static DynLdsOnce lds_set[2];
     if (hipError_t e = set_dyn_lds(lds_set[precision - 1], (const void *)kern, lds)) return (int)e;
-    hipLaunchKernelGGL(kern, dim3(apn_sa_prep_rows(b, n)), dim3(PS_NT), lds, (hipStream_t)stream, n, tpc, b * tpc, f,
+    const int rows = apn_sa_prep_rows(b, n);
+    int roles = 0, by_xcd = 0;
+    if (fq) {
+        const char *e1 = getenv("APN_SR_MAX"), *e2 = getenv("APN_SR_XCD");
+        const int cap = e1 ? atoi(e1) : SR_MAX_ROWS;
+        by_xcd = e2 ? atoi(e2) : 0;
+        const long long want = (long long)b * ((m + 31) / 32);
+        roles = (int)(want < cap ? want : cap);
+        if (by_xcd) roles = (roles + 7) & ~7;
+    }
+    hipLaunchKernelGGL(kern, dim3(rows + roles), dim3(PS_NT), lds, (hipStream_t)stream, n, tpc, b * tpc, f,
                        (const long long *)geo, (const double *)dd, b * (apn_sa_geo_dd_doubles(n) / 6), w1, stats, hi, lo, part1,
-                       (unsigned long long *)zero, zero_words);
+                       (unsigned long long *)zero, zero_words, rows, by_xcd, b, m, fidx, ws, bs, fq, ident);
     APN_LAUNCH_CHECK();
     return APN_OK;
+}
+
+extern "C" int apn_sa_prep_stats(int b, int n, const float *f, const void *geo, const void *dd, const float *w1,
+                                 int precision, int stats, void *ft, float *part1, void *zero, long long zero_words,
+                                 void *stream) {
+    return apn_sa_prep_stats_skip(b, n, 0, f, geo, dd, w1, precision, stats, ft, part1, zero, zero_words, nullptr, nullptr,
+                                  nullptr, nullptr, nullptr, stream);
 }
 
 #ifdef APN_WG_STAMPS
diff --git a/adaptpoint_amd/csrc/sa_glue.hip b/adaptpoint_amd/csrc/sa_glue.hip
--- a/adaptpoint_amd/csrc/sa_glue.hip
+++ b/adaptpoint_amd/csrc/sa_glue.hip
@@ -193,6 +193,34 @@
     for (int t = 0; t < WPT; ++t) sws[q0 + G * t][i] = wv[t];
 }
 
+template <int NT, int QT, int WST, int FST>
+__device__ __forceinline__ void stage_skip_rows(int cloud, int m, int m0, const float *__restrict__ fq,
+                                                const int *__restrict__ fidx, const float *__restrict__ ws,
+                                                float (*sws)[WST], float (*sfi)[FST], int *ssrc) {
+    constexpr int G = NT / 32, QPT = QT / G, WPT = 64 / G;
+    const int tid = threadIdx.x, i = tid & 31, q0 = tid >> 5;
+    int src[QPT];
+    float v[QPT];
+#pragma unroll
+    for (int t = 0; t < QPT; ++t) {
+        const int q = m0 + q0 + G * t;
+        const size_t row = (size_t)cloud * m + (q < m ? q : m - 1);
+        src[t] = ssrc ? fidx[row] : 0;
+        v[t] = fq[row * 32 + i];
+    }
+    float wv[WPT];
+#pragma unroll
+    for (int t = 0; t < WPT; ++t) wv[t] = ws[(q0 + G * t) * 32 + i];
+#pragma unroll
+    for (int t = 0; t < QPT; ++t) {
+        const bool in = m0 + q0 + G * t < m;
+        sfi[q0 + G * t][i] = in ? v[t] : 0.0f;
+        if (ssrc && i == 0) ssrc[q0 + G * t] = in ? src[t] : 0;
+    }
+#pragma unroll
+    for (int t = 0; t < WPT; ++t) sws[q0 + G * t][i] = wv[t];
+}
+
 template <int QT>
 __global__ __launch_bounds__(QT * 16) void fwd_out_kernel(int n, int m, const float *__restrict__ ysel,
                                                           const unsigned long long *__restrict__ acc2,
@@ -204,7 +232,8 @@
                                                           const float *__restrict__ ws,
                                                           const float *__restrict__ bs, int relu,
                                                           float *__restrict__ out, float4 *__restrict__ zero,
-                                                          long long zero_n4) {
+                                                          long long zero_n4, const float *__restrict__ fq,
+                                                          const float *__restrict__ ident) {
     constexpr int NT = QT * 16, NW = NT / 64, HALVES = 64 / QT;
     __shared__ float tile[QT][65];
     __shared__ __attribute__((aligned(16))) float sfi[QT][36];
@@ -228,13 +257,20 @@
     const int cloud = blockIdx.y, m0 = blockIdx.x * QT;
     const int tx = threadIdx.x & 63, ty = threadIdx.x >> 6;
     if (threadIdx.x >= 128 && threadIdx.x < 192) s_bs[tx] = (ws && bs) ? bs[tx] : 0.0f;
-    float ys4[4];
+    const bool hoisted = ws && ident;
+    const float *idp = hoisted ? ident : ysel;
+    float ys4[4], id4[4];
 #pragma unroll
     for (int k = 0; k < 4; ++k) {
         const int q = m0 + ty + NW * k;
-        ys4[k] = ysel[((size_t)cloud * m + (q < m ? q : m - 1)) * 64 + tx];
-    }
-    if (ws) stage_skip_operands<NT, QT, 36, 36>(cloud, n, m, m0, ft, ft_lo, fidx, ws, sws, sfi, nullptr);
+        const size_t o = ((size_t)cloud * m + (q < m ? q : m - 1)) * 64 + tx;
+        ys4[k] = ysel[o];
+        id4[k] = idp[o];
+    }
+    if (ws && !hoisted) {
+        if (fq) stage_skip_rows<NT, QT, 36, 36>(cloud, m, m0, fq, fidx, ws, sws, sfi, nullptr);
+        else stage_skip_operands<NT, QT, 36, 36>(cloud, n, m, m0, ft, ft_lo, fidx, ws, sws, sfi, nullptr);
+    }
     wg_stamp(1);
     __syncthreads();
     wg_stamp(2);
@@ -252,13 +288,15 @@
 #pragma unroll
         for (int k = 0; k < 4; ++k) {
             const int j = ty + NW * k;
-            tile[j][tx] = m0 + j < m ? ys4[k] * sc + sh : 0.f;
+            float t = ys4[k] * sc + sh;
+            if (hoisted) t = t + id4[k];
+            tile[j][tx] = m0 + j < m ? t : 0.f;
         }
     }
     wg_stamp(3);
     __syncthreads();
     wg_stamp(4);
-    if (ws) {
+    if (ws && !hoisted) {
         constexpr int QB = QT / 32;
         if (ty < 2 * QB) {
             const int cb = ty & 1, qb = ty >> 1, r = tx & 31, h = tx >> 5;
@@ -315,7 +353,8 @@
                                                            unsigned long long *__restrict__ accS,
                                                            float *__restrict__ partWs,
                                                            float *__restrict__ gip,
-                                                           const int *__restrict__ dup) {
+                                                           const int *__restrict__ dup,
+                                                           const float *__restrict__ fq) {
     constexpr int NT = QT * 16, NW = NT / 64, HALVES = 64 / QT;
     __shared__ float tile[QT][65];
     __shared__ float red[NW][2][64];
@@ -345,7 +384,10 @@
         const int q = m0 + ty + NW * k;
         ys[k] = ysel[((size_t)cloud * m + (q < m ? q : m - 1)) * 64 + tx];
     }
-    if (ws) stage_skip_operands<NT, QT, 33, 36>(cloud, n, m, m0, ft, ft_lo, fidx, ws, sws, sfi, ssrc);
+    if (ws) {
+        if (fq) stage_skip_rows<NT, QT, 33, 36>(cloud, m, m0, fq, fidx, ws, sws, sfi, ssrc);
+        else stage_skip_operands<NT, QT, 33, 36>(cloud, n, m, m0, ft, ft_lo, fidx, ws, sws, sfi, ssrc);
+    }
 #pragma unroll
     for (int k = 0; k < 4; ++k) {
         const int c = (ty + NW * k) * HALVES + hh;
@@ -803,23 +845,24 @@
                               const float *g2, const float *b2, float *rm2, float *rv2, void *nbt2, float eps2,
                               float mom2, int train2, double count, float *pack2, const void *ft, int precision,
                               const int *fidx, const float *ws, const float *bs, int relu, float *out,
-                              float *zero_base, long long zero_floats, void *stream) {
+                              float *zero_base, long long zero_floats, const float *fq, const float *ident,
+                              void *stream) {
     if (b <= 0 || m <= 0 || b > 65535 || !ysel || !pack2 || !out) return APN_EINVAL;
     if (train2 && !acc2 && !sums2) return APN_EINVAL;
     if (!train2 && (!rm2 || !rv2)) return APN_EINVAL;
-    if (ws && (!ft || !fidx || n <= 0 || (precision != 1 && precision != 2))) return APN_EINVAL;
+    if (ws && !ident && !fq && (!ft || !fidx || n <= 0 || (precision != 1 && precision != 2))) return APN_EINVAL;
     const __bf16 *hi = (const __bf16 *)ft;
-    const __bf16 *lo = (ws && precision == 2) ? hi + (size_t)b * n * 32 : nullptr;
+    const __bf16 *lo = (ws && hi && precision == 2) ? hi + (size_t)b * n * 32 : nullptr;
     if (zero_base && (zero_floats < 0 || (zero_floats & 3) || ((uintptr_t)zero_base & 15))) return APN_EINVAL;
     apn::BnArgs bn{g2, b2, rm2, rv2, (long long *)nbt2, eps2, mom2, train2, count};
     if (apn_sa_glue_tile(b, m) == 32)
         hipLaunchKernelGGL(apn::fwd_out_kernel<32>, dim3((m + 31) / 32, b), dim3(512), 0, APN_ST, n, m, ysel,
                            (const unsigned long long *)(sums2 ? nullptr : acc2), sums2, bn, pack2, hi, lo, fidx, ws, bs,
-                           relu, out, (float4 *)zero_base, zero_base ? zero_floats / 4 : 0);
+                           relu, out, (float4 *)zero_base, zero_base ? zero_floats / 4 : 0, fq, ident);
     else
         hipLaunchKernelGGL(apn::fwd_out_kernel<64>, dim3((m + 63) / 64, b), dim3(1024), 0, APN_ST, n, m, ysel,
                            (const unsigned long long *)(sums2 ? nullptr : acc2), sums2, bn, pack2, hi, lo, fidx, ws, bs,
-                           relu, out, (float4 *)zero_base, zero_base ? zero_floats / 4 : 0);
+                           relu, out, (float4 *)zero_base, zero_base ? zero_floats / 4 : 0, fq, ident);
     APN_LAUNCH_CHECK();
     return APN_OK;
 }
@@ -833,21 +876,21 @@
                                long long gs_c, long long gs_m, const float *out, int relu,
                                const float *ysel, const float *pack2, const void *ft, int precision,
                                const int *fidx, const float *ws, float *goa, void *accS,
-                               float *partWs, float *gip, const int *dup, void *stream) {
+                               float *partWs, float *gip, const int *dup, const float *fq, void *stream) {
     if (b <= 0 || m <= 0 || b > 65535 || !g_out || !ysel || !pack2 || !goa || !accS) return APN_EINVAL;
     if (relu && !out) return APN_EINVAL;
-    if (ws && (!ft || !fidx || !partWs || !gip || n <= 0 || (precision != 1 && precision != 2)))
+    if (ws && (!fidx || !partWs || !gip || n <= 0 || (!fq && (!ft || (precision != 1 && precision != 2)))))
         return APN_EINVAL;
     const __bf16 *hi = (const __bf16 *)ft;
-    const __bf16 *lo = (ws && precision == 2) ? hi + (size_t)b * n * 32 : nullptr;
+    const __bf16 *lo = (ws && hi && precision == 2) ? hi + (size_t)b * n * 32 : nullptr;
     if (apn_sa_glue_tile(b, m) == 32)
         hipLaunchKernelGGL(apn::bwd_prep_kernel<32>, dim3((m + 31) / 32, b), dim3(512), 0, APN_ST, n, m, g_out,
                            gs_b, gs_c, gs_m, out, relu, ysel, pack2, hi, lo, fidx, ws, goa, (unsigned long long *)accS,
-                           partWs, gip, dup);
+                           partWs, gip, dup, fq);
     else
         hipLaunchKernelGGL(apn::bwd_prep_kernel<64>, dim3((m + 63) / 64, b), dim3(1024), 0, APN_ST, n, m, g_out,
                            gs_b, gs_c, gs_m, out, relu, ysel, pack2, hi, lo, fidx, ws, goa, (unsigned long long *)accS,
-                           partWs, gip, dup);
+                           partWs, gip, dup, fq);
     APN_LAUNCH_CHECK();
     return APN_OK;
 }
diff --git a/adaptpoint_amd/csrc/sa_seq.hip b/adaptpoint_amd/csrc/sa_seq.hip
--- a/adaptpoint_amd/csrc/sa_seq.hip
+++ b/adaptpoint_amd/csrc/sa_seq.hip
@@ -38,10 +38,12 @@
     int train2,
     double count, int relu, void *ft, float *part1, const double *sums1, const double *sums2,
     float *pack1, float *pack2, void *acc2, float *ysel, void *ksel,
-    float *out, float *zero_base, long long zero_floats, void *stream) {
+    float *out, float *zero_base, long long zero_floats,
+    float *fq, float *ident, void *stream) {
+    if (!ws) fq = ident = nullptr;
     if (phases & 1)
-        APN_TRY(apn_sa_prep_stats(b, n, f, geo, dd, w1, precision, train1, ft, part1, acc2, apn_sa_acc_words(128),
-                                  stream));
+        APN_TRY(apn_sa_prep_stats_skip(b, n, m, f, geo, dd, w1, precision, train1, ft, part1, acc2, apn_sa_acc_words(128),
+                                       fq ? fidx : nullptr, ws, bs, fq, ident, stream));
     if (phases & 2)
         APN_TRY(apn_sa_fwd_main(b, n, m, precision, radius, xyz, new_xyz, ft, idx, tmap, w1, w2, g1, b1, rm1, rv1,
                                 nbt1, eps1, mom1, train1, count, part1, apn_sa_prep_rows(b, n), sums1, pack1, g2,
@@ -49,7 +51,7 @@
     if (phases & 4)
         APN_TRY(apn_sa_fwd_out(b, n, m, ysel, acc2, sums2, g2, b2, rm2, rv2, nbt2, eps2, mom2, train2, count, pack2,
                                ws ? ft : nullptr, precision, ws ? fidx : nullptr, ws, bs, relu, out, zero_base,
-                               zero_floats, stream));
+                               zero_floats, fq, ident, stream));
     return APN_OK;
 }
 
@@ -64,12 +66,14 @@
     float *goa, float *partWs, float *partW2, float *partW, const double *sumsS, const double *sumsT,
     float *HA, float *HB,
     float *g_f, float *g_p, float *g_newp, float *g_w1, float *g_w2, float *g_g1, float *g_b1, float *g_g2,
-    float *g_b2, float *g_ws, float *g_bs, void *stream) {
+    float *g_b2, float *g_ws, float *g_bs,
+    const float *fq,
+    void *stream) {
     if (phases & 1) {
         if (zero_bytes) APN_TRY(apn_zero_fill(zero_base, zero_bytes, stream));
         APN_TRY(apn_sa_bwd_prep(b, n, m, g_out, gs_b, gs_c, gs_m, out, relu, ysel, pack2, ws ? ft : nullptr, precision,
                                 ws ? fidx : nullptr, ws, goa, accS, partWs, gip,
-                                pcnt_poff ? pcnt_poff + 2ll * b * n : nullptr, stream));
+                                pcnt_poff ? pcnt_poff + 2ll * b * n : nullptr, ws ? fq : nullptr, stream));
     }
     if (phases & 2)
         APN_TRY(apn_sa_bwd_main(b, n, m, precision, radius, xyz, new_xyz, ft, idx, tmap, w1, w2, pack1, pack2, accS,
diff --git a/adaptpoint_amd/fused.py b/adaptpoint_amd/fused.py
--- a/adaptpoint_amd/fused.py
+++ b/adaptpoint_amd/fused.py
@@ -161,7 +161,10 @@
         rows1 = lib.apn_sa_prep_rows(B, N)
         v, _buf = _carve(dev, [("ft", prec * B * N * C // 2), ("pack1", 4 * C_MID), ("pack2", 4 * C_OUT),
                                ("ysel", B * M * C_OUT), ("ksel", B * M * C_OUT // 4),
-                               ("part1", rows1 * 64), ("acc2", _acc_floats(128))])
+                               ("part1", rows1 * 64), ("acc2", _acc_floats(128))]
+                         + ([("fq", B * M * C_IN), ("ident", B * M * C_OUT)]
+                            if ws is not None and not PER_KERNEL_LAUNCH else []))
+        fq, ident = v.get("fq"), v.get("ident")
         out = torch.empty(B, C_OUT, M, dtype=torch.float32, device=dev)
         self.zsizes = (([("gip", B * N * C_MID)] if ws is not None else [])
                        + [("accS", _acc_floats(128)), ("accT", _acc_floats(64))])
@@ -182,7 +185,7 @@
                  w1.data_ptr(), w2.data_ptr(), _ptr(ws), _ptr(bs), *bn1a, *bn2a, count, self.relu,
                  v["ft"].data_ptr(), v["part1"].data_ptr(), _ptr(sums1), _ptr(sums2),
                  v["pack1"].data_ptr(), v["pack2"].data_ptr(), v["acc2"].data_ptr(),
-                 v["ysel"].data_ptr(), v["ksel"].data_ptr(), out.data_ptr(), zptr, zfl)
+                 v["ysel"].data_ptr(), v["ksel"].data_ptr(), out.data_ptr(), zptr, zfl, _ptr(fq), _ptr(ident))
 
         if not _phased(sync_bn):
             run(7)
@@ -196,7 +199,7 @@
         self.saved = dict(p=p, f=f, new_p=new_p, idx=idx, tmap=tmap, rowmap=rowmap, fidx=fidx,
                           geo=geo, ft=v["ft"], w1=w1, w2=w2, ws=ws,
                           has_bs=bs is not None, pack1=v["pack1"], pack2=v["pack2"], ysel=v["ysel"],
-                          ksel=v["ksel"], count=count)
+                          ksel=v["ksel"], count=count, fq=fq)
 
 
 def _backward(fw, g_out, need_p, need_newp):
@@ -259,7 +262,8 @@
              v["partWs"].data_ptr() if has_skip else None, v["partW2"].data_ptr(), v["partW"].data_ptr(),
              _ptr(sumsS), _ptr(sumsT), v["HA"].data_ptr(), v["HB"].data_ptr(),
              g_f.data_ptr(), _ptr(g_p), _ptr(g_newp), g["w1"].data_ptr(), g["w2"].data_ptr(),
-             g["g1"].data_ptr(), g["b1"].data_ptr(), g["g2"].data_ptr(), g["b2"].data_ptr(), gws, gbs)
+             g["g1"].data_ptr(), g["b1"].data_ptr(), g["g2"].data_ptr(), g["b2"].data_ptr(), gws, gbs,
+             _ptr(sv["fq"]))
 
     if not _phased(sync):
         run(7)
@@ -289,7 +293,7 @@
     if phases & 4:
         call("apn_sa_fwd_out", B, N, M, v["ysel"].data_ptr(), v["acc2"].data_ptr(), _ptr(sums2), *bn2a, count,
              v["pack2"].data_ptr(), v["ft"].data_ptr() if ws is not None else None, prec,
-             _ptr(fidx) if ws is not None else None, _ptr(ws), _ptr(bs), relu, out.data_ptr(), zptr, zfl)
+             _ptr(fidx) if ws is not None else None, _ptr(ws), _ptr(bs), relu, out.data_ptr(), zptr, zfl, None, None)
 
 
 def _backward_per_kernel(call, phases, fw, sv, g_out, buf, zero_floats, v, g, sumsS, sumsT, g_f, g_p,
@@ -304,7 +308,8 @@
              sv["ysel"].data_ptr(), sv["pack2"].data_ptr(), sv["ft"].data_ptr() if has_skip else None,
              fw.prec, _ptr(sv["fidx"]) if has_skip else None, _ptr(ws), v["goa"].data_ptr(),
              v["accS"].data_ptr(), v["partWs"].data_ptr() if has_skip else None, gip,
-             pcnt_poff.data_ptr() + 8 * B * N)
+             pcnt_poff.data_ptr() + 8 * B * N,
+             None)
     if phases & 2:
         call("apn_sa_bwd_main", B, N, M, fw.prec, fw.radius, sv["p"].data_ptr(), sv["new_p"].data_ptr(),
              sv["ft"].data_ptr(), sv["idx"].data_ptr(), _ptr(sv["tmap"]), w1.data_ptr(), w2.data_ptr(),
diff --git a/include/adaptpoint_amd.h b/include/adaptpoint_amd.h
--- a/include/adaptpoint_amd.h
+++ b/include/adaptpoint_amd.h
@@ -80,6 +80,10 @@
 APN_API int apn_sa_prep_stats(int b, int n, const float *f, const void *geo, const void *dd, const float *w1,
                               int precision, int stats, void *ft, float *part1, void *zero, long long zero_words,
                               void *stream);
+APN_API int apn_sa_prep_stats_skip(int b, int n, int m, const float *f, const void *geo, const void *dd,
+                                   const float *w1, int precision, int stats, void *ft, float *part1, void *zero,
+                                   long long zero_words, const int *fidx, const float *ws, const float *bs, float *fq,
+                                   float *ident, void *stream);
 
 APN_API int apn_sa_reduce_rows(const float *part, int rows, int ncol, double count, double *out,
                                void *stream);
@@ -102,14 +106,15 @@
                            const float *g2, const float *b2, float *rm2, float *rv2, void *nbt2, float eps2,
                            float mom2, int train2, double count, float *pack2, const void *ft, int precision,
                            const int *fidx, const float *ws, const float *bs, int relu, float *out,
-                           float *zero_base, long long zero_floats, void *stream);
+                           float *zero_base, long long zero_floats, const float *fq, const float *ident,
+                           void *stream);
 
 APN_API int apn_sa_bwd_prep_rows(int b, int m);
 APN_API int apn_sa_bwd_prep(int b, int n, int m, const float *g_out, long long gs_b,
                             long long gs_c, long long gs_m, const float *out, int relu,
                             const float *ysel, const float *pack2, const void *ft, int precision,
                             const int *fidx, const float *ws, float *goa, void *accS,
-                            float *partWs, float *gip, const int *dup, void *stream);
+                            float *partWs, float *gip, const int *dup, const float *fq, void *stream);
 
 APN_API int apn_sa_bwd_main(int b, int n, int m, int precision, float radius, const float *xyz,
                             const float *new_xyz, const void *ft, const int *idx, const int *tmap, const float *w1,
@@ -144,7 +149,9 @@
     int train2,
     double count, int relu, void *ft, float *part1, const double *sums1, const double *sums2,
     float *pack1, float *pack2, void *acc2, float *ysel, void *ksel,
-    float *out, float *zero_base, long long zero_floats, void *stream);
+    float *out, float *zero_base, long long zero_floats,
+    float *fq, float *ident,
+    void *stream);
 APN_API int apn_sa_backward_seq(
     int phases, int precision, int b, int n, int m, float radius, const float *xyz, const float *new_xyz,
     const int *idx, const int *tmap, const int *fidx, const void *geo, const float *w1, const float *w2,
@@ -156,7 +163,7 @@
     float *goa, float *partWs, float *partW2, float *partW, const double *sumsS, const double *sumsT,
     float *HA, float *HB,
     float *g_f, float *g_p, float *g_newp, float *g_w1, float *g_w2, float *g_g1, float *g_b1, float *g_g2,
-    float *g_b2, float *g_ws, float *g_bs, void *stream);
+    float *g_b2, float *g_ws, float *g_bs, const float *fq, void *stream);
 APN_API int apn_sa_sample_overlap(int b, int n, int m, float radius, int nsample,
                                   const float *xyz_a, int *fidx_a, float *new_xyz_a,
                                   const float *xyz_b, const float *new_xyz_b, int *idx_b,
```

Result: no change. 123,100, median of 4 (+0.4%).
